# IDEA-Research/MP-Former

Measured on AMD Instinct MI355X. Metric: training images/sec COCO-instance R50 1024x1024, higher is better.
Workload: dtype bf16 (backbone, decoder) + f32 (pixel decoder, losses), as the reference's AMP; 1 GPU; COCO-instance R50, 100 queries, 80 classes, 1024x1024: full train step = R50 backbone + MSDeformAttn pixel decoder (6 layers) + MP masked decoder (9 layers, NUM_DN 1) + Hungarian matching + 60 losses + backward + grad all-reduce + clip + AdamW; head_only_workload=False, global_batch=2, per_gpu_batch=2, parallelism=dp1, msda_offsets=init, full=False, autograd_threads=backward on the launch thread, miopen_find_db=shipped

## Files before the change

include/mpformer_hip.h:

```cpp
#ifndef MPFORMER_HIP_H
#define MPFORMER_HIP_H

#include <stddef.h>
#include <stdint.h>

#ifdef __cplusplus
extern "C" {
#endif

enum { MPF_F32 = 0, MPF_F64 = 1, MPF_BF16 = 2, MPF_U8 = 3, MPF_BITS = 4  };

enum {
    MPF_OK = 0,
    MPF_E_DTYPE = -1,
    MPF_E_SHAPE = -2,
    MPF_E_NULL = -3,
    MPF_E_TOO_LARGE = -4
};

int mpf_abi_version(void);
const char* mpf_last_error(void);


int mpf_msda_forward(const void* value, const int64_t* spatial_shapes,
// ... 174 lines not shown
                       int pad, uint8_t* out, int32_t* flags, int N, int Q, int HW, void* stream);

typedef struct MpfLsaProblem {
    int64_t cost_off, n_rows, n_cols, row_stride;
    int64_t out_pos, col_base;
    int64_t a_base, a_stride, b_base, b_stride;
    int64_t scatter_base;
} MpfLsaProblem;

int mpf_lsa_assign(const float* cost, const MpfLsaProblem* problems, int n_problems, int max_dim, int64_t max_entries,
                   int32_t* row_out, int32_t* col_out, int64_t* aff_a, int64_t* aff_b, int64_t* scatter_dst,
                   const int64_t* scatter_src, void* stream);
int mpf_lsa_assign_status(const float* cost, const MpfLsaProblem* problems, int n_problems, int max_dim, int64_t max_entries,
                          int32_t* row_out, int32_t* col_out, int64_t* aff_a, int64_t* aff_b, int64_t* scatter_dst,
                          const int64_t* scatter_src, int32_t* status, void* stream);

typedef struct MpfDecoderLayer {
    const void *ca_wq, *ca_bq, *ca_wo, *ca_bo;
    const float *ca_gamma, *ca_beta;
    const void *sa_wq, *sa_bq, *sa_wk, *sa_bk, *sa_wv, *sa_bv, *sa_wo, *sa_bo;
    const float *sa_gamma, *sa_beta;
    const void *ff_w1, *ff_b1, *ff_w2, *ff_b2;
    const float *ff_gamma, *ff_beta;
    const float* x0;
    const void* xb0;
    const void *k_c, *v_c;
    const uint8_t *mask_c, *mask_s;
    void *q_c, *kT_c, *o_c;
    float* lse_c;
    float *s1, *mean1, *rstd1;
    void* xb1;
    void *q_s, *k_s, *v_s, *kT_s, *o_s;
    float* lse_s;
    float *s2, *mean2, *rstd2;
    void* xb2;
    void* h;
    float *s3, *mean3, *rstd3;
    float* x3;
    void* xb3;
    void *scratch, *attn_ws;
    uint64_t scratch_bytes, attn_ws_bytes;
    int32_t Qt, N, H, S, ffn_dim;
    float eps;
    int64_t kv_row_stride, kv_img_stride;
} MpfDecoderLayer;

typedef struct MpfDecoderLayerGrad {
    const float* g_x3;
    const void* g_xb3;
    float* d_x0;
    void* d_xb0;
    void *d_k_c, *d_v_c;
    void *d_ca_wq, *d_ca_bq, *d_ca_wo, *d_ca_bo;
    void *d_sa_wq, *d_sa_bq, *d_sa_wk, *d_sa_bk, *d_sa_wv, *d_sa_bv, *d_sa_wo, *d_sa_bo;
    void *d_ff_w1, *d_ff_b1, *d_ff_w2, *d_ff_b2;
    float* d_ln;
    int64_t dkv_row_stride, dkv_img_stride;
    const float* g_x3_plus;
} MpfDecoderLayerGrad;

int mpf_lin256_res_ln_forward(const void* a, const void* w, const void* bias, const float* x, const float* gamma, const float* beta,
                              float* s_out, float* y32, void* y16, float* mean, float* rstd, int rows, float eps, void* stream);
int mpf_ln256_mlp3_forward(const float* x, const float* gamma, const float* beta, const void* w0, const void* b0, const void* w1,
                           const void* b1, const void* w2, const void* b2, void* out, int rows, float eps, void* stream);
uint64_t mpf_decoder_layer_struct_bytes(int which);
uint64_t mpf_decoder_layer_scratch_bytes(int Qt, int N, int H, int S, int ffn_dim, int backward);
int mpf_decoder_layer_forward(const MpfDecoderLayer* layer, void* stream);
typedef struct MpfNextMask {
    const float* x;
    const float* ln_gamma;
    const float* ln_beta;
    const void* w0;
    const void* b0;
    const void* w1;
    const void* b1;
    const void* w2;
    const void* b2;
    const void* pooled;
    const uint8_t* mp_rows;
    uint8_t* out;
    int32_t* flags;
    void* scratch;
    size_t scratch_bytes;
    int N, Q, HW, pad;
    float eps;
} MpfNextMask;
size_t mpf_next_attn_mask_scratch_bytes(int N, int Q);
int mpf_next_attn_mask(const MpfNextMask* m, void* stream);
int mpf_decoder_layer_backward(const MpfDecoderLayer* layer, const MpfDecoderLayerGrad* grad, void* stream);

typedef struct MpfDecoderLayerPos {
    const float* qpos;
    void *xq0, *xq1;
    float* d_qpos;
} MpfDecoderLayerPos;
int mpf_qpos_operand_forward(const float* x, const float* qpos, void* out, int Q, int N, void* stream);
int mpf_qpos_backward(const void* dxq0, const void* dxq1, float* d_x0, float* d_qpos, int Q, int N, void* stream);
uint64_t mpf_decoder_layer_pos_struct_bytes(void);
uint64_t mpf_decoder_layer_pos_scratch_bytes(int Qt, int N, int H, int S, int ffn_dim, int backward);
int mpf_decoder_layer_pos_forward(const MpfDecoderLayer* layer, const MpfDecoderLayerPos* pos, void* stream);
int mpf_decoder_layer_pos_backward(const MpfDecoderLayer* layer, const MpfDecoderLayerPos* pos, const MpfDecoderLayerGrad* grad,
                                   void* stream);

typedef struct MpfScaleCastItem {
    const void* src;
    void* dst;
    const float* scale;
    int64_t numel, inner, first_block;
} MpfScaleCastItem;

int mpf_grouped_scale_cast(const MpfScaleCastItem* items_device, int n_items, int64_t total_blocks, int src_dtype, int dst_dtype,
                           void* stream);

#define MPF_AMAX_SLOT_FLOATS 512
typedef struct MpfAmaxItem {
    const float* src;
    float* out;
    int64_t numel, first_block;
} MpfAmaxItem;
typedef struct MpfSplitItemH2 {
    const float* src;
    void* dst;
    const float* amax;
    int64_t rows, cols, transpose, dst_ld, plane_stride, first_block;
} MpfSplitItemH2;
int mpf_amax_f32(const float* x, int64_t n, float* amax, void* stream);
int mpf_amax_f32_grouped(const MpfAmaxItem* items_device, int n_items, int64_t total_blocks, void* stream);
int mpf_h2_range_stats(const float* a, int rows, int cols, int64_t lda, const float* amax_slot, int log2_below,
                       unsigned long long* counters_device, void* stream);
int mpf_gemm3_split_grouped_h2(const MpfSplitItemH2* items_device, int n_items, int64_t total_blocks, void* stream);
typedef struct MpfNtItemH2 {
    const float* a;
    int64_t lda;
    const float* a_amax;
    const float* b;
    int64_t ldb;
    const float* b_amax;
    float* c_part;
    float* csum_a;
    int64_t Mdim, Ndim;
} MpfNtItemH2;
int mpf_gemm3_nt_h2(const float* a, int64_t lda, const float* a_amax, const float* b, int64_t ldb, const float* b_amax,
                    float* c_part, float* csum_a, float* csum_b, int R, int Mdim, int Ndim, int rows_per_split,
                    int transpose_out, void* stream);
int mpf_gemm3_nt_grouped_h2(const MpfNtItemH2* items, int n_items, int R, int rows_per_split, int64_t split_stride, void* stream);
int mpf_gemm3_conv3x3_h2(const float* x, const float* x_amax, const void* w_planes_h2, const float* w_amax, const float* bias,
                         float* y, float* out_amax, int n_img, int H, int W, int Cin, int Cout, int transposed, void* stream);
int mpf_gemm3_conv3x3_wgrad_h2(const float* dy, const float* dy_amax, const float* x, const float* x_amax, float* c_part,
                               float* csum_dy, int n_img, int H, int W, int Cin, int Cout, int rows_per_split, void* stream);
int mpf_gemm3_tn_h2(const float* a, int64_t lda, const float* a_amax, const void* b_planes_h2, const float* b_amax,
                    const float* bias, const float* c_in, int64_t ldcin, const float* c_in2, int64_t ldcin2,
                    const float* gate, int64_t ldgate, float* c, int64_t ldc, float* out_amax, int M, int N, int K,
                    int relu, void* stream);
int mpf_gemm3_tn_h2_bits(const float* a, int64_t lda, const float* a_amax, const void* b_planes_h2, const float* b_amax,
                         const float* bias, const float* c_in, int64_t ldcin, const float* c_in2, int64_t ldcin2,
                         const unsigned char* gate_bits, int64_t ldgbits, float* c, int64_t ldc, float* out_amax,
                         unsigned char* gate_bits_out, int64_t ldgbits_out, int M, int N, int K, int relu, void* stream);

typedef struct MpfNtItem {
    const float* a;
    int64_t lda;
    const float* b;
    int64_t ldb;
    float* c_part;
    float* csum_a;
    int64_t Mdim, Ndim;
} MpfNtItem;
int mpf_gemm3_nt_grouped(const MpfNtItem* items, int n_items, int R, int rows_per_split, int64_t split_stride, void* stream);

int mpf_gemm3_conv3x3(const float* x, const void* w_planes, const float* bias, float* y, int n_img, int H, int W, int Cin,
                      int Cout, int transposed, void* stream);
int mpf_gemm3_conv3x3_wgrad(const float* dy, const float* x, float* c_part, float* csum_dy, int n_img, int H, int W, int Cin, int Cout,
                            int rows_per_split, void* stream);

int mpf_gemm3_tn_ex(const void* a, int a_dtype, int64_t lda, const void* b_planes, const float* bias, const float* c_in, int64_t ldcin,
                    void* c, int c_dtype, int64_t ldc, int M, int N, int K, int relu, void* stream);
int mpf_gemm3_nt_ex(const void* a, int a_dtype, int64_t lda, const void* b, int b_dtype, int64_t ldb, float* c_part, float* csum_a,
                    int R, int Mdim, int Ndim, int rows_per_split, void* stream);

typedef struct MpfSplitItem {
    const float* src;
    void* dst;
    int64_t rows, cols, transpose, dst_ld, plane_stride, first_block;
} MpfSplitItem;

int mpf_gemm3_split_grouped(const MpfSplitItem* items_device, int n_items, int64_t total_blocks, void* stream);

typedef struct MpfOptItem {
    float* param;
    const float* grad;
    float* exp_avg;
    float* exp_avg_sq;
    int64_t numel, first_block;
    float lr, weight_decay, bc1, bc2_sqrt;
} MpfOptItem;

int mpf_clip_adamw_step(const MpfOptItem* items_device, int n_items, int64_t total_blocks, float max_norm, double beta1,
                        double beta2, double eps, float* partial, float* norm_clip, void* stream);

int mpf_transpose_f32(const float* in, int64_t in_batch_stride, float* out, int64_t out_batch_stride, int B, int R, int C,
                      void* stream);

int mpf_gemm3_nt_reduce(const float* c_part, int64_t c_numel, const float* s_part, int64_t s_numel, int nsplit,
                        float* c_out, float* s_out, void* stream);
int mpf_gemm3_nt_reduce_levels(const float* c_part, int64_t c_numel, const float* s_part, int64_t s_numel, int nsplit,
                               const int64_t* level_of_split, int n_levels, float* c_out, float* lvl_out, float* s_out, void* stream);

int mpf_tall_gemm_bf16(const void* a, int64_t lda, const void* b, int64_t ldb, const void* bias, void* c, int64_t ldc, int M, int N,
                       int K, void* stream);
size_t mpf_gemm_nt_bf16_workspace_bytes(int R, int Mdim, int Ndim, int rows_per_split);
int mpf_gemm_nt_bf16(const void* a, int64_t lda, const void* b, int64_t ldb, void* c_out, void* csum_out, int R, int Mdim,
                     int Ndim, int rows_per_split, void* workspace, size_t workspace_bytes, void* stream);

int mpf_small_gemm_bf16_blocked(const void* a, int64_t a_rs, int64_t a_ks, int a_blk, int64_t a_bs, const void* gate, const void* b,
                                int64_t b_rs, int64_t b_ks, const void* bias, const void* c_in, int64_t ldcin, void* c, int64_t ldc,
                                int c_blk, int64_t c_bs, void* rowsum_a, int I, int J, int Kc, int relu, void* stream);

int mpf_class_loss_forward(const void* logits, int dtype, int64_t sl, int64_t sn, int64_t sq, const int64_t* target,
                           int target_per_output, const float* weight, int L, int N, int Q, int C, float* lse, float* ce,
                           float* wsum, void* stream);
int mpf_class_loss_backward(const void* logits, int dtype, int64_t sl, int64_t sn, int64_t sq, const int64_t* target,
                            int target_per_output, const float* weight, int L, int N, int Q, int C, const float* lse,
                            const float* wsum, const float* grad_ce, void* dlogits, void* stream);
int mpf_mask_loss_finalize(const float* sums, const int64_t* runs, const float* norm, int n, int G, int points, float* out,
                           void* stream);
int mpf_mask_loss_finalize_backward(const float* sums, const int64_t* runs, const float* norm, int n, int G, int points,
                                    const float* grad_out, float* dsums, void* stream);

typedef struct {
    const void* a;
    const void* gate;
    const void* b;
    void* c;
    void* rowsum_a;
    int64_t a_rs, a_ks, a_bs, b_rs, b_ks, ldc;
    int a_blk, I, J, Kc;
} MpfSmallGemmItem;
int mpf_small_gemm_bf16_group(const MpfSmallGemmItem* items, int n_items, void* stream);
typedef struct MpfTransposeItem {
    const void* src;
    const void* gate;
    void* dst;
    int64_t ld;
    int R, C;
} MpfTransposeItem;
int mpf_transpose_group_bf16(const MpfTransposeItem* items, int n_items, int Rp, void* stream);

int mpf_bias_act(const void* x, const float* bias, const void* res, void* y, int64_t numel, int C, int dtype,
                 int relu, void* stream);
int mpf_relu_bwd_add(const void* ga, const void* gb, const void* y, void* out, int64_t numel, int dtype, void* stream);
int mpf_maxpool3x3s2_forward(const void* x, void* y, void* code, int N, int H, int W, int C, void* stream);
int mpf_maxpool3x3s2_backward(const void* gy, const void* code, void* gx, int N, int H, int W, int C, void* stream);

int mpf_upload_small(const void* host_src, void* device_dst, int64_t nbytes, void* stream);

int mpf_res_ln256_forward(const float* x, const void* t, int t_dtype, const float* gamma, const float* beta,
                          float* s_out, float* y32, void* y16, float* mean, float* rstd, int rows, float eps,
                          const float* padd, int padd_rows, float* y_plus, void* stream);
int mpf_res_ln256_forward_b(const float* x, const void* t, int t_dtype, const float* gamma, const float* beta, float* s_out, float* y32,
                            void* y16, float* mean, float* rstd, int rows, float eps, const float* padd, int padd_rows, float* y_plus,
                            float* y_bound, const float* padd_amax, float* yplus_bound, void* stream);
int mpf_res_ln256_backward(const float* s, const float* mean, const float* rstd, const float* gamma, const float* gy32,
                           const void* gy16, const float* gy_plus, float* ds32, void* ds16, float* dgamma, float* dbeta,
                           int rows, void* stream);
size_t mpf_res_ln256_backward_workspace_bytes(int rows);
int mpf_res_ln256_backward_ws(const float* s, const float* mean, const float* rstd, const float* gamma, const float* gy32,
                              const void* gy16, const float* gy_plus, float* ds32, void* ds16, float* dgamma, float* dbeta, int rows,
                              void* workspace, size_t workspace_bytes, void* stream);
int mpf_res_ln256_backward_ws_amax(const float* s, const float* mean, const float* rstd, const float* gamma, const float* gy32,
                                   const void* gy16, const float* gy_plus, float* ds32, void* ds16, float* dgamma, float* dbeta, int rows,
                                   void* workspace, size_t workspace_bytes, float* ds_amax, void* stream);
int mpf_res_ln256_backward_partial(const float* s, const float* mean, const float* rstd, const float* gamma, const float* gy32,
                                   const void* gy16, const float* gy_plus, float* ds32, void* ds16, int rows, void* partials,
                                   size_t partials_bytes, void* stream);
int mpf_res_ln256_backward_partial_amax(const float* s, const float* mean, const float* rstd, const float* gamma, const float* gy32,
                                        const void* gy16, const float* gy_plus, float* ds32, void* ds16, int rows, void* partials,
                                        size_t partials_bytes, float* ds_amax, void* stream);
int mpf_ln_partial_reduce(const void* partials, size_t stride_bytes, int rows, int n_ln, float* out, void* stream);
size_t mpf_res_ln256_backward_det_workspace_bytes(int rows);
int mpf_res_ln256_backward_det(const float* s, const float* mean, const float* rstd, const float* gamma, const float* gy32,
                               const void* gy16, const float* gy_plus, float* ds32, void* ds16, float* dgamma_dbeta, int rows,
                               void* workspace, size_t workspace_bytes, void* stream);
size_t mpf_res_ln256_backward_workspace_bytes(int rows);
int mpf_res_ln256_backward_ws(const float* s, const float* mean, const float* rstd, const float* gamma, const float* gy32,
                              const void* gy16, const float* gy_plus, float* ds32, void* ds16, float* dgamma, float* dbeta, int rows,
                              void* workspace, size_t workspace_bytes, void* stream);

int mpf_mask_loss_backward_dense(const void* pred, int pred_dtype, int h, int w, const int64_t* pred_rows,
                                 const void* gt, int gt_dtype, int H, int W, const int32_t* gt_rows, const float* coords,
                                 const float* grad_sums, void* grad, int grad_dtype, const int64_t* grad_offs,
                                 int n, int P, void* stream);

size_t mpf_group_stats_workspace_bytes(int rows, int64_t row_len);
int mpf_group_stats(const float* x, int rows, int64_t row_len, float eps, float* mean, float* rstd,
                    void* workspace, size_t workspace_bytes, void* stream);

int mpf_gn_cl_supported(int HW, int C, int G);
size_t mpf_gn_cl_workspace_bytes(int N, int HW, int C, int G);
int mpf_gn_cl_forward(const float* x, int64_t x_bs, const float* gamma, const float* beta, int N, int HW, int C, int G,
                      float eps, int relu, const float* top, int64_t top_bs, int W, float* y, int64_t y_bs, float* mean,
                      float* rstd, void* workspace, size_t workspace_bytes, void* stream);
int mpf_gn_cl_backward(const float* gy, int64_t gy_bs, const float* x, int64_t x_bs, const float* gamma, const float* beta,
                       const float* mean, const float* rstd, int N, int HW, int C, int G, int relu, float* dx,
                       int64_t dx_bs, float* dgamma, float* dbeta, void* workspace, size_t workspace_bytes, void* stream);
int mpf_upsample2x_cl_backward(const float* gy, int64_t gy_bs, int N, int Ht, int Wt, int C, float* dtop, int64_t dtop_bs,
                               void* stream);

size_t mpf_match_cost_fused_workspace_bytes(int G, int Q, int Tmax, int P, int tsamp_rows);
int mpf_match_cost_fused(const void* embed, const int64_t* embed_first, int64_t embed_row_stride, const void* features,
                         int64_t feat_img_stride, const int32_t* group_image, int h, int w, int channels, const float* coords,
                         const float* tsamp, int tsamp_rows, const int32_t* t_first, const int32_t* t_count, float* cost, int G,
                         int Q, int Tmax, int P, float w_mask, float w_dice, void* workspace, size_t workspace_bytes, void* stream);
size_t mpf_match_cost_fused_clip_workspace_bytes(int G, int Q, int Tmax, int P, int F, int tsamp_rows);
int mpf_match_cost_fused_clip(const void* embed, const int64_t* embed_first, int64_t embed_row_stride, const void* features,
                              int64_t feat_clip_stride, int64_t feat_frame_stride, const int32_t* group_clip, int h, int w,
                              int channels, const float* coords, const float* tsamp, int tsamp_rows, const int32_t* t_first,
                              const int32_t* t_count, float* cost, int G, int Q, int Tmax, int P, int F, float w_mask, float w_dice,
                              void* workspace, size_t workspace_bytes, void* stream);
int mpf_pair_planes_forward(const void* embed, const int64_t* row_off, const int32_t* pair_of_slot, const int32_t* slot_first,
                            const int32_t* slot_count, const void* features, int64_t feat_img_stride, void* out, int N, int HW,
                            int channels, void* stream);
size_t mpf_pair_planes_backward_workspace_bytes(int N, int HW, int total_slots, int max_count);
int mpf_pair_planes_backward(const void* grad_planes, const void* embed, const int64_t* row_off, const int32_t* pair_of_slot,
                             const int32_t* slot_first, const int32_t* slot_count, const void* features, int64_t feat_img_stride,
                             void* d_features, int64_t dfeat_img_stride, void* d_embed, int d_embed_dtype, int N, int HW, int channels,
                             int total_slots, int max_count, void* workspace, size_t workspace_bytes, void* stream);

int mpf_profile_enable(int on);
int mpf_profile_get(const char* name_substr, int* count, double* total_ms, double* total_bytes);
int mpf_profile_get_flops(const char* name_substr, double* total_flops);

enum {
    MPF_ENC_PV, MPF_ENC_PV_AM, MPF_ENC_PO, MPF_ENC_PO_AM, MPF_ENC_P1, MPF_ENC_P1_AM, MPF_ENC_P2, MPF_ENC_P2_AM, MPF_ENC_P288, MPF_ENC_P288_AM,
    MPF_ENC_BV, MPF_ENC_BO, MPF_ENC_BB1, MPF_ENC_BB2, MPF_ENC_B288, MPF_ENC_G1, MPF_ENC_B1, MPF_ENC_G2, MPF_ENC_B2,
    MPF_ENC_VALUE, MPF_ENC_RAW, MPF_ENC_LOC, MPF_ENC_ATTN, MPF_ENC_AO, MPF_ENC_S1, MPF_ENC_MEAN1, MPF_ENC_RSTD1, MPF_ENC_X1, MPF_ENC_H,
    MPF_ENC_HBITS, MPF_ENC_S2, MPF_ENC_MEAN2, MPF_ENC_RSTD2, MPF_ENC_X2, MPF_ENC_QN,
    MPF_ENC_AO_AM, MPF_ENC_X1_AM, MPF_ENC_H_AM, MPF_ENC_XN_AM, MPF_ENC_QN_AM,
    MPF_ENC_FIELDS
};
typedef struct MpfEncoderCall {
    int32_t N, S, M, L, P, nl, F, reserved;
    float eps, pad_;
    const int64_t* host_shapes;
    const void* shapes_dev;
    const void* lsi_dev;
    const float* ref;
    const float* pos_full;
    const float* pos_am;
    const float* x0;
    const float* x0_am;
    const float* q0;
    const float* q0_am;
    const uint64_t* layers;
} MpfEncoderCall;
int mpf_encoder_fields(void);
int mpf_encoder_forward(const MpfEncoderCall* call, void* stream);

enum {
    MPF_ENCB_X, MPF_ENCB_Q, MPF_ENCB_VALUE, MPF_ENCB_LOC, MPF_ENCB_ATTN, MPF_ENCB_AO, MPF_ENCB_S1, MPF_ENCB_MEAN1, MPF_ENCB_RSTD1, MPF_ENCB_X1,
    MPF_ENCB_H, MPF_ENCB_HBITS, MPF_ENCB_S2, MPF_ENCB_MEAN2, MPF_ENCB_RSTD2,
    MPF_ENCB_X_AM, MPF_ENCB_Q_AM, MPF_ENCB_AO_AM, MPF_ENCB_X1_AM, MPF_ENCB_H_AM,
    MPF_ENCB_G1, MPF_ENCB_G2,
    MPF_ENCB_TV, MPF_ENCB_TV_AM, MPF_ENCB_TO, MPF_ENCB_TO_AM, MPF_ENCB_T1, MPF_ENCB_T1_AM, MPF_ENCB_T2, MPF_ENCB_T2_AM, MPF_ENCB_T288, MPF_ENCB_T288_AM,
    MPF_ENCB_DS2_AM, MPF_ENCB_DH_AM, MPF_ENCB_DS1_AM, MPF_ENCB_DRAW_AM, MPF_ENCB_GV_AM,
    MPF_ENCB_WGRAD, MPF_ENCB_DW288, MPF_ENCB_LVL, MPF_ENCB_DB288,
    MPF_ENCB_FIELDS
};
typedef struct MpfEncoderBwdCall {
    int32_t N, S, M, L, P, nl, F, rps288, rps_group, reserved;
    int64_t group_stride;
    const int64_t* host_shapes;
    const float* gout;
    const int64_t* split_level;
    float *ds2, *dh, *dx1, *ds1, *dao, *gv, *draw;
    float* dq[2];
    float* g[2];
    float *cpart288, *cs288, *part_group;
    void* ln_parts;
    uint64_t ln_stride;
    void* msda_ws;
    uint64_t msda_ws_bytes;
    float* dgb_out;
    const uint64_t* layers;
} MpfEncoderBwdCall;
int mpf_encoder_bwd_fields(void);
int mpf_encoder_backward(const MpfEncoderBwdCall* call, void* stream);

int mpf_seg_softmax(const float* cls, int Q, int K1, float object_mask_threshold, float* probs, float* max_score, int* max_label,
                    int* kept, float* kept_score, void* stream);
int mpf_seg_semantic(const void* masks, int64_t stride_q, int dtype, int Q, int h, int w, int Hp, int Wp, int hi, int wi, int H, int W,
                     const float* probs, int K, float* out, void* stream);
size_t mpf_seg_instance_workspace_bytes(int T, int H, int W);
int mpf_seg_instance_scores(const void* masks, int64_t stride_q, int dtype, int Q, int h, int w, int Hp, int Wp, int hi, int wi, int H,
                            int W, const int64_t* sel_q, const float* cls_score, int T, float* scores, void* workspace,
                            size_t workspace_bytes, void* stream);
int mpf_seg_instance_masks(const void* masks, int64_t stride_q, int dtype, int Q, int h, int w, int Hp, int Wp, int hi, int wi, int H,
                           int W, const int64_t* sel_q, int T, float* masks_out, void* stream);
int mpf_seg_panoptic_areas(const void* masks, int64_t stride_q, int dtype, int Q, int h, int w, int Hp, int Wp, int hi, int wi, int H,
                           int W, const int* kept, const float* kept_score, int* code, int* areas, void* stream);
int mpf_seg_panoptic_paint(const int* code, int H, int W, const int* lut, int* out, void* stream);
int mpf_seg_semantic_labels(const void* masks, int64_t stride_q, int dtype, int Q, int h, int w, int Hp, int Wp, int hi, int wi, int H,
                            int W, const float* probs, int K, int* labels, void* stream);
int mpf_seg_labels_resize(const float* scores, int K, int hi, int wi, int H, int W, int* labels, void* stream);
int mpf_seg_confusion_add(const int* pred, const int* gt, int64_t n, int K, int ignore_label, int64_t* conf, void* stream);
size_t mpf_seg_instance_rle_workspace_bytes(int T, int H, int W);
int mpf_seg_instance_rle_count(const void* masks, int64_t stride_q, int dtype, int Q, int h, int w, int Hp, int Wp, int hi, int wi, int H,
                               int W, const int64_t* sel_q, int T, int64_t* offsets, void* workspace, size_t workspace_bytes,
                               void* stream);
int mpf_seg_instance_rle_write(const void* workspace, size_t workspace_bytes, int T, int H, int W, const int64_t* offsets, int64_t total,
                               uint32_t* pos, uint32_t* counts, void* stream);

int mpf_seg_tta_accumulate(const void* masks, int64_t stride_q, int dtype, int Q, int h, int w, int Hp, int Wp, int hi, int wi, int H,
                           int W, const float* probs, int K, int mode, float* acc, void* stream);
int mpf_seg_tta_resize_add(const float* scores, int K, int hi, int wi, int H, int W, int mode, float* acc, void* stream);
int mpf_seg_tta_finish(float* acc, int K, int H, int W, int count, int* labels , void* stream);

size_t mpf_seg_pq_workspace_bytes(int G, int S);
int mpf_seg_pq_pairs(const int* pred, const void* gt, int gt_format, int64_t n, const int* gt_ids, int G, int gt_base,
                     const int* pred_ids, int S, int pred_base, int void_id, int* table, size_t table_bytes, void* stream);
int mpf_seg_pq_match(int* table, size_t table_bytes, int G, int S, int K, const int* gt_cat, const int* gt_flags, const int* pred_cat,
                     int implicit, int64_t* tp, int64_t* fp, int64_t* fn, double* iou, int64_t* err, void* stream);

int mpf_seg_instance_bits(const void* masks, int64_t stride_q, int dtype, int Q, int h, int w, int Hp, int Wp, int hi, int wi, int H,
                          int W, const int64_t* sel_q, int T, uint64_t* bits, void* stream);
int mpf_seg_pack_masks(const void* masks, int dtype, int M, int H, int W, uint64_t* bits, void* stream);
int mpf_seg_mask_pairs(const uint64_t* a_bits, int T, const uint64_t* b_bits, int G, int64_t nwords, int* inter, int* area_a,
                       int* area_b, void* stream);
size_t mpf_seg_ap_workspace_bytes(int G, int A, int Tn);
int mpf_seg_ap_match(const int* inter, const int* area_d, const int* area_g, int D, int G, const float* dt_score, const int* dt_cat,
                     const int* gt_cat, const int* gt_crowd, const double* gt_area, const double* iou_thrs, int Tn,
                     const double* area_rngs, int A, int K, int max_det, int crowd_rule, int image, int64_t* records, int64_t* npig,
                     void* workspace, size_t workspace_bytes, void* stream);

int mpf_seg_mask_boundary(const uint64_t* bits, int M, int H, int W, int d, uint64_t* out, void* stream);
int mpf_seg_ap_match_boundary(const int* inter, const int* area_d, const int* area_g, const int* inter_b, const int* area_db,
                              const int* area_gb, int D, int G, const float* dt_score, const int* dt_cat, const int* gt_cat,
                              const int* gt_crowd, const double* gt_area, const double* iou_thrs, int Tn, const double* area_rngs, int A,
                              int K, int max_det, int crowd_rule, int image, int64_t* records, int64_t* npig, void* workspace,
                              size_t workspace_bytes, void* stream);

int mpf_seg_bits_boxes(const uint64_t* bits, int M, int H, int W, int* boxes , void* stream);
int mpf_seg_ap_match_box(const double* dt_box , const double* gt_box , int D, int G,
                         const float* dt_score, const int* dt_cat, const int* gt_cat, const int* gt_crowd, const double* gt_area,
                         const double* iou_thrs, int Tn, const double* area_rngs, int A, int K, int max_det, int crowd_rule, int image,
                         int64_t* records, int64_t* npig, void* workspace, size_t workspace_bytes, void* stream);

int mpf_seg_video_bits(const void* masks, int64_t stride_q, int64_t stride_f, int dtype, int Q, int F, int h, int w, int Hp, int Wp,
                       int hi, int wi, int H, int W, const int64_t* sel_q, int T, uint64_t* bits, int* frame_area,
                       uint8_t* dense , void* stream);
int mpf_seg_tube_areas(const int* frame_area, int M, int F, double* avg_area, void* stream);
int mpf_seg_ap_match_tube(const int* inter, const int* area_d, const int* area_g, int D, int G, const float* dt_score, const int* dt_cat,
                          const int* gt_cat, const int* gt_crowd, const double* gt_area, const double* dt_area, const double* iou_thrs,
                          int Tn, const double* area_rngs, int A, int K, int max_det, int crowd_rule, int image, int64_t* records,
                          int64_t* npig, void* workspace, size_t workspace_bytes, void* stream);
size_t mpf_seg_bits_rle_workspace_bytes(int M, int H, int W);
int mpf_seg_bits_rle_count(const uint64_t* bits, int M, int H, int W, int64_t* offsets, void* workspace, size_t workspace_bytes,
                           void* stream);
int mpf_seg_bits_rle_write(const uint64_t* bits, const void* workspace, size_t workspace_bytes, int M, int H, int W,
                           const int64_t* offsets, int64_t total, uint32_t* pos, uint32_t* counts, void* stream);

int mpf_seg_poly_stage_edges(void);
int mpf_seg_poly_toggles(const double* xy, const int64_t* ring_off, int R, int H, int W, uint64_t* planes, void* stream);
int mpf_seg_rle_toggles(const uint32_t* counts, const int64_t* off, int M, int H, int W, uint64_t* planes, void* stream);
int mpf_seg_toggles_fill(const uint64_t* planes, const int* plane_obj, int R, int M, int H, int W, uint64_t* bits, void* stream);
int mpf_seg_unpack_masks(const uint64_t* bits, int M, int H, int W, uint8_t* masks, void* stream);

size_t mpf_win_attn_workspace_bytes(int B, int Hp, int Wp, int heads, int ws);
int mpf_win_attn_forward(const void* qkv, const float* table, void* out, int B, int Hp, int Wp, int heads, int head_dim, int ws,
                         int shift, float scale, void* stream);
int mpf_win_attn_backward(const void* qkv, const float* table, const void* out, const void* dout, void* dqkv, float* dtable, int B,
                          int Hp, int Wp, int heads, int head_dim, int ws, int shift, float scale, void* workspace,
                          size_t workspace_bytes, void* stream);

#ifdef __cplusplus
}
#endif
#endif
```

mp_former_amd/_lib.py:

```python
import ctypes

import torch
import os

_HERE = os.path.dirname(os.path.abspath(__file__))
LIB_PATH = os.path.join(_HERE, "libmpformer_hip.so")
LIB_PATH = os.environ.get("MPF_LIB_PATH", LIB_PATH)
ABI_VERSION = 1

MPF_F32, MPF_F64, MPF_BF16, MPF_U8, MPF_BITS = 0, 1, 2, 3, 4
DTYPE = {torch.float32: MPF_F32, torch.float64: MPF_F64, torch.bfloat16: MPF_BF16, torch.uint8: MPF_U8, torch.bool: MPF_U8}

_lib = None
_status_fns = {}

_c_int = ctypes.c_int
_c_vp = ctypes.c_void_p

SIGNATURES = {
    "mpf_abi_version": (_c_int, []),
    "mpf_last_error": (ctypes.c_char_p, []),
    "mpf_last_kernel": (ctypes.c_char_p, []),
    "mpf_set_option": (_c_int, [ctypes.c_char_p, _c_int]),
    "mpf_match_cost_fused_workspace_bytes": (ctypes.c_size_t, [_c_int] * 5),
    "mpf_match_cost_fused": (_c_int, [_c_vp, _c_vp, ctypes.c_int64, _c_vp, ctypes.c_int64, _c_vp, _c_int, _c_int, _c_int, _c_vp, _c_vp, _c_int,
                                      _c_vp, _c_vp, _c_vp, _c_int, _c_int, _c_int, _c_int, ctypes.c_float, ctypes.c_float, _c_vp,
                                      ctypes.c_size_t, _c_vp]),
    "mpf_match_cost_fused_clip_workspace_bytes": (ctypes.c_size_t, [_c_int] * 6),
    "mpf_match_cost_fused_clip": (_c_int, [_c_vp, _c_vp, ctypes.c_int64, _c_vp, ctypes.c_int64, ctypes.c_int64, _c_vp, _c_int, _c_int, _c_int,
                                           _c_vp, _c_vp, _c_int, _c_vp, _c_vp, _c_vp, _c_int, _c_int, _c_int, _c_int, _c_int, ctypes.c_float,
                                           ctypes.c_float, _c_vp, ctypes.c_size_t, _c_vp]),
    "mpf_pair_planes_forward": (_c_int, [_c_vp] * 6 + [ctypes.c_int64, _c_vp, _c_int, _c_int, _c_int, _c_vp]),
    "mpf_pair_planes_backward_workspace_bytes": (ctypes.c_size_t, [_c_int] * 4),
    "mpf_pair_planes_backward": (_c_int, [_c_vp] * 7 + [ctypes.c_int64, _c_vp, ctypes.c_int64, _c_vp, _c_int, _c_int, _c_int, _c_int, _c_int,
                                          _c_int, _c_vp, ctypes.c_size_t, _c_vp]),
    "mpf_msda_dev_workspace_bytes": (ctypes.c_size_t, [_c_int] * 7),
    "mpf_msda_forward_dev": (_c_int, [_c_vp] * 6 + [_c_int] * 8 + [_c_vp, ctypes.c_size_t, _c_vp]),
    "mpf_msda_backward_dev": (_c_int, [_c_vp] * 9 + [_c_int] * 8 + [_c_vp, ctypes.c_size_t, _c_vp]),
    "mpf_msda_dev_geometry": (_c_int, [_c_vp, ctypes.POINTER(_c_int), _c_int]),
    "mpf_msda_stats": (_c_int, [ctypes.POINTER(ctypes.c_ulonglong), _c_int, _c_int]),
    "mpf_profile_enable": (_c_int, [_c_int]),
    "mpf_profile_get_flops": (_c_int, [ctypes.c_char_p, ctypes.POINTER(ctypes.c_double)]),
    "mpf_profile_get": (_c_int, [ctypes.c_char_p, ctypes.POINTER(_c_int), ctypes.POINTER(ctypes.c_double),
                                 ctypes.POINTER(ctypes.c_double)]),
    "mpf_point_sample": (_c_int, [_c_vp, _c_int, _c_int, _c_int, _c_vp, _c_vp, _c_vp, _c_vp, _c_int, _c_int, _c_vp]),
    "mpf_mask_loss_forward": (_c_int, [_c_vp, _c_int, _c_int, _c_int, _c_vp, _c_vp, _c_int, _c_int, _c_int, _c_vp, _c_vp,
                                       _c_vp, _c_int, _c_int, _c_int, _c_vp]),
    "mpf_pack_mask_bits": (_c_int, [_c_vp, _c_vp, ctypes.c_int64, _c_vp]),
    "mpf_mask_loss_backward": (_c_int, [_c_vp, _c_int, _c_int, _c_int, _c_vp, _c_vp, _c_int, _c_int, _c_vp, _c_vp,
                                        _c_vp, _c_vp, _c_vp, _c_int, _c_int, _c_vp]),
    "mpf_select_uncertain": (_c_int, [_c_vp, _c_vp, _c_vp, _c_int, _c_int, _c_int, _c_int, _c_vp]),
    "mpf_sample_select_uncertain": (_c_int, [_c_vp, _c_int, _c_int, _c_int, _c_vp, _c_vp, _c_vp, _c_int, _c_int, _c_int, _c_int, _c_vp]),
    "mpf_match_cost": (_c_int, [_c_vp, _c_int, _c_int, _c_int, _c_vp, _c_vp, _c_vp, _c_vp, _c_vp, _c_vp, _c_vp,
                                _c_int, _c_int, _c_int, ctypes.c_float, ctypes.c_float, _c_int, _c_vp]),
    "mpf_match_cost_clip_workspace_bytes": (ctypes.c_size_t, [_c_int] * 3),
    "mpf_match_cost_clip": (_c_int, [_c_vp, _c_int, _c_int, _c_int, _c_vp, _c_int, ctypes.c_int64, _c_vp, _c_vp, _c_vp, _c_vp, _c_vp, _c_vp,
                                     _c_int, _c_int, _c_int, ctypes.c_float, ctypes.c_float, _c_int, _c_vp, ctypes.c_size_t, _c_vp]),
    "mpf_attn_mask": (_c_int, [_c_vp, _c_int, ctypes.c_int64, ctypes.c_int64, _c_int, _c_int, _c_vp, _c_int, _c_vp,
                               _c_int, _c_int, _c_int, _c_int, _c_vp]),
    "mpf_attn_workspace_bytes": (ctypes.c_size_t, [_c_int] * 4),
    "mpf_attn_forward": (_c_int, [_c_vp, _c_vp, _c_vp, _c_vp, _c_int, _c_vp, _c_vp, _c_int, _c_int, _c_int, _c_int, _c_int,
                                  ctypes.c_float, _c_vp, ctypes.c_size_t, _c_vp]),
    "mpf_attn_backward": (_c_int, [_c_vp] * 8 + [_c_int] + [_c_vp] * 5 + [_c_int] * 6 + [ctypes.c_float, _c_vp, ctypes.c_size_t, _c_vp]),
    "mpf_attn_transpose2": (_c_int, [_c_vp] * 4 + [_c_int] * 4 + [_c_vp]),
    "mpf_attn_transpose2_strided": (_c_int, [_c_vp] * 2 + [ctypes.c_int64] * 2 + [_c_vp] * 2 + [_c_int] * 4 + [_c_vp]),
    "mpf_attn_forward_kv": (_c_int, [_c_vp, _c_vp, ctypes.c_int64, ctypes.c_int64, _c_vp, _c_vp, _c_int, _c_vp, _c_vp, _c_int, _c_int,
                                     _c_int, _c_int, _c_int, ctypes.c_float, _c_vp, ctypes.c_size_t, _c_vp]),
    "mpf_attn_backward_kv": (_c_int, [_c_vp] * 3 + [ctypes.c_int64] * 2 + [_c_vp] * 5 + [_c_int] + [_c_vp] * 5 + [ctypes.c_int64] * 2
                             + [_c_int] * 6 + [ctypes.c_float, _c_vp, ctypes.c_size_t, _c_vp]),
    "mpf_attn_backward_kv_aux": (_c_int, [_c_vp] * 3 + [ctypes.c_int64] * 2 + [_c_vp] * 5 + [_c_int] + [_c_vp] * 5 + [ctypes.c_int64] * 2
                                 + [_c_int] * 6 + [ctypes.c_float, _c_vp, ctypes.c_size_t, _c_vp, _c_vp]),
    "mpf_attn_bwd_aux_bytes": (ctypes.c_size_t, [_c_int] * 5),
    "mpf_attn_bwd_prep_aux": (_c_int, [_c_vp] * 5 + [_c_int] * 2 + [_c_vp] * 4 + [ctypes.c_size_t] + [_c_int] * 4 + [_c_vp]),
    "mpf_attn_delta": (_c_int, [_c_vp] * 3 + [_c_int] * 3 + [_c_vp]),
    "mpf_attn_bwd_prep": (_c_int, [_c_vp] * 6 + [_c_int] * 4 + [_c_vp]),
    "mpf_win_attn_workspace_bytes": (ctypes.c_size_t, [_c_int] * 5),
    "mpf_win_attn_forward": (_c_int, [_c_vp] * 3 + [_c_int] * 7 + [ctypes.c_float, _c_vp]),
    "mpf_win_attn_backward": (_c_int, [_c_vp] * 6 + [_c_int] * 7 + [ctypes.c_float, _c_vp, ctypes.c_size_t, _c_vp]),
    "mpf_gemm3_split": (_c_int, [_c_vp, _c_int, _c_int, _c_int, _c_vp, _c_vp]),
    "mpf_gemm3_tn": (_c_int, [_c_vp, ctypes.c_int64, _c_vp, _c_int, _c_vp, _c_vp, _c_vp, ctypes.c_int64, _c_vp, ctypes.c_int64,
                           _c_vp, ctypes.c_int64, _c_vp, ctypes.c_int64, _c_int, _c_int, _c_int, _c_int, _c_vp]),
    "mpf_gemm3_nt": (_c_int, [_c_vp, ctypes.c_int64, _c_vp, ctypes.c_int64, _c_vp, ctypes.c_int64, _c_int, _c_vp, _c_vp, _c_vp,
                           _c_int, _c_int, _c_int, _c_int, _c_int, _c_vp]),
    "mpf_amax_f32": (_c_int, [_c_vp, ctypes.c_int64, _c_vp, _c_vp]),
    "mpf_amax_f32_grouped": (_c_int, [_c_vp, _c_int, ctypes.c_int64, _c_vp]),
    "mpf_h2_range_stats": (_c_int, [_c_vp, _c_int, _c_int, ctypes.c_int64, _c_vp, _c_int, _c_vp, _c_vp]),
    "mpf_gemm3_split_grouped_h2": (_c_int, [_c_vp, _c_int, ctypes.c_int64, _c_vp]),
    "mpf_gemm3_tn_h2": (_c_int, [_c_vp, ctypes.c_int64, _c_vp, _c_vp, _c_vp, _c_vp, _c_vp, ctypes.c_int64, _c_vp, ctypes.c_int64,
                              _c_vp, ctypes.c_int64, _c_vp, ctypes.c_int64, _c_vp, _c_int, _c_int, _c_int, _c_int, _c_vp]),
    "mpf_gemm3_tn_h2_bits": (_c_int, [_c_vp, ctypes.c_int64, _c_vp, _c_vp, _c_vp, _c_vp, _c_vp, ctypes.c_int64, _c_vp, ctypes.c_int64,
                                   _c_vp, ctypes.c_int64, _c_vp, ctypes.c_int64, _c_vp, _c_vp, ctypes.c_int64,
                                   _c_int, _c_int, _c_int, _c_int, _c_vp]),
    "mpf_gemm3_nt_h2": (_c_int, [_c_vp, ctypes.c_int64, _c_vp, _c_vp, ctypes.c_int64, _c_vp, _c_vp, _c_vp, _c_vp,
                              _c_int, _c_int, _c_int, _c_int, _c_int, _c_vp]),
    "mpf_gemm3_nt_grouped_h2": (_c_int, [_c_vp, _c_int, _c_int, _c_int, ctypes.c_int64, _c_vp]),
    "mpf_gemm3_conv3x3_h2": (_c_int, [_c_vp] * 7 + [_c_int] * 6 + [_c_vp]),
    "mpf_gemm3_conv3x3_wgrad_h2": (_c_int, [_c_vp, _c_vp, _c_vp, _c_vp, _c_vp, _c_vp, _c_int, _c_int, _c_int, _c_int, _c_int, _c_int, _c_vp]),
    "mpf_gemm3_nt_grouped": (_c_int, [_c_vp, _c_int, _c_int, _c_int, ctypes.c_int64, _c_vp]),
    "mpf_small_gemm_bf16": (_c_int, [_c_vp, ctypes.c_int64, ctypes.c_int64, _c_vp, _c_vp, ctypes.c_int64, ctypes.c_int64, _c_vp, _c_vp,
                                     ctypes.c_int64, _c_vp, ctypes.c_int64, _c_vp, _c_int, _c_int, _c_int, _c_int, _c_vp]),
    "mpf_encoder_fields": (_c_int, []),
    "mpf_encoder_forward": (_c_int, [_c_vp, _c_vp]),
    "mpf_encoder_bwd_fields": (_c_int, []),
    "mpf_encoder_backward": (_c_int, [_c_vp, _c_vp]),
    "mpf_decoder_layer_struct_bytes": (ctypes.c_uint64, [_c_int]),
    "mpf_decoder_layer_scratch_bytes": (ctypes.c_uint64, [_c_int] * 6),
    "mpf_decoder_layer_forward": (_c_int, [_c_vp, _c_vp]),
    "mpf_next_attn_mask_scratch_bytes": (ctypes.c_size_t, [_c_int, _c_int]),
    "mpf_next_attn_mask": (_c_int, [_c_vp, _c_vp]),
    "mpf_lin256_res_ln_forward": (_c_int, [_c_vp] * 11 + [_c_int, ctypes.c_float, _c_vp]),
    "mpf_ln256_mlp3_forward": (_c_int, [_c_vp] * 10 + [_c_int, ctypes.c_float, _c_vp]),
    "mpf_decoder_layer_backward": (_c_int, [_c_vp, _c_vp, _c_vp]),
    "mpf_qpos_operand_forward": (_c_int, [_c_vp, _c_vp, _c_vp, _c_int, _c_int, _c_vp]),
    "mpf_qpos_backward": (_c_int, [_c_vp, _c_vp, _c_vp, _c_vp, _c_int, _c_int, _c_vp]),
    "mpf_decoder_layer_pos_struct_bytes": (ctypes.c_uint64, []),
    "mpf_decoder_layer_pos_scratch_bytes": (ctypes.c_uint64, [_c_int] * 6),
    "mpf_decoder_layer_pos_forward": (_c_int, [_c_vp, _c_vp, _c_vp]),
    "mpf_decoder_layer_pos_backward": (_c_int, [_c_vp, _c_vp, _c_vp, _c_vp]),
    "mpf_pool_features": (_c_int, [_c_vp, _c_int, _c_vp] + [_c_int] * 6 + [_c_vp]),
    "mpf_pool_features_cl": (_c_int, [_c_vp, ctypes.c_int64, _c_int, _c_vp, _c_int, _c_int, _c_int, _c_int, _c_int, _c_int, _c_vp]),
    "mpf_mask_head_bits": (_c_int, [_c_vp, ctypes.c_int64, ctypes.c_int64, _c_vp, _c_vp, _c_int, _c_vp, _c_vp] + [_c_int] * 3 + [_c_vp]),
    "mpf_lsa_assign": (_c_int, [_c_vp, _c_vp, _c_int, _c_int, ctypes.c_int64] + [_c_vp] * 7),
    "mpf_lsa_assign_status": (_c_int, [_c_vp, _c_vp, _c_int, _c_int, ctypes.c_int64] + [_c_vp] * 8),
    "mpf_mask_block_empty": (_c_int, [_c_vp, _c_vp] + [_c_int] * 5 + [_c_vp]),
    "mpf_mp_open_counts": (_c_int, [_c_vp, _c_int, _c_int, _c_vp, _c_vp]),
    "mpf_mp_noise_rows": (_c_int, [_c_vp] * 3 + [_c_int] * 4 + [ctypes.c_double, ctypes.c_uint64, ctypes.c_uint64, _c_vp, _c_vp]),
    "mpf_gemm_nt_bf16_workspace_bytes": (ctypes.c_size_t, [_c_int] * 4),
    "mpf_gemm_nt_bf16": (_c_int, [_c_vp, ctypes.c_int64, _c_vp, ctypes.c_int64, _c_vp, _c_vp, _c_int, _c_int, _c_int, _c_int, _c_vp,
                                  ctypes.c_size_t, _c_vp]),
    "mpf_gemm3_nt_reduce": (_c_int, [_c_vp, ctypes.c_int64, _c_vp, ctypes.c_int64, _c_int, _c_vp, _c_vp, _c_vp]),
    "mpf_grouped_scale_cast": (_c_int, [_c_vp, _c_int, ctypes.c_int64, _c_int, _c_int, _c_vp]),
    "mpf_gemm3_split_grouped": (_c_int, [_c_vp, _c_int, ctypes.c_int64, _c_vp]),
    "mpf_decoder_inputs_forward": (_c_int, [_c_vp, ctypes.c_int64, ctypes.c_int64, _c_vp, _c_vp, _c_vp, _c_vp, _c_int, _c_int, _c_int, _c_int,
                                            _c_vp]),
    "mpf_decoder_inputs_backward": (_c_int, [_c_vp, _c_vp, _c_int, _c_vp, ctypes.c_int64, ctypes.c_int64, _c_int, _c_int, _c_int, _c_vp]),
    "mpf_clip_inputs_forward": (_c_int, [_c_vp, ctypes.c_int64, ctypes.c_int64, _c_vp, _c_vp, _c_vp, _c_vp, _c_vp, _c_int, _c_int, _c_int, _c_int,
                                         _c_int, _c_vp]),
    "mpf_clip_inputs_backward": (_c_int, [_c_vp, _c_vp, _c_int, _c_vp, ctypes.c_int64, ctypes.c_int64, _c_int, _c_int, _c_int, _c_int, _c_vp]),
    "mpf_clip_adamw_step": (_c_int, [_c_vp, _c_int, ctypes.c_int64, ctypes.c_float, ctypes.c_double, ctypes.c_double, ctypes.c_double,
                                     _c_vp, _c_vp, _c_vp]),
    "mpf_transpose_f32": (_c_int, [_c_vp, ctypes.c_int64, _c_vp, ctypes.c_int64, _c_int, _c_int, _c_int, _c_vp]),
    "mpf_small_gemm_bf16_blocked": (_c_int, [_c_vp, ctypes.c_int64, ctypes.c_int64, _c_int, ctypes.c_int64, _c_vp, _c_vp, ctypes.c_int64,
                                             ctypes.c_int64, _c_vp, _c_vp, ctypes.c_int64, _c_vp, ctypes.c_int64, _c_int, ctypes.c_int64,
                                             _c_vp, _c_int, _c_int, _c_int, _c_int, _c_vp]),
    "mpf_small_gemm_bf16_group": (_c_int, [_c_vp, _c_int, _c_vp]),
    "mpf_transpose_group_bf16": (_c_int, [_c_vp, _c_int, _c_int, _c_vp]),
    "mpf_class_loss_forward": (_c_int, [_c_vp, _c_int, ctypes.c_int64, ctypes.c_int64, ctypes.c_int64, _c_vp, _c_int, _c_vp, _c_int, _c_int,
                                        _c_int, _c_int, _c_vp, _c_vp, _c_vp, _c_vp]),
    "mpf_class_loss_backward": (_c_int, [_c_vp, _c_int, ctypes.c_int64, ctypes.c_int64, ctypes.c_int64, _c_vp, _c_int, _c_vp, _c_int, _c_int,
                                         _c_int, _c_int, _c_vp, _c_vp, _c_vp, _c_vp, _c_vp]),
    "mpf_mask_loss_finalize": (_c_int, [_c_vp, _c_vp, _c_vp, _c_int, _c_int, _c_int, _c_vp, _c_vp]),
    "mpf_mask_loss_finalize_backward": (_c_int, [_c_vp, _c_vp, _c_vp, _c_int, _c_int, _c_int, _c_vp, _c_vp, _c_vp]),
    "mpf_bias_act": (_c_int, [_c_vp, _c_vp, _c_vp, _c_vp, ctypes.c_int64, _c_int, _c_int, _c_int, _c_vp]),
    "mpf_relu_bwd_add": (_c_int, [_c_vp, _c_vp, _c_vp, _c_vp, ctypes.c_int64, _c_int, _c_vp]),
    "mpf_maxpool3x3s2_forward": (_c_int, [_c_vp] * 3 + [_c_int] * 4 + [_c_vp]),
    "mpf_maxpool3x3s2_backward": (_c_int, [_c_vp] * 3 + [_c_int] * 4 + [_c_vp]),
    "mpf_upload_small": (_c_int, [_c_vp, _c_vp, ctypes.c_int64, _c_vp]),
    "mpf_tall_gemm_bf16": (_c_int, [_c_vp, ctypes.c_int64, _c_vp, ctypes.c_int64, _c_vp, _c_vp, ctypes.c_int64, _c_int, _c_int, _c_int, _c_vp]),
    "mpf_res_ln256_forward": (_c_int, [_c_vp, _c_vp, _c_int, _c_vp, _c_vp, _c_vp, _c_vp, _c_vp, _c_vp, _c_vp, _c_int, ctypes.c_float,
                                       _c_vp, _c_int, _c_vp, _c_vp]),
    "mpf_res_ln256_forward_b": (_c_int, [_c_vp, _c_vp, _c_int, _c_vp, _c_vp, _c_vp, _c_vp, _c_vp, _c_vp, _c_vp, _c_int, ctypes.c_float,
                                         _c_vp, _c_int, _c_vp, _c_vp, _c_vp, _c_vp, _c_vp]),
    "mpf_res_ln256_backward_ws_amax": (_c_int, [_c_vp] * 11 + [_c_int, _c_vp, ctypes.c_size_t, _c_vp, _c_vp]),
    "mpf_res_ln256_backward": (_c_int, [_c_vp] * 11 + [_c_int, _c_vp]),
    "mpf_mask_loss_backward_dense": (_c_int, [_c_vp, _c_int, _c_int, _c_int, _c_vp, _c_vp, _c_int, _c_int, _c_int, _c_vp, _c_vp, _c_vp,
                                              _c_vp, _c_int, _c_vp, _c_int, _c_int, _c_vp]),
    "mpf_gn_cl_supported": (_c_int, [_c_int, _c_int, _c_int]),
    "mpf_gn_cl_workspace_bytes": (ctypes.c_size_t, [_c_int, _c_int, _c_int, _c_int]),
    "mpf_gn_cl_forward": (_c_int, [_c_vp, ctypes.c_int64, _c_vp, _c_vp, _c_int, _c_int, _c_int, _c_int, ctypes.c_float, _c_int,
                                   _c_vp, ctypes.c_int64, _c_int, _c_vp, ctypes.c_int64, _c_vp, _c_vp, _c_vp, ctypes.c_size_t, _c_vp]),
    "mpf_gn_cl_backward": (_c_int, [_c_vp, ctypes.c_int64, _c_vp, ctypes.c_int64, _c_vp, _c_vp, _c_vp, _c_vp, _c_int, _c_int, _c_int,
                                    _c_int, _c_int, _c_vp, ctypes.c_int64, _c_vp, _c_vp, _c_vp, ctypes.c_size_t, _c_vp]),
    "mpf_upsample2x_cl_backward": (_c_int, [_c_vp, ctypes.c_int64, _c_int, _c_int, _c_int, _c_int, _c_vp, ctypes.c_int64, _c_vp]),
    "mpf_gemm3_conv3x3": (_c_int, [_c_vp, _c_vp, _c_vp, _c_vp, _c_int, _c_int, _c_int, _c_int, _c_int, _c_int, _c_vp]),
    "mpf_gemm3_conv3x3_wgrad": (_c_int, [_c_vp, _c_vp, _c_vp, _c_vp, _c_int, _c_int, _c_int, _c_int, _c_int, _c_int, _c_vp]),
    "mpf_gemm3_nt_reduce_levels": (_c_int, [_c_vp, ctypes.c_int64, _c_vp, ctypes.c_int64, _c_int, _c_vp, _c_int, _c_vp, _c_vp, _c_vp, _c_vp]),
    "mpf_gemm3_tn_ex": (_c_int, [_c_vp, _c_int, ctypes.c_int64, _c_vp, _c_vp, _c_vp, ctypes.c_int64, _c_vp, _c_int, ctypes.c_int64,
                                 _c_int, _c_int, _c_int, _c_int, _c_vp]),
    "mpf_gemm3_nt_ex": (_c_int, [_c_vp, _c_int, ctypes.c_int64, _c_vp, _c_int, ctypes.c_int64, _c_vp, _c_vp, _c_int, _c_int, _c_int, _c_int, _c_vp]),
    "mpf_res_ln256_backward_workspace_bytes": (ctypes.c_size_t, [_c_int]),
    "mpf_res_ln256_backward_partial": (_c_int, [_c_vp] * 9 + [_c_int, _c_vp, ctypes.c_size_t, _c_vp]),
    "mpf_res_ln256_backward_partial_amax": (_c_int, [_c_vp] * 9 + [_c_int, _c_vp, ctypes.c_size_t, _c_vp, _c_vp]),
    "mpf_ln_partial_reduce": (_c_int, [_c_vp, ctypes.c_size_t, _c_int, _c_int, _c_vp, _c_vp]),
    "mpf_res_ln256_backward_det_workspace_bytes": (ctypes.c_size_t, [_c_int]),
    "mpf_res_ln256_backward_det": (_c_int, [_c_vp] * 10 + [_c_int, _c_vp, ctypes.c_size_t, _c_vp]),
    "mpf_res_ln256_backward_ws": (_c_int, [_c_vp] * 11 + [_c_int, _c_vp, ctypes.c_size_t, _c_vp]),
    "mpf_group_stats_workspace_bytes": (ctypes.c_size_t, [_c_int, ctypes.c_int64]),
    "mpf_group_stats": (_c_int, [_c_vp, _c_int, ctypes.c_int64, ctypes.c_float, _c_vp, _c_vp, _c_vp, ctypes.c_size_t, _c_vp]),
    "mpf_msda_forward": (_c_int, [_c_vp] * 6 + [_c_int] * 8 + [_c_vp]),
    "mpf_msda_backward": (_c_int, [_c_vp] * 9 + [_c_int] * 8 + [_c_vp]),
    "mpf_msda_forward_hs": (_c_int, [_c_vp] * 7 + [_c_int] * 8 + [_c_vp]),
    "mpf_msda_forward_raw_hs": (_c_int, [_c_vp] * 9 + [_c_int] * 8 + [_c_vp]),
    "mpf_msda_forward_raw": (_c_int, [_c_vp] * 8 + [_c_int] * 8 + [_c_vp]),
    "mpf_msda_backward_ws_raw": (_c_int, [_c_vp] * 7 + [_c_int] * 8 + [_c_vp, ctypes.c_size_t, _c_vp]),
    "mpf_msda_backward_ws_raw_o": (_c_int, [_c_vp] * 8 + [_c_int] * 8 + [_c_vp, ctypes.c_size_t, _c_vp, _c_vp, _c_vp]),
    "mpf_msda_backward_workspace_bytes": (ctypes.c_size_t, [_c_int] * 5 + [_c_vp]),
    "mpf_msda_backward_ws": (_c_int, [_c_vp] * 8 + [_c_int] * 8 + [_c_vp, ctypes.c_size_t, _c_vp]),
    "mpf_seg_softmax": (_c_int, [_c_vp, _c_int, _c_int, ctypes.c_float] + [_c_vp] * 6),
    "mpf_seg_semantic": (_c_int, [_c_vp, ctypes.c_int64] + [_c_int] * 10 + [_c_vp, _c_int, _c_vp, _c_vp]),
    "mpf_seg_instance_workspace_bytes": (ctypes.c_size_t, [_c_int] * 3),
    "mpf_seg_instance_scores": (_c_int, [_c_vp, ctypes.c_int64] + [_c_int] * 10 + [_c_vp, _c_vp, _c_int, _c_vp, _c_vp, ctypes.c_size_t,
                                                                                   _c_vp]),
    "mpf_seg_instance_masks": (_c_int, [_c_vp, ctypes.c_int64] + [_c_int] * 10 + [_c_vp, _c_int, _c_vp, _c_vp]),
    "mpf_seg_panoptic_areas": (_c_int, [_c_vp, ctypes.c_int64] + [_c_int] * 10 + [_c_vp] * 5),
    "mpf_seg_panoptic_paint": (_c_int, [_c_vp, _c_int, _c_int, _c_vp, _c_vp, _c_vp]),
    "mpf_seg_semantic_labels": (_c_int, [_c_vp, ctypes.c_int64] + [_c_int] * 10 + [_c_vp, _c_int, _c_vp, _c_vp]),
    "mpf_seg_labels_resize": (_c_int, [_c_vp] + [_c_int] * 5 + [_c_vp, _c_vp]),
    "mpf_seg_confusion_add": (_c_int, [_c_vp, _c_vp, ctypes.c_int64, _c_int, _c_int, _c_vp, _c_vp]),
    "mpf_seg_instance_rle_workspace_bytes": (ctypes.c_size_t, [_c_int] * 3),
    "mpf_seg_instance_rle_count": (_c_int, [_c_vp, ctypes.c_int64] + [_c_int] * 10 + [_c_vp, _c_int, _c_vp, _c_vp, ctypes.c_size_t, _c_vp]),
    "mpf_seg_instance_rle_write": (_c_int, [_c_vp, ctypes.c_size_t, _c_int, _c_int, _c_int, _c_vp, ctypes.c_int64, _c_vp, _c_vp, _c_vp]),
    "mpf_seg_tta_accumulate": (_c_int, [_c_vp, ctypes.c_int64] + [_c_int] * 10 + [_c_vp, _c_int, _c_int, _c_vp, _c_vp]),
    "mpf_seg_tta_resize_add": (_c_int, [_c_vp] + [_c_int] * 6 + [_c_vp, _c_vp]),
    "mpf_seg_tta_finish": (_c_int, [_c_vp] + [_c_int] * 4 + [_c_vp, _c_vp]),
    "mpf_seg_pq_workspace_bytes": (ctypes.c_size_t, [_c_int] * 2),
    "mpf_seg_pq_pairs": (_c_int, [_c_vp, _c_vp, _c_int, ctypes.c_int64, _c_vp, _c_int, _c_int, _c_vp, _c_int, _c_int, _c_int, _c_vp,
                                  ctypes.c_size_t, _c_vp]),
    "mpf_seg_pq_match": (_c_int, [_c_vp, ctypes.c_size_t, _c_int, _c_int, _c_int, _c_vp, _c_vp, _c_vp, _c_int] + [_c_vp] * 6),
    "mpf_seg_instance_bits": (_c_int, [_c_vp, ctypes.c_int64] + [_c_int] * 10 + [_c_vp, _c_int, _c_vp, _c_vp]),
    "mpf_seg_pack_masks": (_c_int, [_c_vp, _c_int, _c_int, _c_int, _c_int, _c_vp, _c_vp]),
    "mpf_seg_mask_pairs": (_c_int, [_c_vp, _c_int, _c_vp, _c_int, ctypes.c_int64, _c_vp, _c_vp, _c_vp, _c_vp]),
    "mpf_seg_ap_workspace_bytes": (ctypes.c_size_t, [_c_int] * 3),
    "mpf_seg_ap_match": (_c_int, [_c_vp, _c_vp, _c_vp, _c_int, _c_int] + [_c_vp] * 6 + [_c_int, _c_vp] + [_c_int] * 5
                         + [_c_vp, _c_vp, _c_vp, ctypes.c_size_t, _c_vp]),
    "mpf_seg_mask_boundary": (_c_int, [_c_vp, _c_int, _c_int, _c_int, _c_int, _c_vp, _c_vp]),
    "mpf_seg_ap_match_boundary": (_c_int, [_c_vp] * 6 + [_c_int, _c_int] + [_c_vp] * 6 + [_c_int, _c_vp] + [_c_int] * 5
                                  + [_c_vp, _c_vp, _c_vp, ctypes.c_size_t, _c_vp]),
    "mpf_seg_bits_boxes": (_c_int, [_c_vp, _c_int, _c_int, _c_int, _c_vp, _c_vp]),
    "mpf_seg_ap_match_box": (_c_int, [_c_vp, _c_vp, _c_int, _c_int] + [_c_vp] * 6 + [_c_int, _c_vp] + [_c_int] * 5
                             + [_c_vp, _c_vp, _c_vp, ctypes.c_size_t, _c_vp]),
    "mpf_seg_video_bits": (_c_int, [_c_vp, ctypes.c_int64, ctypes.c_int64] + [_c_int] * 11 + [_c_vp, _c_int, _c_vp, _c_vp, _c_vp, _c_vp]),
    "mpf_seg_tube_areas": (_c_int, [_c_vp, _c_int, _c_int, _c_vp, _c_vp]),
    "mpf_seg_ap_match_tube": (_c_int, [_c_vp, _c_vp, _c_vp, _c_int, _c_int] + [_c_vp] * 7 + [_c_int, _c_vp] + [_c_int] * 5
                              + [_c_vp, _c_vp, _c_vp, ctypes.c_size_t, _c_vp]),
    "mpf_seg_bits_rle_workspace_bytes": (ctypes.c_size_t, [_c_int] * 3),
    "mpf_seg_bits_rle_count": (_c_int, [_c_vp, _c_int, _c_int, _c_int, _c_vp, _c_vp, ctypes.c_size_t, _c_vp]),
    "mpf_seg_bits_rle_write": (_c_int, [_c_vp, _c_vp, ctypes.c_size_t, _c_int, _c_int, _c_int, _c_vp, ctypes.c_int64, _c_vp, _c_vp, _c_vp]),
    "mpf_seg_poly_stage_edges": (_c_int, []),
    "mpf_seg_poly_toggles": (_c_int, [_c_vp, _c_vp, _c_int, _c_int, _c_int, _c_vp, _c_vp]),
    "mpf_seg_rle_toggles": (_c_int, [_c_vp, _c_vp, _c_int, _c_int, _c_int, _c_vp, _c_vp]),
    "mpf_seg_toggles_fill": (_c_int, [_c_vp, _c_vp, _c_int, _c_int, _c_int, _c_int, _c_vp, _c_vp]),
    "mpf_seg_unpack_masks": (_c_int, [_c_vp, _c_int, _c_int, _c_int, _c_vp, _c_vp]),
}


class NativeLibraryError(RuntimeError):
    pass


def lib():
    global _lib
    if _lib is None:
        if not os.path.exists(LIB_PATH):
            raise NativeLibraryError(
                f"{LIB_PATH} not found: build it with `python -c 'import __graft_entry__ as g; g.build()'` "
                "or `make -C mp_former_amd/csrc`.  mp_former_amd has no CPU / eager fallback.")
# ... 125 lines not shown
```

mp_former_amd/csrc/common.hip:

```cpp
#include "mpf_common.h"

#include <stdio.h>

#include <atomic>
#include <mutex>
#include <string>
#include <vector>

namespace {
thread_local char t_err[256] = "";
std::atomic<const char*> g_kernel{""};
}

namespace mpf {
int fail(int code, const char* msg)
{
    snprintf(t_err, sizeof(t_err), "%s", msg);
    return code;
}

int failf(int code, const char* who, const char* what)
{
    snprintf(t_err, sizeof(t_err), "%s: %s", who, what);
    return code;
}

int check(hipError_t err, const char* where)
{
    if (err == hipSuccess) return 0;
    snprintf(t_err, sizeof(t_err), "%s: %s (%d)", where, hipGetErrorString(err), (int)err);
    return (int)err;
}

void set_kernel(const char* name) { g_kernel.store(name, std::memory_order_relaxed); }

namespace {
struct ProfRec { const char* name; hipEvent_t e0, e1; double bytes, flops; };
std::mutex g_prof_mu;
std::vector<ProfRec> g_prof;
std::atomic<int> g_prof_on{0};
thread_local hipEvent_t t_e0 = nullptr;
}

bool prof_enabled() { return g_prof_on.load(std::memory_order_relaxed) != 0; }

void prof_begin(hipStream_t st)
{
    if (!prof_enabled()) return;
    hipEvent_t e;
    if (hipEventCreate(&e) != hipSuccess) { t_e0 = nullptr; return; }
    (void)hipEventRecord(e, st);
    t_e0 = e;
}

void prof_end(const char* name, hipStream_t st, double algorithmic_bytes, double flops)
{
    if (!prof_enabled() || !t_e0) return;
    hipEvent_t e;
    if (hipEventCreate(&e) != hipSuccess) return;
    (void)hipEventRecord(e, st);
    std::lock_guard<std::mutex> lk(g_prof_mu);
    g_prof.push_back({name, t_e0, e, algorithmic_bytes, flops});
    t_e0 = nullptr;
}
}

extern "C" int mpf_profile_enable(int on)
{
    std::lock_guard<std::mutex> lk(mpf::g_prof_mu);
    for (auto& r : mpf::g_prof) { (void)hipEventDestroy(r.e0); (void)hipEventDestroy(r.e1); }
    mpf::g_prof.clear();
    mpf::g_prof_on.store(on ? 1 : 0);
    return 0;
}

extern "C" int mpf_profile_get(const char* name_substr, int* count, double* total_ms, double* total_bytes)
{
    if (!name_substr || !count || !total_ms || !total_bytes) return MPF_E_NULL;
    std::lock_guard<std::mutex> lk(mpf::g_prof_mu);
    int n = 0; double ms = 0, by = 0;
    for (auto& r : mpf::g_prof) {
        if (!strstr(r.name, name_substr)) continue;
        if (hipEventSynchronize(r.e1) != hipSuccess) continue;
        float t = 0.f;
        if (hipEventElapsedTime(&t, r.e0, r.e1) != hipSuccess) continue;
        ms += t; by += r.bytes; ++n;
    }
    *count = n; *total_ms = ms; *total_bytes = by;
    return 0;
}

extern "C" int mpf_profile_get_flops(const char* name_substr, double* total_flops)
{
    if (!name_substr || !total_flops) return MPF_E_NULL;
    std::lock_guard<std::mutex> lk(mpf::g_prof_mu);
    double fl = 0;
    for (auto& r : mpf::g_prof)
        if (strstr(r.name, name_substr)) fl += r.flops;
    *total_flops = fl;
    return 0;
}

namespace {
constexpr int kUpPayload = 3968;
struct UpPayload { uint32_t w[kUpPayload / 4]; };
__global__ __launch_bounds__(256) void upload_small_kernel(UpPayload p, uint32_t* __restrict__ dst, int nwords)
{
    for (int i = threadIdx.x; i < nwords; i += 256) dst[i] = p.w[i];
}
}

extern "C" int mpf_upload_small(const void* host_src, void* device_dst, int64_t nbytes, void* stream)
{
    if (nbytes == 0) return 0;
    if (!host_src || !device_dst) return mpf::fail(MPF_E_NULL, "upload_small: NULL buffer");
    if (nbytes < 0 || (nbytes & 3) || ((uintptr_t)device_dst & 3)) return mpf::fail(MPF_E_SHAPE, "upload_small: size / destination must be multiples of 4 bytes");
    const unsigned char* src = static_cast<const unsigned char*>(host_src);
    unsigned char* dst = static_cast<unsigned char*>(device_dst);
    for (int64_t off = 0; off < nbytes; off += kUpPayload) {
        const int n = (int)((nbytes - off) < kUpPayload ? (nbytes - off) : kUpPayload);
        UpPayload p;
        memcpy(p.w, src + off, (size_t)n);
        hipLaunchKernelGGL(upload_small_kernel, dim3(1), dim3(256), 0, (hipStream_t)stream, p, reinterpret_cast<uint32_t*>(dst + off), n / 4);
    }
    return mpf::check(hipGetLastError(), "mpf_upload_small");
}

extern "C" int mpf_abi_version(void) { return 1; }
extern "C" const char* mpf_last_error(void) { return t_err; }
extern "C" const char* mpf_last_kernel(void) { return g_kernel.load(std::memory_order_relaxed); }

extern "C" int mpf_set_option(const char* key, int value)
{
    if (!key) return MPF_E_NULL;
    int r = mpf::set_msda_option(key, value);
    if (r <= 0) return r;
    r = mpf::set_binned_option(key, value);
    if (r <= 0) return r;
    r = mpf::set_gemm3_option(key, value);
    if (r <= 0) return r;
    r = mpf::set_decoder_option(key, value);
    if (r <= 0) return r;
    r = mpf::set_block_option(key, value);
    if (r <= 0) return r;
    r = mpf::set_attn_option(key, value);
    if (r <= 0) return r;
    r = mpf::set_small_gemm_option(key, value);
    if (r <= 0) return r;
    return mpf::fail(MPF_E_SHAPE, "mpf_set_option: unknown key");
}
```

mp_former_amd/csrc/encoder_layer.hip:

```cpp
#include <hip/hip_runtime.h>
#include <stdint.h>

#include "mpf_common.h"

#define MPF_TRY(expr)                \
    do {                             \
        const int rc_ = (expr);      \
        if (rc_ != 0) return rc_;    \
    } while (0)

extern "C" int mpf_encoder_fields(void) { return MPF_ENC_FIELDS; }
extern "C" int mpf_encoder_bwd_fields(void) { return MPF_ENCB_FIELDS; }

extern "C" int mpf_encoder_forward(const MpfEncoderCall* E, void* st)
{
    if (!E || !E->layers || !E->host_shapes || !E->shapes_dev || !E->lsi_dev || !E->ref || !E->x0 || !E->q0 || !E->x0_am || !E->q0_am)
        return mpf::fail(MPF_E_NULL, "encoder_forward: NULL buffer");
    if (E->N <= 0 || E->S <= 0 || E->M != 8 || E->L <= 0 || E->P <= 0 || E->nl <= 0 || E->F <= 0 || E->F % 128 != 0)
        return mpf::fail(MPF_E_SHAPE, "encoder_forward: needs 8 heads (256 channels), ffn width a multiple of 128, positive sizes");
    if (E->nl > 1 && (!E->pos_full || !E->pos_am)) return mpf::fail(MPF_E_NULL, "encoder_forward: NULL positional term");
    constexpr int C = 256;
    const int R = E->N * E->S, F = E->F, NO = E->M * E->L * E->P * 3;
    const float* x = E->x0;
    const float* x_am = E->x0_am;
    const float* q = E->q0;
    const float* q_am = E->q0_am;
    for (int i = 0; i < E->nl; ++i) {
        const uint64_t* f = E->layers + (size_t)i * MPF_ENC_FIELDS;
        auto P = [&](int k) { return reinterpret_cast<void*>(f[k]); };
        auto PF = [&](int k) { return reinterpret_cast<float*>(f[k]); };
        for (int k = 0; k < MPF_ENC_FIELDS; ++k)
            if (!f[k] && k != MPF_ENC_QN && k != MPF_ENC_QN_AM) return mpf::fail(MPF_E_NULL, "encoder_forward: NULL field in a layer table");
        const bool last = i + 1 == E->nl;
        if (!last && (!f[MPF_ENC_QN] || !f[MPF_ENC_QN_AM])) return mpf::fail(MPF_E_NULL, "encoder_forward: NULL q of the next layer");
        MPF_TRY(mpf_gemm3_tn_h2(x, C, x_am, P(MPF_ENC_PV), PF(MPF_ENC_PV_AM), PF(MPF_ENC_BV), nullptr, 0, nullptr, 0, nullptr, 0,
                                PF(MPF_ENC_VALUE), C, PF(MPF_ENC_AO_AM), R, C, C, 0, st));
        MPF_TRY(mpf_gemm3_tn_h2(q, C, q_am, P(MPF_ENC_P288), PF(MPF_ENC_P288_AM), PF(MPF_ENC_B288), nullptr, 0, nullptr, 0, nullptr, 0,
                                PF(MPF_ENC_RAW), NO, nullptr, R, NO, C, 0, st));
        MPF_TRY(mpf_msda_forward_raw_hs(P(MPF_ENC_VALUE), (const int64_t*)E->shapes_dev, (const int64_t*)E->lsi_dev, E->host_shapes,
                                        P(MPF_ENC_RAW), E->ref, P(MPF_ENC_LOC), P(MPF_ENC_ATTN), P(MPF_ENC_AO), E->N, E->S, E->M, 32,
                                        E->L, E->S, E->P, MPF_F32, st));
        MPF_TRY(mpf_gemm3_tn_h2(PF(MPF_ENC_AO), C, PF(MPF_ENC_AO_AM), P(MPF_ENC_PO), PF(MPF_ENC_PO_AM), PF(MPF_ENC_BO), x, C, nullptr, 0,
                                nullptr, 0, PF(MPF_ENC_S1), C, nullptr, R, C, C, 0, st));
        MPF_TRY(mpf_res_ln256_forward_b(PF(MPF_ENC_S1), nullptr, 0, PF(MPF_ENC_G1), PF(MPF_ENC_B1), nullptr, PF(MPF_ENC_X1), nullptr,
                                        PF(MPF_ENC_MEAN1), PF(MPF_ENC_RSTD1), R, E->eps, nullptr, 0, nullptr, PF(MPF_ENC_X1_AM), nullptr,
                                        nullptr, st));
        MPF_TRY(mpf_gemm3_tn_h2_bits(PF(MPF_ENC_X1), C, PF(MPF_ENC_X1_AM), P(MPF_ENC_P1), PF(MPF_ENC_P1_AM), PF(MPF_ENC_BB1), nullptr, 0,
                                     nullptr, 0, nullptr, 0, PF(MPF_ENC_H), F, PF(MPF_ENC_H_AM), (unsigned char*)P(MPF_ENC_HBITS), F / 8,
                                     R, F, C, 1, st));
        MPF_TRY(mpf_gemm3_tn_h2(PF(MPF_ENC_H), F, PF(MPF_ENC_H_AM), P(MPF_ENC_P2), PF(MPF_ENC_P2_AM), PF(MPF_ENC_BB2), PF(MPF_ENC_X1), C,
                                nullptr, 0, nullptr, 0, PF(MPF_ENC_S2), C, nullptr, R, C, F, 0, st));
        MPF_TRY(mpf_res_ln256_forward_b(PF(MPF_ENC_S2), nullptr, 0, PF(MPF_ENC_G2), PF(MPF_ENC_B2), nullptr, PF(MPF_ENC_X2), nullptr,
                                        PF(MPF_ENC_MEAN2), PF(MPF_ENC_RSTD2), R, E->eps, last ? nullptr : E->pos_full, last ? 0 : E->S,
                                        last ? nullptr : PF(MPF_ENC_QN), PF(MPF_ENC_XN_AM), last ? nullptr : E->pos_am,
                                        last ? nullptr : PF(MPF_ENC_QN_AM), st));
        x = PF(MPF_ENC_X2); x_am = PF(MPF_ENC_XN_AM);
        q = PF(MPF_ENC_QN); q_am = PF(MPF_ENC_QN_AM);
    }
    return 0;
}

extern "C" int mpf_encoder_backward(const MpfEncoderBwdCall* E, void* st)
{
    if (!E || !E->layers || !E->host_shapes || !E->gout || !E->split_level || !E->ds2 || !E->dh || !E->dx1 || !E->ds1 || !E->dao || !E->gv ||
        !E->draw || !E->dq[0] || !E->dq[1] || !E->g[0] || !E->g[1] || !E->cpart288 || !E->cs288 || !E->part_group || !E->ln_parts ||
        !E->msda_ws || !E->dgb_out)
        return mpf::fail(MPF_E_NULL, "encoder_backward: NULL buffer");
    if (E->N <= 0 || E->S <= 0 || E->M != 8 || E->L <= 0 || E->L > 4 || E->P <= 0 || E->nl <= 0 || E->F <= 0 || E->F % 128 != 0 || E->rps288 <= 0 ||
        E->rps_group <= 0 || E->group_stride <= 0)
        return mpf::fail(MPF_E_SHAPE, "encoder_backward: bad sizes");
    constexpr int C = 256;
    const int R = E->N * E->S, F = E->F, NO = E->M * E->L * E->P * 3;
    const int ns288 = (R + E->rps288 - 1) / E->rps288, nsg = (R + E->rps_group - 1) / E->rps_group;
    const float* g_in = E->gout;
    const float* gq_in = nullptr;
    int kln = 0;
    char* parts = static_cast<char*>(E->ln_parts);
    for (int i = E->nl - 1; i >= 0; --i) {
        const uint64_t* f = E->layers + (size_t)i * MPF_ENCB_FIELDS;
        for (int k = 0; k < MPF_ENCB_FIELDS; ++k)
            if (!f[k]) return mpf::fail(MPF_E_NULL, "encoder_backward: NULL field in a layer table");
        auto P = [&](int k) { return reinterpret_cast<void*>(f[k]); };
        auto PF = [&](int k) { return reinterpret_cast<float*>(f[k]); };
        float* g_out = E->g[i & 1];
        float* dq = E->dq[i & 1];
        MPF_TRY(mpf_res_ln256_backward_partial_amax(PF(MPF_ENCB_S2), PF(MPF_ENCB_MEAN2), PF(MPF_ENCB_RSTD2), PF(MPF_ENCB_G2), g_in, nullptr,
                                                    gq_in, E->ds2, nullptr, R, parts + (size_t)kln * E->ln_stride, E->ln_stride,
                                                    PF(MPF_ENCB_DS2_AM), st));
        ++kln;
        MPF_TRY(mpf_gemm3_tn_h2_bits(E->ds2, C, PF(MPF_ENCB_DS2_AM), P(MPF_ENCB_T2), PF(MPF_ENCB_T2_AM), nullptr, nullptr, 0, nullptr, 0,
                                     (const unsigned char*)P(MPF_ENCB_HBITS), F / 8, E->dh, F, PF(MPF_ENCB_DH_AM), nullptr, 0, R, F, C, 0, st));
        MPF_TRY(mpf_gemm3_tn_h2(E->dh, F, PF(MPF_ENCB_DH_AM), P(MPF_ENCB_T1), PF(MPF_ENCB_T1_AM), nullptr, E->ds2, C, nullptr, 0, nullptr, 0,
                                E->dx1, C, nullptr, R, C, F, 0, st));
        MPF_TRY(mpf_res_ln256_backward_partial_amax(PF(MPF_ENCB_S1), PF(MPF_ENCB_MEAN1), PF(MPF_ENCB_RSTD1), PF(MPF_ENCB_G1), E->dx1, nullptr,
                                                    nullptr, E->ds1, nullptr, R, parts + (size_t)kln * E->ln_stride, E->ln_stride,
                                                    PF(MPF_ENCB_DS1_AM), st));
        ++kln;
        MPF_TRY(mpf_gemm3_tn_h2(E->ds1, C, PF(MPF_ENCB_DS1_AM), P(MPF_ENCB_TO), PF(MPF_ENCB_TO_AM), nullptr, nullptr, 0, nullptr, 0, nullptr, 0,
                                E->dao, C, nullptr, R, C, C, 0, st));
        MPF_TRY(mpf_msda_backward_ws_raw_o(P(MPF_ENCB_VALUE), E->host_shapes, P(MPF_ENCB_LOC), P(MPF_ENCB_ATTN), E->dao, P(MPF_ENCB_AO), E->gv,
                                           E->draw, E->N, E->S, E->M, 32, E->L, E->S, E->P, MPF_F32, E->msda_ws, E->msda_ws_bytes,
                                           PF(MPF_ENCB_DRAW_AM), PF(MPF_ENCB_GV_AM), st));
        MPF_TRY(mpf_gemm3_tn_h2(E->draw, NO, PF(MPF_ENCB_DRAW_AM), P(MPF_ENCB_T288), PF(MPF_ENCB_T288_AM), nullptr, nullptr, 0, nullptr, 0,
                                nullptr, 0, dq, C, nullptr, R, C, NO, 0, st));
        MPF_TRY(mpf_gemm3_nt_h2(PF(MPF_ENCB_Q), C, PF(MPF_ENCB_Q_AM), E->draw, NO, PF(MPF_ENCB_DRAW_AM), E->cpart288, nullptr, E->cs288, R, C, NO,
                                E->rps288, 1, st));
        MPF_TRY(mpf_gemm3_nt_reduce_levels(E->cpart288, (int64_t)C * NO, E->cs288, NO, ns288, E->split_level, E->L, PF(MPF_ENCB_DW288),
                                           PF(MPF_ENCB_LVL), PF(MPF_ENCB_DB288), st));
        MPF_TRY(mpf_gemm3_tn_h2(E->gv, C, PF(MPF_ENCB_GV_AM), P(MPF_ENCB_TV), PF(MPF_ENCB_TV_AM), nullptr, E->ds1, C, i == 0 ? dq : nullptr,
                                i == 0 ? C : 0, nullptr, 0, g_out, C, nullptr, R, C, C, 0, st));
        {
            float* part = E->part_group;
            const int64_t o2 = 0, o1 = o2 + (int64_t)C * F + C, oo = o1 + (int64_t)F * C + F, ov = oo + (int64_t)C * C + C;
            MpfNtItemH2 it[4] = {
                {E->ds2, C, PF(MPF_ENCB_DS2_AM), PF(MPF_ENCB_H), F, PF(MPF_ENCB_H_AM), part + o2, part + o2 + (int64_t)C * F, C, F},
                {E->dh, F, PF(MPF_ENCB_DH_AM), PF(MPF_ENCB_X1), C, PF(MPF_ENCB_X1_AM), part + o1, part + o1 + (int64_t)F * C, F, C},
                {E->ds1, C, PF(MPF_ENCB_DS1_AM), PF(MPF_ENCB_AO), C, PF(MPF_ENCB_AO_AM), part + oo, part + oo + (int64_t)C * C, C, C},
                {E->gv, C, PF(MPF_ENCB_GV_AM), PF(MPF_ENCB_X), C, PF(MPF_ENCB_X_AM), part + ov, part + ov + (int64_t)C * C, C, C}};
            if (ov + (int64_t)C * C + C != E->group_stride) return mpf::fail(MPF_E_SHAPE, "encoder_backward: group_stride does not match the four gradients");
            MPF_TRY(mpf_gemm3_nt_grouped_h2(it, 4, R, E->rps_group, E->group_stride, st));
            MPF_TRY(mpf_gemm3_nt_reduce(part, E->group_stride, nullptr, 0, nsg, PF(MPF_ENCB_WGRAD), nullptr, st));
        }
        g_in = g_out;
        gq_in = dq;
    }
    return mpf_ln_partial_reduce(E->ln_parts, E->ln_stride, R, kln, E->dgb_out, st);
}
```

mp_former_amd/csrc/gemm3.hip:

```cpp
#include <hip/hip_runtime.h>

#include <algorithm>
#include <atomic>
#include <stdint.h>
#include <stdio.h>

#include "mpf_common.h"
#include "amax.h"
#ifndef G3_PRIO
#define G3_PRIO 1
#endif

namespace {

typedef __attribute__((ext_vector_type(8))) __bf16 bf16x8;
typedef __attribute__((ext_vector_type(4))) float f32x4;

constexpr int kBM = 128;
constexpr int kBK = 32;
constexpr int kThreads = 256;
constexpr int kAKc = kBM * 16;

struct G3 {
    const float* a;
    const float* a2;
    const unsigned short* bp;
    const float* bias;
    const float* cin;
    const float* cin2;
    const float* gate;
    float* c;
    int64_t lda, ldc, ldcin, ldcin2, ldgate, plane;
    int M, N, K, a2_rows, relu, tiles_n, ntiles;
    int bias_cm, cin_cm, cin2_cm, gate_cm;
    unsigned short* c16;
    int cv_H, cv_W, cv_cin, cv_sign;
    int tm0, ntiles2, tiles_n2;
    const float* a_amax;
    const float* b_amax;
    float* out_amax;
    const unsigned char* gbits;
    unsigned char* gbits_out;
    int64_t ldgbits, ldgbits_out;
    int gbits_cm;
    int t3_bm;
};

int g_ablate = 0;
int g_mixed = 1;
int g_two_pass = 256;
int g_two_pass_rows = 0;
int g_nt2 = 1;
int g_tn3 = 1;
int g_tn3_176 = 1;
int g_ws = 512;


__device__ __forceinline__ unsigned pack_hi16(unsigned a, unsigned b)
{
    return __builtin_amdgcn_perm(b, a, 0x07060302u);
}

__device__ __forceinline__ void split8(const float4 u, const float4 v, uint4* h, uint4* m, uint4* l)
{
    const float x[8] = {u.x, u.y, u.z, u.w, v.x, v.y, v.z, v.w};
    unsigned hb[8], mb[8], lb[8];
#pragma unroll
    for (int i = 0; i < 8; ++i) {
        const unsigned xb = __float_as_uint(x[i]);
        hb[i] = xb;
        const float r1 = x[i] - __uint_as_float(xb & 0xFFFF0000u);
        const unsigned rb = __float_as_uint(r1);
        mb[i] = rb;
        const float r2 = r1 - __uint_as_float(rb & 0xFFFF0000u);
        lb[i] = __float_as_uint(r2) + 0x8000u;
    }
    *h = make_uint4(pack_hi16(hb[0], hb[1]), pack_hi16(hb[2], hb[3]), pack_hi16(hb[4], hb[5]), pack_hi16(hb[6], hb[7]));
    *m = make_uint4(pack_hi16(mb[0], mb[1]), pack_hi16(mb[2], mb[3]), pack_hi16(mb[4], mb[5]), pack_hi16(mb[6], mb[7]));
    *l = make_uint4(pack_hi16(lb[0], lb[1]), pack_hi16(lb[2], lb[3]), pack_hi16(lb[4], lb[5]), pack_hi16(lb[6], lb[7]));
}

typedef __attribute__((ext_vector_type(8))) _Float16 f16x8;
typedef __attribute__((ext_vector_type(2))) _Float16 f16x2;
typedef __attribute__((ext_vector_type(2))) float f32x2;

__device__ __forceinline__ void split8h(const float4 u, const float4 v, const float scale, uint4* h, uint4* l)
{
    const float x[8] = {u.x, u.y, u.z, u.w, v.x, v.y, v.z, v.w};
    unsigned hb[4], lb[4];
#pragma unroll
    for (int i = 0; i < 4; ++i) {
        const f32x2 s = {x[2 * i] * scale, x[2 * i + 1] * scale};
        const f16x2 hh = __builtin_convertvector(s, f16x2);
        const f32x2 back = __builtin_convertvector(hh, f32x2);
        const f32x2 r = {s[0] - back[0], s[1] - back[1]};
        const f16x2 ll = __builtin_convertvector(r, f16x2);
        union { f16x2 f; unsigned u; } ch, cl;
        ch.f = hh; cl.f = ll;
        hb[i] = ch.u; lb[i] = cl.u;
    }
    *h = make_uint4(hb[0], hb[1], hb[2], hb[3]);
    *l = make_uint4(lb[0], lb[1], lb[2], lb[3]);
}

__device__ __forceinline__ void h2_scale(const unsigned amax_bits, float* scale, float* inv)
{
    int e = (int)((amax_bits >> 23) & 0xffu);
    e = max(e, 30);
    *scale = __uint_as_float((unsigned)(268 - e) << 23);
    *inv = __uint_as_float((unsigned)(e - 14) << 23);
}

__device__ __forceinline__ f16x8 as_fragh(const uint4 v)
{
    union { uint4 u; f16x8 f; } c;
    c.u = v;
    return c.f;
}

__device__ __forceinline__ float4 add4(float4 x, float4 y) { return make_float4(x.x + y.x, x.y + y.y, x.z + y.z, x.w + y.w); }

__device__ __forceinline__ bf16x8 as_frag(const uint4 v)
{
    union { uint4 u; bf16x8 f; } c;
    c.u = v;
    return c.f;
}

typedef __attribute__((ext_vector_type(16))) float f32x16;

template <int NJ, bool W32 = false>
struct Acc {
    f32x4 v[4][NJ];

    __device__ __forceinline__ void zero()
    {
#pragma unroll
        for (int i = 0; i < 4; ++i)
#pragma unroll
            for (int j = 0; j < NJ; ++j) v[i][j] = f32x4{0.f, 0.f, 0.f, 0.f};
    }

    struct NoHook { __device__ __forceinline__ void operator()(int) const {} };

    template <int AKC, int BKC, bool ONE = false, bool A1 = false, bool BROW = false, typename Hook = NoHook>
    __device__ __forceinline__ void step(const unsigned char* lds, int a_base, int b_base, int lane, Hook hook = Hook())
    {
        const int r16 = lane & 15, g = lane >> 4;
        constexpr int BJ = BROW ? 1024 : 256;
        const int a_frag = a_base + g * AKC + (r16 ^ (2 * g)) * 16;
        const int b_frag = BROW ? b_base + (r16 * 4 + (g ^ ((0 - (r16 >> 2)) & 3))) * 16 : b_base + g * BKC + (r16 ^ (2 * g)) * 16;
        if (A1) {
            bf16x8 fa0[4];
#pragma unroll
            for (int i = 0; i < 4; ++i) fa0[i] = as_frag(*reinterpret_cast<const uint4*>(lds + a_frag + i * 256));
#pragma unroll
            for (int j = 0; j < NJ; ++j) {
                bf16x8 fb[3];
#pragma unroll
                for (int pl = 0; pl < 3; ++pl)
                    fb[pl] = as_frag(*reinterpret_cast<const uint4*>(lds + b_frag + pl * 4 * BKC + j * BJ));
#pragma unroll
                for (int i = 0; i < 4; ++i) v[i][j] = __builtin_amdgcn_mfma_f32_16x16x32_bf16(fb[2], fa0[i], v[i][j], 0, 0, 0);
#pragma unroll
                for (int i = 0; i < 4; ++i) v[i][j] = __builtin_amdgcn_mfma_f32_16x16x32_bf16(fb[1], fa0[i], v[i][j], 0, 0, 0);
#pragma unroll
                for (int i = 0; i < 4; ++i) v[i][j] = __builtin_amdgcn_mfma_f32_16x16x32_bf16(fb[0], fa0[i], v[i][j], 0, 0, 0);
            }
            return;
        }
        if (ONE) {
            bf16x8 fa0[4];
#pragma unroll
            for (int i = 0; i < 4; ++i) fa0[i] = as_frag(*reinterpret_cast<const uint4*>(lds + a_frag + i * 256));
#pragma unroll
            for (int j = 0; j < NJ; ++j) {
                const bf16x8 fb0 = as_frag(*reinterpret_cast<const uint4*>(lds + b_frag + j * BJ));
#pragma unroll
                for (int i = 0; i < 4; ++i) v[i][j] = __builtin_amdgcn_mfma_f32_16x16x32_bf16(fb0, fa0[i], v[i][j], 0, 0, 0);
            }
            return;
        }
        bf16x8 fa[3][4];
#pragma unroll
        for (int pl = 0; pl < 3; ++pl)
#pragma unroll
            for (int i = 0; i < 4; ++i)
                fa[pl][i] = as_frag(*reinterpret_cast<const uint4*>(lds + a_frag + pl * 4 * AKC + i * 256));
#pragma unroll
        for (int j = 0; j < NJ; ++j) {
            bf16x8 fb[3];
#pragma unroll
            for (int pl = 0; pl < 3; ++pl)
                fb[pl] = as_frag(*reinterpret_cast<const uint4*>(lds + b_frag + pl * 4 * BKC + j * BJ));
#pragma unroll
            for (int i = 0; i < 4; ++i) v[i][j] = __builtin_amdgcn_mfma_f32_16x16x32_bf16(fb[0], fa[2][i], v[i][j], 0, 0, 0);
#pragma unroll
            for (int i = 0; i < 4; ++i) v[i][j] = __builtin_amdgcn_mfma_f32_16x16x32_bf16(fb[2], fa[0][i], v[i][j], 0, 0, 0);
#pragma unroll
            for (int i = 0; i < 4; ++i) v[i][j] = __builtin_amdgcn_mfma_f32_16x16x32_bf16(fb[1], fa[1][i], v[i][j], 0, 0, 0);
#pragma unroll
            for (int i = 0; i < 4; ++i) v[i][j] = __builtin_amdgcn_mfma_f32_16x16x32_bf16(fb[0], fa[1][i], v[i][j], 0, 0, 0);
#pragma unroll
            for (int i = 0; i < 4; ++i) v[i][j] = __builtin_amdgcn_mfma_f32_16x16x32_bf16(fb[1], fa[0][i], v[i][j], 0, 0, 0);
#pragma unroll
            for (int i = 0; i < 4; ++i) v[i][j] = __builtin_amdgcn_mfma_f32_16x16x32_bf16(fb[0], fa[0][i], v[i][j], 0, 0, 0);
            hook(j);
        }
    }

    template <int AKC, int BKC, bool BROW = false>
    __device__ __forceinline__ void step_h2(const unsigned char* lds, int a_base, int b_base, int lane)
    {
        const int r16 = lane & 15, g = lane >> 4;
        constexpr int BJ = BROW ? 1024 : 256;
        const int a_frag = a_base + g * AKC + (r16 ^ (2 * g)) * 16;
        const int b_frag = BROW ? b_base + (r16 * 4 + (g ^ ((0 - (r16 >> 2)) & 3))) * 16 : b_base + g * BKC + (r16 ^ (2 * g)) * 16;
        f16x8 fa[2][4];
#pragma unroll
        for (int pl = 0; pl < 2; ++pl)
#pragma unroll
            for (int i = 0; i < 4; ++i) fa[pl][i] = as_fragh(*reinterpret_cast<const uint4*>(lds + a_frag + pl * 4 * AKC + i * 256));
#pragma unroll
        for (int j = 0; j < NJ; ++j) {
            f16x8 fb[2];
#pragma unroll
            for (int pl = 0; pl < 2; ++pl) fb[pl] = as_fragh(*reinterpret_cast<const uint4*>(lds + b_frag + pl * 4 * BKC + j * BJ));
#pragma unroll
            for (int i = 0; i < 4; ++i) v[i][j] = __builtin_amdgcn_mfma_f32_16x16x32_f16(fb[1], fa[0][i], v[i][j], 0, 0, 0);
#pragma unroll
            for (int i = 0; i < 4; ++i) v[i][j] = __builtin_amdgcn_mfma_f32_16x16x32_f16(fb[0], fa[1][i], v[i][j], 0, 0, 0);
#pragma unroll
            for (int i = 0; i < 4; ++i) v[i][j] = __builtin_amdgcn_mfma_f32_16x16x32_f16(fb[0], fa[0][i], v[i][j], 0, 0, 0);
        }
    }

    template <typename F>
    __device__ __forceinline__ void quads(int lane, F f) const
    {
        const int r16 = lane & 15, g = lane >> 4;
#pragma unroll
        for (int j = 0; j < NJ; ++j)
#pragma unroll
            for (int i = 0; i < 4; ++i) f(i * 16 + r16, j * 16 + g * 4, make_float4(v[i][j][0], v[i][j][1], v[i][j][2], v[i][j][3]));
    }
};

template <>
struct Acc<4, true> {
    f32x16 v[2][2];

    __device__ __forceinline__ void zero()
    {
#pragma unroll
        for (int i = 0; i < 2; ++i)
#pragma unroll
            for (int j = 0; j < 2; ++j)
#pragma unroll
                for (int e = 0; e < 16; ++e) v[i][j][e] = 0.f;
    }

    template <int AKC, int BKC, bool ONE = false, bool A1 = false, bool B1 = false>
    __device__ __forceinline__ void step(const unsigned char* lds, int a_base, int b_base, int lane)
    {
// ... 1142 lines not shown
        for (int c = lane; c < cols / 4; c += 64) {
            const float4 v = row[c];
            m = fmaxf(fmaxf(m, fmaxf(fabsf(v.x), fabsf(v.y))), fmaxf(fabsf(v.z), fabsf(v.w)));
        }
#pragma unroll
        for (int o = 32; o >= 1; o >>= 1) m = fmaxf(m, __shfl_xor(m, o));
        nz += m > 0.f;
        below += (m > 0.f && m < thr);
    }
    __shared__ unsigned red[8];
    if (lane == 0) { red[wave * 2] = nz; red[wave * 2 + 1] = below; }
    __syncthreads();
    if (threadIdx.x < 2) {
        const unsigned v = red[threadIdx.x] + red[2 + threadIdx.x] + red[4 + threadIdx.x] + red[6 + threadIdx.x];
        if (v) atomicAdd(counters + threadIdx.x, (unsigned long long)v);
    }
}

extern "C" int mpf_h2_range_stats(const float* a, int rows, int cols, int64_t lda, const float* amax_slot, int log2_below,
                                  unsigned long long* counters_device, void* stream)
{
    if (!a || !amax_slot || !counters_device) return mpf::fail(MPF_E_NULL, "h2_range_stats: NULL buffer");
    if (rows <= 0 || cols <= 0 || cols % 4 || lda < cols || lda % 4 || ((uintptr_t)a & 15) || log2_below < 0 || log2_below > 120)
        return mpf::fail(MPF_E_SHAPE, "h2_range_stats: cols and lda must be multiples of 4, a 16-byte aligned, 0 <= log2_below <= 120");
    const int blocks = std::min(2048, (rows + 3) / 4);
    mpf::set_kernel("h2_range_stats_kernel");
    hipLaunchKernelGGL(h2_range_stats_kernel, dim3(blocks), dim3(256), 0, (hipStream_t)stream, a, rows, cols, lda, amax_slot, log2_below,
                       counters_device);
    return mpf::check(hipGetLastError(), "mpf_h2_range_stats");
}

extern "C" int mpf_amax_f32_grouped(const MpfAmaxItem* items_device, int n_items, int64_t total_blocks, void* stream)
{
    if (n_items == 0 || total_blocks == 0) return 0;
    if (!items_device) return mpf::fail(MPF_E_NULL, "amax_f32_grouped: NULL table");
    if (n_items < 0 || total_blocks < 0 || total_blocks > 0x7fffffffLL) return mpf::fail(MPF_E_SHAPE, "amax_f32_grouped: bad sizes");
    mpf::set_kernel("amax_grouped_kernel");
    hipLaunchKernelGGL(amax_grouped_kernel, dim3((unsigned)total_blocks), dim3(256), 0, (hipStream_t)stream, items_device, n_items);
    return mpf::check(hipGetLastError(), "mpf_amax_f32_grouped");
}

extern "C" int mpf_gemm3_split_grouped_h2(const MpfSplitItemH2* items_device, int n_items, int64_t total_blocks, void* stream)
{
    if (n_items == 0 || total_blocks == 0) return 0;
    if (!items_device) return mpf::fail(MPF_E_NULL, "gemm3_split_grouped_h2: NULL table");
    if (n_items < 0 || total_blocks < 0 || total_blocks > 0x7fffffffLL) return mpf::fail(MPF_E_SHAPE, "gemm3_split_grouped_h2: bad sizes");
    mpf::set_kernel("gemm3_split_grouped_h2_kernel");
    hipLaunchKernelGGL(gemm3_split_grouped_h2_kernel, dim3((unsigned)total_blocks), dim3(256), 0, (hipStream_t)stream, items_device,
                       n_items);
    return mpf::check(hipGetLastError(), "mpf_gemm3_split_grouped_h2");
}

int mpf::set_gemm3_option(const char* key, int v)
{
    if (!strcmp(key, "gemm3_mixed_tiles")) { g_mixed = v; return 0; }
    if (!strcmp(key, "gemm3_two_pass")) { g_two_pass = v; return 0; }
    if (!strcmp(key, "gemm3_two_pass_rows")) { g_two_pass_rows = v; return 0; }
    if (!strcmp(key, "gemm3_ws")) { g_ws = v; return 0; }
    if (!strcmp(key, "gemm3_tn3")) { g_tn3 = v; return 0; }
    if (!strcmp(key, "gemm3_tn3_176")) { g_tn3_176 = v; return 0; }
    if (!strcmp(key, "gemm3_nt2")) { g_nt2 = v; return 0; }
    if (strcmp(key, "gemm3_ablate") != 0) return 1;
    g_ablate = v;
    return 0;
}

extern "C" int mpf_gemm3_split(const float* w, int rows, int cols, int transpose, void* planes, void* stream)
{
    hipStream_t st = (hipStream_t)stream;
    if (!w || !planes) return mpf::fail(MPF_E_NULL, "gemm3_split: NULL buffer");
    if (rows <= 0 || cols <= 0) return mpf::fail(MPF_E_SHAPE, "gemm3_split: bad sizes");
    const int64_t total = (int64_t)rows * cols;
    const int blocks = (int)((total + 255) / 256 < 2048 ? (total + 255) / 256 : 2048);
    mpf::set_kernel("gemm3_split_kernel");
    hipLaunchKernelGGL(gemm3_split_kernel, dim3(blocks), dim3(256), 0, st, w, (unsigned short*)planes, rows, cols, transpose);
    return mpf::check(hipGetLastError(), "mpf_gemm3_split");
}

extern "C" int mpf_gemm3_split_grouped(const MpfSplitItem* items_device, int n_items, int64_t total_blocks, void* stream)
{
    if (n_items == 0 || total_blocks == 0) return 0;
    if (!items_device) return mpf::fail(MPF_E_NULL, "gemm3_split_grouped: NULL table");
    if (n_items < 0 || total_blocks < 0 || total_blocks > 0x7fffffffLL) return mpf::fail(MPF_E_SHAPE, "gemm3_split_grouped: bad sizes");
    mpf::set_kernel("gemm3_split_grouped_kernel");
    hipLaunchKernelGGL(gemm3_split_grouped_kernel, dim3((unsigned)total_blocks), dim3(256), 0, (hipStream_t)stream, items_device,
                       n_items);
    return mpf::check(hipGetLastError(), "mpf_gemm3_split_grouped");
}

namespace {

struct Route {
    const void* fn = nullptr;
    const char* name = nullptr;
    const char* what = nullptr;
    int threads = kThreads;
    int blocks = 0;
    size_t lds = 0;
    mpf::LdsAttr* attr = nullptr;
    double w_el = 6.0;
    int arg[2] = {0, 0};
};

struct Work { double bytes, flops; };

template <typename P>
int g3_launch(const Route& r, const P& p, hipStream_t st, const Work w)
{
    if (r.lds)
        if (int e = mpf::ensure_dynamic_lds(r.fn, r.lds, *r.attr)) return e;
    mpf::prof_begin(st);
    mpf::set_kernel(r.name);
    void* args[] = {(void*)&p, (void*)&r.arg[0], (void*)&r.arg[1]};
    if (hipError_t e = hipLaunchKernel(r.fn, dim3(r.blocks), dim3(r.threads), args, r.lds, st); e != hipSuccess) return mpf::check(e, r.what);
    mpf::prof_end(r.name, st, w.bytes, w.flops);
    return mpf::check(hipGetLastError(), r.what);
}

constexpr int round8(int tiles) { return (tiles + 7) / 8 * 8; }
constexpr int cdiv(int a, int b) { return (a + b - 1) / b; }
inline int g3_slots() { return 2 * mpf::cu_count(); }

struct ColTile { int bn, tiles_n; };
inline ColTile g3_col_tile(int N)
{
    const int t128 = cdiv(N, 128), t96 = cdiv(N, 96);
    return t96 * 96 < t128 * 128 ? ColTile{96, t96} : ColTile{128, t128};
}


int g3_fill(G3& p, const char* who, const void* a, int64_t lda, const void* planes, const float* bias, int64_t ldc, int M, int N, int K)
{
    const float* consts = nullptr;
    if (int rc = g3_consts(&consts, who)) return rc;
    p = G3{};
    p.a = (const float*)a; p.lda = lda; p.bp = (const unsigned short*)planes; p.plane = (int64_t)N * K; p.ldc = ldc;
    p.M = M; p.N = N; p.K = K;
    p.bias = bias ? bias : consts; p.bias_cm = bias ? 1 : 0;
    p.cin = p.cin2 = consts; p.gate = consts + 4;
    p.gbits = reinterpret_cast<const unsigned char*>(consts + 8);
    p.cv_sign = 1;
    p.t3_bm = kT3BM;
    return 0;
}

inline void g3_operand(const float*& slot, int64_t& ld, int& cm, const float* v, int64_t ldv)
{
    if (v) { slot = v; ld = ldv; cm = 1; }
}

inline Work g3_tn_work(const G3& p, const Route& r, double a_el = 4.0)
{
    const double M = p.M, N = p.N, K = p.K;
    return {a_el * M * (p.cv_cin ? p.cv_cin : p.K) + (p.c16 ? 2.0 : 4.0) * M * N + r.w_el * N * K, 2.0 * M * N * K};
}

Route g3_ws_route(const G3& p)
{
    static const struct { int key; const void* fn; } kEpilogues[] = {
        {0, (const void*)gemm3_ws_kernel<0, false, false, false>},  {8, (const void*)gemm3_ws_kernel<1, false, false, false>},
        {2, (const void*)gemm3_ws_kernel<0, false, true, false>},   {10, (const void*)gemm3_ws_kernel<1, false, true, false>},
        {3, (const void*)gemm3_ws_kernel<0, false, true, true>},    {4, (const void*)gemm3_ws_kernel<0, true, false, false>},
        {12, (const void*)gemm3_ws_kernel<1, true, false, false>}};
    static mpf::LdsAttr attr[sizeof(kEpilogues) / sizeof(kEpilogues[0])];
    const int key = (p.cin_cm ? 8 : 0) | (p.gbits_cm ? 4 : 0) | (p.relu ? 2 : 0) | (p.gbits_out ? 1 : 0);
    Route r;
    for (size_t i = 0; i < sizeof(kEpilogues) / sizeof(kEpilogues[0]); ++i) {
        if (kEpilogues[i].key != key) continue;
        const int ncg = p.N / 256;
        int per_xcd = mpf::cu_count() / 8 / ncg * ncg;
        if (per_xcd < ncg) per_xcd = ncg;
        int workers = per_xcd / ncg * 8;
        const int tiles16 = cdiv(p.M, 16);
        if (workers > tiles16) workers = round8(tiles16);
        r.fn = kEpilogues[i].fn; r.name = "gemm3_tn_kernel<h2 ws>"; r.what = "mpf_gemm3_tn_h2(ws)";
        r.threads = kWsThreads; r.lds = kWsLds; r.attr = &attr[i]; r.w_el = 4.0;
        r.blocks = workers * ncg;
        r.arg[0] = cdiv(cdiv(p.M, workers), 16) * 16;
        r.arg[1] = ncg;
    }
    return r;
}

Route g3_tn_route(G3& p, bool a_bf16, const char* what)
{
    const bool h2 = p.a_amax != nullptr, a2 = p.a2 != nullptr, a_al16 = ((uintptr_t)p.a & 15) == 0;
    const int M = p.M, N = p.N;
    const ColTile ct = g3_col_tile(N);
    const int tiles_m = cdiv(M, kBM);
    p.tiles_n = ct.tiles_n;
    p.ntiles = tiles_m * ct.tiles_n;
    Route r;
    r.what = what;
    r.w_el = h2 ? 4.0 : 6.0;
    if (h2 && !a2 && !p.gate_cm && !p.cin2_cm && g_ws > 0 && N >= g_ws && p.K == kWsK && N % 256 == 0 && a_al16) {
        const Route ws = g3_ws_route(p);
        if (ws.fn) return ws;
    }
    if (h2 && !a2 && g_tn3 && N % 256 == 0 && M >= 2048 && a_al16 && p.lda % 4 == 0) {
        const int cus = mpf::cu_count(), nt3 = cdiv(M, kT3BM) * (N / 256), rem = nt3 % cus;
        if (g_tn3 == 2 || (nt3 >= cus * 3 / 4 && (rem == 0 || 4 * rem >= 3 * cus || nt3 >= 4 * cus))) {
            const int nt176 = cdiv(M, 176) * (N / 256);
            static mpf::LdsAttr attr;
            if (g_tn3_176 && cdiv(nt176, cus) <= cdiv(nt3, cus)) p.t3_bm = 176;
            p.tiles_n = N / 256;
            p.ntiles = cdiv(M, p.t3_bm) * p.tiles_n;
            r.fn = (const void*)gemm3_tn3_kernel;
            r.name = p.t3_bm == kT3BM ? "gemm3_tn_kernel<h2 192x256>" : "gemm3_tn_kernel<h2 192x256:176>";
            r.what = "mpf_gemm3_tn_h2(192x256)";
            r.threads = kT3T; r.lds = kT3Lds; r.attr = &attr;
            r.blocks = round8(p.ntiles);
            return r;
        }
    }
    if (!a2 && !a_bf16 && g_two_pass > 0 && N % 256 == 0 && N >= g_two_pass) {
        const int slots = g3_slots();
        p.tiles_n = N / 256;
        const int t128 = cdiv(M, 128) * p.tiles_n, t96 = cdiv(M, 96) * p.tiles_n;
        const bool rows96 = g_two_pass_rows == 96 || (g_two_pass_rows == 0 && cdiv(t96, slots) * 96 < cdiv(t128, slots) * 128);
        p.ntiles = rows96 ? t96 : t128;
        if (h2) {
            r.fn = rows96 ? (const void*)gemm3_tn2_kernel<96, false, true> : (const void*)gemm3_tn2_kernel<128, false, true>;
            r.name = rows96 ? "gemm3_tn_kernel<h2 96x256>" : "gemm3_tn_kernel<h2 128x256>";
        } else {
            r.fn = rows96 ? (const void*)gemm3_tn2_kernel<96> : (const void*)gemm3_tn2_kernel<128>;
            r.name = rows96 ? "gemm3_tn_kernel<96x256>" : "gemm3_tn_kernel<128x256>";
        }
        r.blocks = round8(p.ntiles);
        return r;
    }
    const bool w96 = ct.bn == 96;
    r.blocks = round8(p.ntiles);
    if (h2) {
        r.fn = w96 ? (const void*)gemm3_tn_kernel<96, false, true> : (const void*)gemm3_tn_kernel<128, false, true>;
        r.name = w96 ? "gemm3_tn_kernel<h2 96>" : "gemm3_tn_kernel<h2 128>";
        r.what = "mpf_gemm3_tn_h2";
        return r;
    }
    if (!w96 && N % 64 == 0 && g_mixed && !a_bf16 && !p.c16) {
        const int slots = g3_slots(), rounds = p.ntiles / slots, rem = p.ntiles - rounds * slots;
        if (rounds >= 1 && rem > 0 && 2 * rem <= slots && slots % p.tiles_n == 0) {
            p.tm0 = rounds * (slots / p.tiles_n);
            p.tiles_n2 = N / 64;
            p.ntiles2 = (tiles_m - p.tm0) * p.tiles_n2;
            p.ntiles = p.tm0 * p.tiles_n;
            r.fn = a2 ? (const void*)gemm3_tn_mixed_kernel<true> : (const void*)gemm3_tn_mixed_kernel<false>;
            r.name = "gemm3_tn_kernel<128+64>";
            r.blocks = round8(p.ntiles) + round8(p.ntiles2);
            return r;
        }
    }
    if (a_bf16) {
        r.fn = w96 ? (const void*)gemm3_tn_abf_kernel<96> : (const void*)gemm3_tn_abf_kernel<128>;
        r.name = "gemm3_tn_kernel<a16>";
    } else if (a2) {
        r.fn = w96 ? (const void*)gemm3_tn_kernel<96, true> : (const void*)gemm3_tn_kernel<128, true>;
        r.name = w96 ? "gemm3_tn_kernel<96>" : "gemm3_tn_kernel<128>";
    } else {
        r.fn = w96 ? (const void*)gemm3_tn_kernel<96, false> : (const void*)gemm3_tn_kernel<128, false>;
        r.name = p.c16 ? "gemm3_tn_kernel<c16>" : w96 ? "gemm3_tn_kernel<96>" : "gemm3_tn_kernel<128>";
    }
    return r;
}

Route g3_conv_route(G3& p)
{
    const bool h2 = p.a_amax != nullptr, two_pass = h2 || (g_two_pass > 0 && p.N % 256 == 0);
    Route r;
    r.what = "mpf_gemm3_conv3x3";
    r.w_el = h2 ? 4.0 : 6.0;
    r.name = h2 ? "gemm3_conv_kernel<h2>" : "gemm3_conv_kernel";
    r.fn = h2 ? (const void*)gemm3_tn2_kernel<128, true, true> : two_pass ? (const void*)gemm3_tn2_kernel<128, true> : (const void*)gemm3_conv_kernel;
    p.tiles_n = two_pass ? p.N / 256 : cdiv(p.N, 128);
    p.ntiles = cdiv(p.M, kBM) * p.tiles_n;
    r.blocks = round8(p.ntiles);
    return r;
}

int g3_tn_impl(const float* a, int64_t lda, const float* a2, int a2_rows, const void* b_planes,
               const float* bias, const float* c_in, int64_t ldcin, const float* c_in2, int64_t ldcin2,
               const float* gate, int64_t ldgate, float* c, int64_t ldc, int M, int N, int K,
               int relu, void* stream, const float* a_amax, const float* b_amax, float* out_amax,
               const unsigned char* gbits = nullptr, int64_t ldgbits = 0, unsigned char* gbits_out = nullptr,
               int64_t ldgbits_out = 0)
{
    if (!a || !b_planes || !c) return mpf::fail(MPF_E_NULL, "gemm3_tn: NULL buffer");
    if (M <= 0 || N <= 0 || K <= 0) return mpf::fail(MPF_E_SHAPE, "gemm3_tn: bad sizes");
    if (K % kBK != 0 || N % 4 != 0 || lda % 4 != 0 || ldc % 4 != 0 || (c_in && ldcin % 4 != 0) || (c_in2 && ldcin2 % 4 != 0) ||
        (gate && ldgate % 4 != 0))
        return mpf::fail(MPF_E_SHAPE, "gemm3_tn: K must be a multiple of 32; N, lda, ldc multiples of 4");
    if (a2 && a2_rows <= 0) return mpf::fail(MPF_E_SHAPE, "gemm3_tn: a2_rows must be positive");
    G3 p;
    if (int rc = g3_fill(p, "gemm3_tn: constants", a, lda, b_planes, bias, ldc, M, N, K)) return rc;
    p.c = c; p.a2 = a2; p.a2_rows = a2_rows; p.relu = relu;
    g3_operand(p.cin, p.ldcin, p.cin_cm, c_in, ldcin);
    g3_operand(p.cin2, p.ldcin2, p.cin2_cm, c_in2, ldcin2);
    g3_operand(p.gate, p.ldgate, p.gate_cm, gate, ldgate);
    if (gbits) { p.gbits = gbits; p.ldgbits = ldgbits; p.gbits_cm = 1; }
    p.gbits_out = gbits_out; p.ldgbits_out = ldgbits_out;
    p.a_amax = a_amax; p.b_amax = b_amax; p.out_amax = out_amax;
    const Route r = g3_tn_route(p, false, "mpf_gemm3_tn");
    return g3_launch(r, p, (hipStream_t)stream, g3_tn_work(p, r));
}

int g3_conv_impl(const float* x, const void* w_planes, const float* bias, float* y, int n_img, int H, int W, int Cin,
                 int Cout, int transposed, void* stream, const float* x_amax, const float* w_amax, float* out_amax)
{
    if (!x || !w_planes || !y) return mpf::fail(MPF_E_NULL, "gemm3_conv3x3: NULL buffer");
    if (n_img <= 0 || H <= 0 || W <= 0 || Cin <= 0 || Cout <= 0 || Cin % 32 != 0 || Cout % 4 != 0)
        return mpf::fail(MPF_E_SHAPE, "gemm3_conv3x3: Cin must be a multiple of 32, Cout of 4");
    const int64_t M64 = (int64_t)n_img * H * W;
    if (M64 >= (1ll << 31) / 4 || M64 * Cin >= (1ll << 40)) return mpf::fail(MPF_E_TOO_LARGE, "gemm3_conv3x3: image too large");
    G3 p;
    if (int rc = g3_fill(p, "gemm3_conv3x3: constants", x, Cin, w_planes, bias, Cout, (int)M64, Cout, 9 * Cin)) return rc;
    p.c = y;
    p.cv_H = H; p.cv_W = W; p.cv_cin = Cin; p.cv_sign = transposed ? -1 : 1;
    p.a_amax = x_amax; p.b_amax = w_amax; p.out_amax = out_amax;
    const Route r = g3_conv_route(p);
    return g3_launch(r, p, (hipStream_t)stream, g3_tn_work(p, r));
}

}

extern "C" int mpf_gemm3_tn(const float* a, int64_t lda, const float* a2, int a2_rows, const void* b_planes,
                            const float* bias, const float* c_in, int64_t ldcin, const float* c_in2, int64_t ldcin2,
                            const float* gate, int64_t ldgate, float* c, int64_t ldc, int M, int N, int K,
                            int relu, void* stream)
{
    return g3_tn_impl(a, lda, a2, a2_rows, b_planes, bias, c_in, ldcin, c_in2, ldcin2, gate, ldgate, c, ldc, M, N, K, relu, stream,
                      nullptr, nullptr, nullptr);
}

extern "C" int mpf_gemm3_tn_h2(const float* a, int64_t lda, const float* a_amax, const void* b_planes_h2, const float* b_amax,
                               const float* bias, const float* c_in, int64_t ldcin, const float* c_in2, int64_t ldcin2,
                               const float* gate, int64_t ldgate, float* c, int64_t ldc, float* out_amax, int M, int N, int K,
                               int relu, void* stream)
{
    if (!a_amax || !b_amax) return mpf::fail(MPF_E_NULL, "gemm3_tn_h2: NULL amax");
    return g3_tn_impl(a, lda, nullptr, 0, b_planes_h2, bias, c_in, ldcin, c_in2, ldcin2, gate, ldgate, c, ldc, M, N, K, relu, stream,
                      a_amax, b_amax, out_amax);
}

extern "C" int mpf_gemm3_tn_h2_bits(const float* a, int64_t lda, const float* a_amax, const void* b_planes_h2, const float* b_amax,
                                    const float* bias, const float* c_in, int64_t ldcin, const float* c_in2, int64_t ldcin2,
                                    const unsigned char* gate_bits, int64_t ldgbits, float* c, int64_t ldc, float* out_amax,
                                    unsigned char* gate_bits_out, int64_t ldgbits_out, int M, int N, int K, int relu, void* stream)
{
    if (!a_amax || !b_amax) return mpf::fail(MPF_E_NULL, "gemm3_tn_h2_bits: NULL amax");
    if (N % 128 != 0 || (gate_bits && (ldgbits < N / 8 || ldgbits % 8 != 0 || ((uintptr_t)gate_bits & 7))) ||
        (gate_bits_out && (ldgbits_out < N / 8 || ldgbits_out % 8 != 0 || ((uintptr_t)gate_bits_out & 7))))
        return mpf::fail(MPF_E_SHAPE, "gemm3_tn_h2_bits: N must be a multiple of 128; mask rows of >= N / 8 bytes, 8-byte aligned");
    return g3_tn_impl(a, lda, nullptr, 0, b_planes_h2, bias, c_in, ldcin, c_in2, ldcin2, nullptr, 0, c, ldc, M, N, K, relu, stream,
                      a_amax, b_amax, out_amax, gate_bits, ldgbits, gate_bits_out, ldgbits_out);
}

extern "C" int mpf_gemm3_tn_ex(const void* a, int a_dtype, int64_t lda, const void* b_planes, const float* bias, const float* c_in,
                               int64_t ldcin, void* c, int c_dtype, int64_t ldc, int M, int N, int K, int relu, void* stream)
{
    if (!a || !b_planes || !c) return mpf::fail(MPF_E_NULL, "gemm3_tn_ex: NULL buffer");
    if ((a_dtype != MPF_F32 && a_dtype != MPF_BF16) || (c_dtype != MPF_F32 && c_dtype != MPF_BF16))
        return mpf::fail(MPF_E_DTYPE, "gemm3_tn_ex: a / c must be MPF_F32 or MPF_BF16");
    const bool a16 = a_dtype == MPF_BF16;
    if (M <= 0 || N <= 0 || K <= 0 || K % kBK != 0 || N % 4 != 0 || lda % (a16 ? 8 : 4) != 0 || ldc % 4 != 0 || (c_in && ldcin % 4 != 0) ||
        ((uintptr_t)a & 15))
        return mpf::fail(MPF_E_SHAPE, "gemm3_tn_ex: K must be a multiple of 32, N / ldc of 4, 16-byte aligned A rows");
    if (!a16 && c_dtype == MPF_F32)
        return mpf_gemm3_tn((const float*)a, lda, nullptr, 0, b_planes, bias, c_in, ldcin, nullptr, 0, nullptr, 0, (float*)c, ldc, M, N, K, relu, stream);
    G3 p;
    if (int rc = g3_fill(p, "gemm3_tn_ex: constants", a, lda, b_planes, bias, ldc, M, N, K)) return rc;
    if (c_dtype == MPF_BF16) p.c16 = (unsigned short*)c;
    else p.c = (float*)c;
    p.relu = relu;
    g3_operand(p.cin, p.ldcin, p.cin_cm, c_in, ldcin);
    const Route r = g3_tn_route(p, a16, "mpf_gemm3_tn_ex");
    return g3_launch(r, p, (hipStream_t)stream, g3_tn_work(p, r, a16 ? 2.0 : 4.0));
}

extern "C" int mpf_gemm3_conv3x3(const float* x, const void* w_planes, const float* bias, float* y, int n_img, int H, int W, int Cin,
                                 int Cout, int transposed, void* stream)
{
    return g3_conv_impl(x, w_planes, bias, y, n_img, H, W, Cin, Cout, transposed, stream, nullptr, nullptr, nullptr);
}

extern "C" int mpf_gemm3_conv3x3_h2(const float* x, const float* x_amax, const void* w_planes_h2, const float* w_amax, const float* bias,
                                    float* y, float* out_amax, int n_img, int H, int W, int Cin, int Cout, int transposed, void* stream)
{
    if (!x_amax || !w_amax) return mpf::fail(MPF_E_NULL, "gemm3_conv3x3_h2: NULL amax");
    if (Cout % 256 != 0) return mpf::fail(MPF_E_SHAPE, "gemm3_conv3x3_h2: Cout must be a multiple of 256");
    return g3_conv_impl(x, w_planes_h2, bias, y, n_img, H, W, Cin, Cout, transposed, stream, x_amax, w_amax, out_amax);
}

namespace {

int g3n_fill(G3N& p, const char* who, const void* a, int64_t lda, int el_a, const void* b, int64_t ldb, int el_b, float* c_part,
             float* csum_a, int R, int Mdim, int Ndim, int rows_per_split)
{
    const uint64_t ab = ((uint64_t)(R - 1) * lda + Mdim) * el_a, bb = ((uint64_t)(R - 1) * ldb + Ndim) * el_b;
    if (ab >= (1ull << 32) || bb >= (1ull << 32) || lda * el_a >= (1ll << 31) || ldb * el_b >= (1ll << 31)) {
        char msg[96];
        snprintf(msg, sizeof(msg), "%s: an operand spans 4 GiB or more", who);
        return mpf::fail(MPF_E_TOO_LARGE, msg);
    }
    p = G3N{};
    p.a = (const float*)a; p.b = (const float*)b; p.c = c_part; p.csum_a = csum_a;
    p.lda = lda; p.ldb = ldb;
    p.R = R; p.Mdim = Mdim; p.Ndim = Ndim; p.rows_per_split = rows_per_split;
    p.nsplit = cdiv(R, rows_per_split);
    p.a_bytes = (unsigned)ab; p.b_bytes = (unsigned)bb;
    p.c_ss = (int64_t)Mdim * Ndim; p.csa_ss = Mdim; p.csb_ss = Ndim;
    return 0;
}

inline void g3n_tiles(G3N& p, int bm, int bn)
{
    p.tiles_m = cdiv(p.Mdim, bm);
    p.tiles_n = cdiv(p.Ndim, bn);
    p.ntiles = p.tiles_m * p.tiles_n * p.nsplit;
}

inline Route g3n_route(const void* fn, const char* name, const char* what, int tiles)
{
    Route r;
    r.fn = fn; r.name = name; r.what = what; r.blocks = round8(tiles);
    return r;
}

inline Route g3n_route_256(const void* fn, mpf::LdsAttr& attr, const char* name, const char* what, int tiles)
{
    Route r = g3n_route(fn, name, what, tiles);
    r.threads = kN2T; r.lds = kN2Lds; r.attr = &attr;
    return r;
}

inline Work g3n_work(const G3N& p, double a_el = 4.0, double b_el = 4.0)
{
    const double R = p.R, M = p.Mdim, N = p.Ndim;
    return {a_el * R * M + b_el * R * (p.cv_cin ? p.cv_cin : p.Ndim) + 4.0 * p.nsplit * M * N, 2.0 * R * M * N};
}

int g3_nt_impl(const float* a, int64_t lda, const float* b, int64_t ldb, const float* b2, int64_t ldb2, int b2_rows,
               float* c_part, float* csum_a, float* csum_b, int R, int Mdim, int Ndim, int rows_per_split,
               int transpose_out, void* stream, const float* a_amax, const float* b_amax)
{
    if (!a || !b || !c_part) return mpf::fail(MPF_E_NULL, "gemm3_nt: NULL buffer");
    if (R <= 0 || Mdim <= 0 || Ndim <= 0 || rows_per_split <= 0 || rows_per_split % kBK != 0)
        return mpf::fail(MPF_E_SHAPE, "gemm3_nt: bad sizes (rows_per_split must be a positive multiple of 32)");
    if (b2 && b2_rows <= 0) return mpf::fail(MPF_E_SHAPE, "gemm3_nt: b2_rows must be positive");
    if (!transpose_out && Ndim % 4 != 0) return mpf::fail(MPF_E_SHAPE, "gemm3_nt: Ndim must be a multiple of 4 unless transpose_out");
    G3N p;
    if (int rc = g3n_fill(p, "gemm3_nt", a, lda, 4, b, ldb, 4, c_part, csum_a, R, Mdim, Ndim, rows_per_split)) return rc;
    p.b2 = b2; p.ldb2 = ldb2; p.b2_rows = b2_rows; p.csum_b = csum_b; p.transpose_out = transpose_out;
    p.a_amax = a_amax; p.b_amax = b_amax;
    const bool w96 = g3_col_tile(Ndim).bn == 96;
    g3n_tiles(p, kBM, w96 ? 96 : 128);
    const void* fn = a_amax ? (w96 ? (const void*)gemm3_nt_kernel<96, false, false, false, false, true>
                                   : (const void*)gemm3_nt_kernel<128, false, false, false, false, true>)
                            : (w96 ? (const void*)gemm3_nt_kernel<96> : (const void*)gemm3_nt_kernel<128>);
    const char* name = a_amax ? (w96 ? "gemm3_nt_kernel<96>h2" : "gemm3_nt_kernel<128>h2") : (w96 ? "gemm3_nt_kernel<96>" : "gemm3_nt_kernel<128>");
    return g3_launch(g3n_route(fn, name, "mpf_gemm3_nt", p.ntiles), p, (hipStream_t)stream, g3n_work(p));
}

template <typename Item, bool H2>
int g3_nt_grouped_impl(const Item* items, int n_items, int R, int rows_per_split, int64_t split_stride, void* stream)
{
    if (!items) return mpf::fail(MPF_E_NULL, "gemm3_nt_grouped: NULL items");
    if (n_items <= 0 || n_items > kNtGroupMax) return mpf::fail(MPF_E_SHAPE, "gemm3_nt_grouped: 1..8 items");
    if (R <= 0 || rows_per_split <= 0 || rows_per_split % kBK != 0 || split_stride <= 0)
        return mpf::fail(MPF_E_SHAPE, "gemm3_nt_grouped: bad sizes (rows_per_split must be a positive multiple of 32)");
    G3NG g{};
    Work w{0.0, 0.0};
    bool big = H2 && g_nt2;
    for (int i = 0; i < n_items && big; ++i) big = items[i].Mdim % 256 == 0 && items[i].Ndim % 256 == 0 && items[i].Mdim > 0 && items[i].Ndim > 0;
    for (int i = 0; i < n_items; ++i) {
        const Item& it = items[i];
        if (!it.a || !it.b || !it.c_part) return mpf::fail(MPF_E_NULL, "gemm3_nt_grouped: NULL buffer");
        if (it.Mdim <= 0 || it.Ndim <= 0 || it.Ndim % 4 != 0 || it.Mdim > (1 << 20) || it.Ndim > (1 << 20))
            return mpf::fail(MPF_E_SHAPE, "gemm3_nt_grouped: Ndim must be a positive multiple of 4");
        G3N& p = g.it[i];
        if (int rc = g3n_fill(p, "gemm3_nt_grouped", it.a, it.lda, 4, it.b, it.ldb, 4, it.c_part, it.csum_a, R, (int)it.Mdim, (int)it.Ndim,
                              rows_per_split))
            return rc;
        p.c_ss = p.csa_ss = split_stride; p.csb_ss = 0;
        g3n_tiles(p, big ? 256 : kBM, big ? 256 : 128);
        if constexpr (H2) {
            if (!it.a_amax || !it.b_amax) return mpf::fail(MPF_E_NULL, "gemm3_nt_grouped_h2: NULL amax");
            p.a_amax = it.a_amax; p.b_amax = it.b_amax;
        }
        g.ntiles += p.ntiles;
        g.tile_end[i] = g.ntiles;
        const Work wi = g3n_work(p);
        w.bytes += wi.bytes; w.flops += wi.flops;
    }
    g.n_items = n_items;
// ... 263 lines not shown
```

mp_former_amd/csrc/gemm3_tn3.h:

```cpp
constexpr int kT3BM = 192;
constexpr int kT3T = 512;
constexpr int kT3AKc = kT3BM * 16;
constexpr int kT3A = 2 * 4 * kT3AKc;
constexpr int kT3B = 2 * 256 * 64;
constexpr int kT3Stage = kT3A + kT3B;
constexpr int kT3Lds = 2 * kT3Stage;

__device__ __forceinline__ void split4h(const float4 u, const float scale, uint2* h, uint2* l)
{
    const float x[4] = {u.x, u.y, u.z, u.w};
    unsigned hb[2], lb[2];
#pragma unroll
    for (int i = 0; i < 2; ++i) {
        const f32x2 s = {x[2 * i] * scale, x[2 * i + 1] * scale};
        const f16x2 hh = __builtin_convertvector(s, f16x2);
        const f32x2 back = __builtin_convertvector(hh, f32x2);
        const f32x2 r = {s[0] - back[0], s[1] - back[1]};
        const f16x2 ll = __builtin_convertvector(r, f16x2);
        union { f16x2 f; unsigned u; } ch, cl;
        ch.f = hh; cl.f = ll;
        hb[i] = ch.u; lb[i] = cl.u;
    }
    *h = make_uint2(hb[0], hb[1]);
    *l = make_uint2(lb[0], lb[1]);
}

__global__ __launch_bounds__(kT3T, 2) void gemm3_tn3_kernel(G3 p)
{
    extern __shared__ __attribute__((aligned(16))) unsigned char t3_lds[];
    const int per_xcd = (p.ntiles + 7) >> 3;
    const int tile = ((int)blockIdx.x & 7) * per_xcd + ((int)blockIdx.x >> 3);
    if (tile >= p.ntiles) return;
    const int tm = tile / p.tiles_n, tn = tile - tm * p.tiles_n;
    const int bm = p.t3_bm;
    const int m0 = tm * bm, n0 = tn * 256, m_end = min(m0 + bm, p.M);
    const int tid = threadIdx.x, lane = tid & 63;
    const int wave = __builtin_amdgcn_readfirstlane(tid >> 6);
    const int wr = wave >> 2, wc = wave & 3;
    const int r16 = lane & 15, g = lane >> 4;

    float sc_a, inv_a, sc_b, inv_b;
    h2_scale(amax_read(p.a_amax), &sc_a, &inv_a);
    h2_scale(amax_read(p.b_amax), &sc_b, &inv_b);
    (void)sc_b;

    const int srow = tid >> 3, shc = tid & 7;
    const float* ap[3];
    int aoff[3];
#pragma unroll
    for (int u = 0; u < 3; ++u) {
        const int row = srow + 64 * u;
        ap[u] = p.a + (int64_t)min(m0 + row, m_end - 1) * p.lda + shc * 4;
        const int kc = shc >> 1;
        aoff[u] = kc * kT3AKc + (row ^ (2 * kc)) * 16 + (shc & 1) * 8;
    }
    unsigned boff[4];
    int bdst[4];
    {
        const int nl = lane >> 2, kc = (lane & 3) ^ ((0 - (nl >> 2)) & 3);
#pragma unroll
        for (int i = 0; i < 4; ++i) {
            const int q = wave + 8 * i;
            const int pl = q >> 4, nb = (q & 15) * 16;
            boff[i] = (unsigned)(((int64_t)pl * p.plane + (int64_t)(n0 + nb + nl) * p.K + kc * 8) * 2);
            bdst[i] = __builtin_amdgcn_readfirstlane(kT3A + pl * (256 * 64) + nb * 64);
        }
    }
    const unsigned lds0 = (unsigned)(uintptr_t)t3_lds;

    float4 ra[2][3];
#define T3_LOAD_A(set, k0)                                                            \
    {                                                                                 \
        _Pragma("unroll") for (int u = 0; u < 3; ++u) ra[set][u] = *reinterpret_cast<const float4*>(ap[u] + (k0)); \
    }
    f32x4 acc[6][4];
#pragma unroll
    for (int i = 0; i < 6; ++i)
#pragma unroll
        for (int j = 0; j < 4; ++j) acc[i][j] = f32x4{0.f, 0.f, 0.f, 0.f};

    const int nk = p.K / kBK;
    const int klast = (nk - 1) * kBK;
    const int nrt = wr ? (bm - 96) >> 4 : 6;
    const int a_frag = g * kT3AKc + ((wr * 96 + r16) ^ (2 * g)) * 16;
    const int b_frag = kT3A + (wc * 64 + r16) * 64 + ((g ^ ((0 - (r16 >> 2)) & 3)) * 16);

    T3_LOAD_A(0, 0);
    __builtin_amdgcn_sched_barrier(0);
#pragma unroll
    for (int i = 0; i < 4; ++i) glds16(p.bp, boff[i], lds0 + (unsigned)bdst[i]);
    __builtin_amdgcn_sched_barrier(0);
    T3_LOAD_A(1, min(kBK, klast));
    __builtin_amdgcn_sched_barrier(0);

#define T3_STEP(set, kt)                                                                                                        \
    {                                                                                                                           \
        unsigned char* st = t3_lds + ((kt) & 1) * kT3Stage;                                                                     \
        _Pragma("unroll") for (int u = 0; u < 3; ++u) {                                                                         \
            uint2 h, l;                                                                                                         \
            split4h(ra[set][u], sc_a, &h, &l);                                                                                  \
            *reinterpret_cast<uint2*>(st + aoff[u]) = h;                                                                        \
            *reinterpret_cast<uint2*>(st + 4 * kT3AKc + aoff[u]) = l;                                                           \
        }                                                                                                                       \
        __builtin_amdgcn_sched_barrier(0);                                                                                      \
        T3_LOAD_A(set, min(((kt) + 2) * kBK, klast));                                                                           \
        __builtin_amdgcn_sched_barrier(0);                                                                                      \
         \
        asm volatile("s_waitcnt vmcnt(3)" ::: "memory");                                                                        \
        ws_barrier();                                                                                                           \
                      \
        const int kn = min(((kt) + 1) * kBK, klast);                                                                            \
        const unsigned nst = lds0 + (unsigned)((((kt) + 1) & 1) * kT3Stage);                                                    \
        f16x8 fb[2][4];                                                                                                         \
        _Pragma("unroll") for (int pl = 0; pl < 2; ++pl) _Pragma("unroll") for (int j = 0; j < 4; ++j)                          \
            fb[pl][j] = as_fragh(*reinterpret_cast<const uint4*>(st + b_frag + pl * (256 * 64) + j * 1024));                    \
        _Pragma("unroll") for (int i = 0; i < 6; ++i) {                                                                         \
            if (i == 5 && nrt < 6) break;                                                                                       \
            const f16x8 fh0 = as_fragh(*reinterpret_cast<const uint4*>(st + a_frag + i * 256));                                 \
            const f16x8 fh1 = as_fragh(*reinterpret_cast<const uint4*>(st + a_frag + 4 * kT3AKc + i * 256));                    \
            _Pragma("unroll") for (int j = 0; j < 4; ++j) acc[i][j] = __builtin_amdgcn_mfma_f32_16x16x32_f16(fb[1][j], fh0, acc[i][j], 0, 0, 0); \
            _Pragma("unroll") for (int j = 0; j < 4; ++j) acc[i][j] = __builtin_amdgcn_mfma_f32_16x16x32_f16(fb[0][j], fh1, acc[i][j], 0, 0, 0); \
            _Pragma("unroll") for (int j = 0; j < 4; ++j) acc[i][j] = __builtin_amdgcn_mfma_f32_16x16x32_f16(fb[0][j], fh0, acc[i][j], 0, 0, 0); \
            if (i < 4) glds16(p.bp + kn, boff[i], nst + (unsigned)bdst[i]);                                                     \
        }                                                                                                                       \
    }
    int kt = 0;
    for (; kt + 1 < nk; kt += 2) {
        T3_STEP(0, kt)
        T3_STEP(1, kt + 1)
    }
    if (kt < nk) T3_STEP(0, kt)
#undef T3_STEP
#undef T3_LOAD_A
    asm volatile("s_waitcnt vmcnt(0)" ::: "memory");
    float omax = 0.f;
#pragma unroll
    for (int hf = 0; hf < 2; ++hf) {
        struct { f32x4 v[3][4]; } out;
#pragma unroll
        for (int i = 0; i < 3; ++i)
#pragma unroll
            for (int j = 0; j < 4; ++j) out.v[i][j] = acc[hf * 3 + i][j];
        omax = fmaxf(omax, g3_epilogue<4, 3, decltype(out), true, true>(p, out, lane, m0 + wr * 96 + hf * 48, n0 + wc * 64, inv_a, inv_b, m_end));
    }
    if (p.out_amax) {
        float m = omax;
#pragma unroll
        for (int o = 32; o >= 1; o >>= 1) m = fmaxf(m, __shfl_xor(m, o));
        float* red = reinterpret_cast<float*>(t3_lds);
        __syncthreads();
        if (lane == 0) red[wave] = m;
        __syncthreads();
        if (tid == 0) {
            m = red[0];
#pragma unroll
            for (int w = 1; w < 8; ++w) m = fmaxf(m, red[w]);
            atomicMax(reinterpret_cast<unsigned*>(p.out_amax) + (blockIdx.x % kAmaxSub) * kAmaxStride, __float_as_uint(m));
        }
    }
}
```

mp_former_amd/csrc/mpf_common.h:

```cpp
#pragma once
#include <hip/hip_runtime.h>
#include <string.h>

#include <atomic>
#include <initializer_list>
#include <type_traits>

#include "../../include/mpformer_hip.h"

namespace mpf {
inline size_t align256(size_t x) { return (x + 255) & ~(size_t)255; }

template <int... Vs, class F>
void with_int_of(int v, F&& f) { (void)((v == Vs && (f(std::integral_constant<int, Vs>{}), true)) || ...); }
template <class F>
void with_bool(bool b, F&& f) { b ? f(std::true_type{}) : f(std::false_type{}); }

int fail(int code, const char* msg);
int failf(int code, const char* who, const char* what);
inline bool any_null(std::initializer_list<const void*> ps) { bool null = false; for (const void* p : ps) null |= !p; return null; }
int check(hipError_t err, const char* where);
void set_kernel(const char* name);
void prof_begin(hipStream_t st);
void prof_end(const char* name, hipStream_t st, double algorithmic_bytes, double flops = 0.0);
constexpr int kMaxDevices = 32;
struct LdsAttr { std::atomic<int> bytes[kMaxDevices] = {}; };
inline int ensure_dynamic_lds(const void* fn, size_t bytes, LdsAttr& slots)
{
    int dev = 0;
    if (hipGetDevice(&dev) != hipSuccess || dev < 0 || dev >= kMaxDevices) dev = -1;
    if (dev >= 0 && slots.bytes[dev].load(std::memory_order_relaxed) >= (int)bytes) return 0;
    if (int e = check(hipFuncSetAttribute(fn, hipFuncAttributeMaxDynamicSharedMemorySize, (int)bytes), "hipFuncSetAttribute")) return e;
    if (dev >= 0) slots.bytes[dev].store((int)bytes, std::memory_order_relaxed);
    return 0;
}
inline int cu_count()
{
    static std::atomic<int> cache[kMaxDevices];
    int dev = 0, cus = 0;
    if (hipGetDevice(&dev) != hipSuccess || dev < 0 || dev >= kMaxDevices) return 256;
    cus = cache[dev].load(std::memory_order_relaxed);
    if (cus > 0) return cus;
    if (hipDeviceGetAttribute(&cus, hipDeviceAttributeMultiprocessorCount, dev) != hipSuccess || cus <= 0) cus = 256;
    cache[dev].store(cus, std::memory_order_relaxed);
    return cus;
}
int bf16_rows_add256(const void* g, float* acc, int64_t rows, void* stream);
int set_msda_option(const char* key, int v);
int set_binned_option(const char* key, int v);
int set_gemm3_option(const char* key, int v);
int set_block_option(const char* key, int v);
int set_decoder_option(const char* key, int v);
int set_attn_option(const char* key, int v);
int set_small_gemm_option(const char* key, int v);
}
```

mp_former_amd/encoder_fused.py:

```python
import ctypes
import math
import os
from collections import namedtuple
from itertools import accumulate, chain, islice

import numpy as np
import torch
from torch.autograd import Function

from . import _lib
from .gemm3 import (amax, amax_slots, gemm3_h2, gemm3_h2_bits, gemm3_nt, gemm3_nt_grouped, nt_reduce_levels, split_weights_grouped_h2,
                    workgroup_slots)
from .msda import host_workspace, ms_deform_attn_backward_raw, ms_deform_attn_forward_raw
from .resln import LnGradGroup, ln256_forward, ln_partial_stride

_EPS = 1e-5

RANGE_AUDIT = None

RANGE_GUARD_EVERY = int(os.environ.get("MPF_H2_RANGE_GUARD_EVERY", "64"))
RANGE_GUARD_LOG2 = 18
RANGE_GUARD_SHARE = 1e-3
_GUARD_SLOTS = 64
_guard = {"calls": 0, "active": False, "names": {}, "counters": None, "pending": None, "host": None, "warned": False}


def _guard_begin():
    n = _guard["calls"]
    _guard["calls"] = n + 1
    if RANGE_GUARD_EVERY <= 0 or RANGE_AUDIT is not None:
        return False
    if not (n == 2 or (n > 2 and (n - 2) % RANGE_GUARD_EVERY == 0) or RANGE_GUARD_EVERY == 1):
        return False
    if _guard["pending"] is not None and _guard["pending"][1].query():
        _guard["host"] = _guard["pending"][0].clone()
        _guard["pending"] = None
        _guard_check(_guard["host"])
    if _guard["counters"] is not None and _guard["pending"] is None:
        pinned = torch.empty((_GUARD_SLOTS, 2), dtype=torch.int64).pin_memory()
        pinned.copy_(_guard["counters"], non_blocking=True)
        ev = torch.cuda.Event()
        ev.record()
        _guard["pending"] = (pinned, ev)
    return True


def _guard_shares(host):
    out = {}
    for name, i in _guard["names"].items():
        nz, below = int(host[i, 0]), int(host[i, 1])
        out[name] = {"rows": nz, "below": below, "share": below / nz if nz else 0.0}
    return out


def _guard_check(host):
    bad = {k: v for k, v in _guard_shares(host).items() if v["share"] > RANGE_GUARD_SHARE}
    if bad and not _guard["warned"]:
        import warnings
        _guard["warned"] = True
        worst = max(bad.items(), key=lambda kv: kv[1]["share"])
        warnings.warn("mp_former_amd: fp16 x 2 GEMM operand '%s' has %.3f %% of its non-zero rows below 2^-%d of the operand's largest "
                      "magnitude (%d of %d): those rows keep fewer than 22 bits in the pixel decoder's fp32 GEMMs (DESIGN.md section 2); "
                      "%d operand(s) over the %.1f %% bar" % (worst[0], 100 * worst[1]["share"], RANGE_GUARD_LOG2, worst[1]["below"],
                                                               worst[1]["rows"], len(bad), 100 * RANGE_GUARD_SHARE))


def range_guard_report(sync=False, reset=False):
    if _guard["counters"] is None:
        return {}
    if sync:
        host = _guard["counters"].cpu()
        _guard_check(host)
    else:
        host = _guard["host"]
        if host is None:
            return {}
    rep = _guard_shares(host)
    if reset:
        _guard["counters"].zero_()
        _guard["host"] = _guard["pending"] = None
        _guard["warned"] = False
    return rep


def _audit(name, t, slot):
    if _guard["active"]:
        if _guard["counters"] is None or _guard["counters"].device != t.device:
            _guard["counters"] = torch.zeros((_GUARD_SLOTS, 2), dtype=torch.int64, device=t.device)
        i = _guard["names"].setdefault(name, len(_guard["names"]))
        if i < _GUARD_SLOTS and t.dim() == 2 and t.stride(1) == 1 and t.shape[1] % 4 == 0 and t.stride(0) % 4 == 0:
            _lib.call("mpf_h2_range_stats", t.device, t.data_ptr(), t.shape[0], t.shape[1], t.stride(0), slot.data_ptr(), RANGE_GUARD_LOG2,
                      _guard["counters"][i].data_ptr(), _lib.stream_ptr(t.device))
    if RANGE_AUDIT is None:
        return
    from .gemm3 import amax_value
    ref = amax_value(slot).clamp_min(1e-38)
    r = (t.detach().abs().amax(1) / ref).clamp(2.0 ** -41, 1.0)
    b = torch.floor(-torch.log2(r)).clamp(0, 40).long()
    h = torch.bincount(b, minlength=41)
    RANGE_AUDIT[name] = h if name not in RANGE_AUDIT else RANGE_AUDIT[name] + h


_PARAM_SLOTS = ((("self_attn", "sampling_offsets"), "wso", "bso"), (("self_attn", "attention_weights"), "waw", "baw"),
                (("self_attn", "value_proj"), "wv", "bv"), (("self_attn", "output_proj"), "wo", "bo"), (("norm1",), "g1", "b1"),
                (("linear1",), "w1", "bb1"), (("linear2",), "w2", "bb2"), (("norm2",), "g2", "b2"))
LayerParams = namedtuple("LayerParams", [n for _, w, b in _PARAM_SLOTS for n in (w, b)], defaults=(None,) * (2 * len(_PARAM_SLOTS)))
PARAMS_PER_LAYER = len(LayerParams._fields)
Saved = namedtuple("Saved", "x q value loc attn ao s1 mean1 rstd1 x1 h s2 mean2 rstd2 x_am ao_am x1_am h_am q_am hbits")
_PLANE_SRCS = (("v", ("wv",)), ("o", ("wo",)), ("1", ("w1",)), ("2", ("w2",)), ("288", ("wso", "waw")))
FwdPlanes = namedtuple("FwdPlanes", [f"p{k}{am}" for k, _ in _PLANE_SRCS for am in ("", "_am")])
BwdPlanes = namedtuple("BwdPlanes", [f"t{k}{am}" for k, _ in _PLANE_SRCS for am in ("", "_am")])
FwdAmax = namedtuple("FwdAmax", "ao_am x1_am h_am xn_am qn_am")
BwdAmax = namedtuple("BwdAmax", "ds2_am dh_am ds1_am draw_am gv_am")


def _records(cls, items, n):
    it = iter(items)
    return [cls._make(islice(it, len(cls._fields))) for _ in range(n)], tuple(it)


def _put(row, at, rec):
    for k, t in zip(rec._fields, rec):
        if k in at:
            row[at[k]] = t.data_ptr()


def layer_params(layer):
    owners = layer.__dict__.get("_mpf_param_owners")
    if owners is not None:
        for path, m in owners:
            cur = layer
            for name in path:
                cur = cur._modules.get(name)
                if cur is None:
                    break
            if cur is not m:
                owners = None
                break
    if owners is None:
        owners = []
        for path, _, _ in _PARAM_SLOTS:
            m = layer
            for name in path:
                m = getattr(m, name)
            owners.append((path, m))
        layer.__dict__["_mpf_param_owners"] = owners
    return LayerParams._make(m._parameters[k] for _, m in owners for k in ("weight", "bias"))


def _weight_planes(prm):
    groups = []
    for p in prm:
        srcs = [[getattr(p, n) for n in names] for _, names in _PLANE_SRCS]
        groups += [(w, False) for w in srcs] + [(w, True) for w in srcs]
    it = chain.from_iterable(split_weights_grouped_h2(groups))
    return [(FwdPlanes._make(islice(it, len(FwdPlanes._fields))), BwdPlanes._make(islice(it, len(BwdPlanes._fields)))) for _ in prm]


def rows_per_split(sizes):
    g = 0
    for s_ in sizes:
        g = math.gcd(g, s_)
    for r in (512, 256, 128, 1024, 64, 32):
        if g % r == 0:
# ... 20 lines not shown


_ENC_FIELDS = ("pv", "pv_am", "po", "po_am", "p1", "p1_am", "p2", "p2_am", "p288", "p288_am", "bv", "bo", "bb1", "bb2", "b288", "g1", "b1",
               "g2", "b2", "value", "raw", "loc", "attn", "ao", "s1", "mean1", "rstd1", "x1", "h", "hbits", "s2", "mean2", "rstd2", "x2", "qn",
               "ao_am", "x1_am", "h_am", "xn_am", "qn_am")
_ENC_AT = {k: i for i, k in enumerate(_ENC_FIELDS)}
_NATIVE_FWD = os.environ.get("MPF_ENCODER_NATIVE", "1") != "0"
_NATIVE_BWD = _NATIVE_FWD
ROUTE_CALLS = {"native_fwd": 0, "python_fwd": 0, "native_bwd": 0, "python_bwd": 0}


class MpfEncoderCall(ctypes.Structure):
    _fields_ = [("N", ctypes.c_int32), ("S", ctypes.c_int32), ("M", ctypes.c_int32), ("L", ctypes.c_int32), ("P", ctypes.c_int32),
                ("nl", ctypes.c_int32), ("F", ctypes.c_int32), ("reserved", ctypes.c_int32), ("eps", ctypes.c_float), ("pad_", ctypes.c_float),
                ("host_shapes", ctypes.c_void_p), ("shapes_dev", ctypes.c_void_p), ("lsi_dev", ctypes.c_void_p), ("ref", ctypes.c_void_p),
                ("pos_full", ctypes.c_void_p), ("pos_am", ctypes.c_void_p), ("x0", ctypes.c_void_p), ("x0_am", ctypes.c_void_p),
                ("q0", ctypes.c_void_p), ("q0_am", ctypes.c_void_p), ("layers", ctypes.c_void_p)]


def _native_forward_applies(guarded, meta, C, prm):
    F = prm[0].w1.shape[0]
    return (_NATIVE_FWD and RANGE_AUDIT is None and not guarded and getattr(meta["shapes"], "_mpf_host", None) is not None and C == 256
            and meta["n_heads"] == 8 and F % 128 == 0 and all(p.w1.shape[0] == F for p in prm))


def _arena_members(rows, C, F, no, M, L, P):
    R, f32 = math.prod(rows), torch.float32
    return (("value", (R, C), f32), ("raw", (R, no), f32), ("loc", (*rows, M, L, P, 2), f32), ("attn", (*rows, M, L, P), f32), ("ao", (R, C), f32),
            ("s1", (R, C), f32), ("mean1", (R,), f32), ("rstd1", (R,), f32), ("x1", (R, C), f32), ("h", (R, F), f32),
            ("hbits", (R, F // 8), torch.uint8), ("s2", (R, C), f32), ("mean2", (R,), f32), ("rstd2", (R,), f32), ("x2", (R, C), f32),
            ("qn", (R, C), f32))


_arena_layouts = {}


def _arena_layout(R, C, F, no, M, L, P):
    key = (R, C, F, no, M, L, P)
    hit = _arena_layouts.get(key)
    if hit is None:
        offs, tot = {}, 0
        for name, shape, dt in _arena_members((R,), C, F, no, M, L, P):
            n = math.prod(shape) * dt.itemsize // 4
            offs[name] = (tot, n)
            tot += (n + 3) // 4 * 4
        hit = _arena_layouts[key] = (offs, tot)
    return hit


def _native_forward(x, x_am, q_am, pos_full, pos_am, prm, planes, b288_all, ams, meta, dims):
    N, S, C = dims
    R, nl, F = N * S, len(prm), prm[0].w1.shape[0]
    M, L, P = meta["n_heads"], meta["n_levels"], meta["n_points"]
    no3 = M * L * P * 3
    lib = _lib.lib()
    if lib.mpf_encoder_fields() != len(_ENC_FIELDS):
        raise RuntimeError("MpfEncoderCall field table differs between encoder_fused.py and libmpformer_hip.so")
    q = (x.view(N, S, C) + pos_full).view(R, C)
    amax(q, q_am)
    offs, per = _arena_layout(R, C, F, no3, M, L, P)
    arena = torch.empty((nl, per), dtype=torch.float32, device=x.device)
    tab = np.zeros((nl, len(_ENC_FIELDS)), dtype=np.uint64)
    for row, p, w, am, b288, a in zip(tab, prm, planes, ams, b288_all, arena):
        for rec in (p, w, am):
            _put(row, _ENC_AT, rec)
        row[_ENC_AT["b288"]] = b288.data_ptr()
        for k, (o, _) in offs.items():
            row[_ENC_AT[k]] = a.data_ptr() + 4 * o
    assert tab.all(), "a field of _ENC_FIELDS that no record fills"
    host_shapes = meta["shapes"]._mpf_host
    call = MpfEncoderCall(N, S, M, L, P, nl, F, 0, _EPS, 0.0, host_shapes.data_ptr(), meta["shapes"].data_ptr(), meta["lsi"].data_ptr(),
                          meta["ref"].data_ptr(), pos_full.data_ptr(), pos_am.data_ptr(), x.data_ptr(), x_am.data_ptr(), q.data_ptr(),
                          q_am.data_ptr(), tab.ctypes.data)
    _lib.call("mpf_encoder_forward", x.device, ctypes.byref(call), _lib.stream_ptr(x.device))
    saved, members = [], _arena_members((N, S), C, F, no3, M, L, P)
    for am, a in zip(ams, arena):
        t = {k: a[offs[k][0]:sum(offs[k])].view(dt).view(shape) for k, shape, dt in members}
        saved.append(Saved(x=x, q=q, x_am=x_am, q_am=q_am, ao_am=am.ao_am, x1_am=am.x1_am, h_am=am.h_am,
                           **{k: v for k, v in t.items() if k in Saved._fields}))
        x, q, x_am, q_am = t["x2"], t["qn"], am.xn_am, am.qn_am
    return saved, x


def _python_forward(x, x_am, q_am, pos_full, pos_am, prm, planes, b288_all, ams, meta, dims):
    N, S, C = dims
    R, M, shapes = N * S, meta["n_heads"], meta["shapes"]
    host_shapes = getattr(shapes, "_mpf_host", None)
    saved, q = [], None
    for i, (p, w, am, b288) in enumerate(zip(prm, planes, ams, b288_all)):
        _audit("fwd x (value_proj)", x, x_am)
        value = gemm3_h2(x, x_am, w.pv, w.pv_am, p.bv, out_amax=am.ao_am)
        if q is None:
            q = (x.view(N, S, C) + pos_full).view(R, C)
            amax(q, q_am)
        _audit("fwd q (offsets | weights)", q, q_am)
        raw = gemm3_h2(q, q_am, w.p288, w.p288_am, b288)
        ao, loc, attn = ms_deform_attn_forward_raw(value.view(N, S, M, C // M), shapes, meta["lsi"], raw, meta["ref"], host_shapes)
        ao = ao.view(R, C)
        _audit("fwd attention output (output_proj)", ao, am.ao_am)
        s1 = gemm3_h2(ao, am.ao_am, w.po, w.po_am, p.bo, cin=x)
        x1, mean1, rstd1, _ = ln256_forward(s1, p.g1, p.b1, _EPS, y_bound=am.x1_am)
        if w.p1.shape[1] % 128 == 0:
            h, hbits = gemm3_h2_bits(x1, am.x1_am, w.p1, w.p1_am, p.bb1, relu=True, out_amax=am.h_am, want_bits=True)
        else:
            h, hbits = gemm3_h2(x1, am.x1_am, w.p1, w.p1_am, p.bb1, relu=True, out_amax=am.h_am), None
        _audit("fwd x1 (linear1)", x1, am.x1_am)
        _audit("fwd hidden (linear2)", h, am.h_am)
        s2 = gemm3_h2(h, am.h_am, w.p2, w.p2_am, p.bb2, cin=x1)
        last = i + 1 == len(prm)
        x2, mean2, rstd2, qn = ln256_forward(s2, p.g2, p.b2, _EPS, padd=None if last else pos_full, y_bound=am.xn_am,
                                             padd_amax=None if last else pos_am, yplus_bound=None if last else am.qn_am)
        saved.append(Saved(x, q, value, loc, attn, ao, s1, mean1, rstd1, x1, h, s2, mean2, rstd2, x_am, am.ao_am, am.x1_am, am.h_am, q_am, hbits))
        x, q, x_am, q_am = x2, qn, am.xn_am, am.qn_am
    return saved, x


_ENCB_FIELDS = ("x", "q", "value", "loc", "attn", "ao", "s1", "mean1", "rstd1", "x1", "h", "hbits", "s2", "mean2", "rstd2",
                "x_am", "q_am", "ao_am", "x1_am", "h_am", "g1", "g2", "tv", "tv_am", "to", "to_am", "t1", "t1_am", "t2", "t2_am", "t288", "t288_am",
                "ds2_am", "dh_am", "ds1_am", "draw_am", "gv_am", "wgrad", "dw288", "lvl", "db288")
_ENCB_AT = {k: i for i, k in enumerate(_ENCB_FIELDS)}


class MpfEncoderBwdCall(ctypes.Structure):
    _fields_ = [("N", ctypes.c_int32), ("S", ctypes.c_int32), ("M", ctypes.c_int32), ("L", ctypes.c_int32), ("P", ctypes.c_int32),
                ("nl", ctypes.c_int32), ("F", ctypes.c_int32), ("rps288", ctypes.c_int32), ("rps_group", ctypes.c_int32),
                ("reserved", ctypes.c_int32), ("group_stride", ctypes.c_int64), ("host_shapes", ctypes.c_void_p), ("gout", ctypes.c_void_p),
                ("split_level", ctypes.c_void_p), ("ds2", ctypes.c_void_p), ("dh", ctypes.c_void_p), ("dx1", ctypes.c_void_p),
                ("ds1", ctypes.c_void_p), ("dao", ctypes.c_void_p), ("gv", ctypes.c_void_p), ("draw", ctypes.c_void_p),
                ("dq", ctypes.c_void_p * 2), ("g", ctypes.c_void_p * 2), ("cpart288", ctypes.c_void_p), ("cs288", ctypes.c_void_p),
                ("part_group", ctypes.c_void_p), ("ln_parts", ctypes.c_void_p), ("ln_stride", ctypes.c_uint64), ("msda_ws", ctypes.c_void_p),
                ("msda_ws_bytes", ctypes.c_uint64), ("dgb_out", ctypes.c_void_p), ("layers", ctypes.c_void_p)]


def _native_backward_applies(guarded, meta, aligned, C, prm, saved):
    F = prm[0].w1.shape[0]
    return (_NATIVE_BWD and RANGE_AUDIT is None and not guarded and getattr(meta["shapes"], "_mpf_host", None) is not None and aligned
            and meta["n_levels"] <= 4 and C == 256 and meta["n_heads"] == 8 and F % 256 == 0
            and all(s.hbits is not None and p.w1.shape[0] == F for s, p in zip(saved, prm)))


def _native_backward(gout, prm, saved, planes_t, meta, dims, rps, split_level):
    N, S, C = dims
    R, nl, F = N * S, len(prm), prm[0].w1.shape[0]
    M, L, P = meta["n_heads"], meta["n_levels"], meta["n_points"]
    no, no3 = M * L * P * 2, M * L * P * 3
    dev, lib = gout.device, _lib.lib()
    if lib.mpf_encoder_bwd_fields() != len(_ENCB_FIELDS):
        raise RuntimeError("MpfEncoderBwdCall field table differs between encoder_fused.py and libmpformer_hip.so")
    wgrads = (("w2", "bb2", C, F), ("w1", "bb1", F, C), ("wo", "bo", C, C), ("wv", "bv", C, C))
    rpg = _wgrad_rps(R, [(m_, n_) for _, _, m_, n_ in wgrads], dev)
    ns288, nsg = (R + rps - 1) // rps, (R + rpg - 1) // rpg
    gstride = sum(m_ * n_ + m_ for _, _, m_, n_ in wgrads)
    outs = (("wgrad", gstride), ("dw288", no3 * C), ("lvl", L * no3), ("db288", no3))
    tmps = (("ds2", R * C), ("dx1", R * C), ("ds1", R * C), ("dao", R * C), ("gv", R * C), ("dh", R * F), ("draw", R * no3), ("dq0", R * C),
            ("dq1", R * C), ("g0", R * C), ("g1", R * C), ("cpart", ns288 * no3 * C), ("cs", ns288 * no3), ("pgroup", nsg * gstride))
    oo = dict(zip((k for k, _ in outs), accumulate((n for _, n in outs), initial=0)))
    ot = dict(zip((k for k, _ in tmps), accumulate((n for _, n in tmps), initial=0)))
    out = torch.empty((nl, sum(n for _, n in outs)), dtype=torch.float32, device=dev)
    tmp = torch.empty(sum(n for _, n in tmps), dtype=torch.float32, device=dev)
    t = {k: tmp.data_ptr() + 4 * o for k, o in ot.items()}
    ln_stride = ln_partial_stride(R)
    ln_parts = torch.empty(2 * nl * ln_stride, dtype=torch.uint8, device=dev)
    host_shapes = meta["shapes"]._mpf_host
    stream = _lib.stream_ptr(dev)
    ws = host_workspace(dev, stream, N, M, L, S, P, host_shapes)
    dgb = torch.empty((2 * nl, 2, 256), dtype=torch.float32, device=dev)
    ams, _ = _records(BwdAmax, amax_slots(len(BwdAmax._fields) * nl, dev).unbind(0), nl)
    tab = np.zeros((nl, len(_ENCB_FIELDS)), dtype=np.uint64)
    for row, p, s, w, am, o_ in zip(tab, prm, saved, planes_t, ams, out):
        for rec in (s, p, w, am):
            _put(row, _ENCB_AT, rec)
        for k, o in oo.items():
            row[_ENCB_AT[k]] = o_.data_ptr() + 4 * o
    assert tab.all(), "a field of _ENCB_FIELDS that no record fills"
    call = MpfEncoderBwdCall(N, S, M, L, P, nl, F, rps, rpg, 0, gstride, host_shapes.data_ptr(), gout.data_ptr(), split_level.data_ptr(),
                             t["ds2"], t["dh"], t["dx1"], t["ds1"], t["dao"], t["gv"], t["draw"], (ctypes.c_void_p * 2)(t["dq0"], t["dq1"]),
                             (ctypes.c_void_p * 2)(t["g0"], t["g1"]), t["cpart"], t["cs"], t["pgroup"],
                             ln_parts.data_ptr(), ln_stride, ws.data_ptr(), ws.numel(), dgb.data_ptr(), tab.ctypes.data)
    _lib.call("mpf_encoder_backward", dev, ctypes.byref(call), stream)
    dprm = []
    for o_ in out:
        dw288, db288 = o_[oo["dw288"]:oo["lvl"]].view(no3, C), o_[oo["db288"]:]
        d, k = {}, 0
        for w, b, m_, n_ in wgrads:
            d[w], d[b] = o_[k:k + m_ * n_].view(m_, n_), o_[k + m_ * n_:k + m_ * n_ + m_]
            k += m_ * n_ + m_
        dprm.append(LayerParams(wso=dw288[:no], bso=db288[:no], waw=dw288[no:], baw=db288[no:], **d))
    g = tmp[ot["g0"]:ot["g0"] + R * C].view(R, C)
    return g, dprm, dgb, out[:, oo["lvl"]:oo["db288"]].view(nl, L, no3)


def _python_backward(g, prm, saved, planes_t, meta, dims, rps, aligned, split_level):
    N, S, C = dims
    R, nl = N * S, len(prm)
    M, L = meta["n_heads"], meta["n_levels"]
    sizes, host_shapes = meta["sizes"], getattr(meta["shapes"], "_mpf_host", None)
    no = M * L * meta["n_points"] * 2
    ams, _ = _records(BwdAmax, amax_slots(len(BwdAmax._fields) * nl, g.device).unbind(0), nl)
    dprm, lvls, gq = [None] * nl, [None] * nl, None
    lng = LnGradGroup(2 * nl, R, g.device)
    for i in reversed(range(nl)):
        p, s, t, am = prm[i], saved[i], planes_t[i], ams[i]
        ds2 = lng.backward(s.s2, s.mean2, s.rstd2, p.g2, g, gq, ds_amax=am.ds2_am)
        if s.hbits is not None:
            dh = gemm3_h2_bits(ds2, am.ds2_am, t.t2, t.t2_am, gate_bits=s.hbits, out_amax=am.dh_am)
        else:
            dh = gemm3_h2(ds2, am.ds2_am, t.t2, t.t2_am, gate=s.h, out_amax=am.dh_am)
        _audit("bwd ds2 (d linear2 output)", ds2, am.ds2_am)
        _audit("bwd dh (d hidden)", dh, am.dh_am)
        dx1 = gemm3_h2(dh, am.dh_am, t.t1, t.t1_am, cin=ds2)
        ds1 = lng.backward(s.s1, s.mean1, s.rstd1, p.g1, dx1, ds_amax=am.ds1_am)
        _audit("bwd ds1 (d output_proj output)", ds1, am.ds1_am)
        dao = gemm3_h2(ds1, am.ds1_am, t.to, t.to_am)
        gv, draw = ms_deform_attn_backward_raw(s.value.view(N, S, M, C // M), host_shapes, s.loc, s.attn, dao.view(N, S, C), s.ao.view(N, S, C),
                                               am.draw_am, am.gv_am)
        _audit("bwd draw (d offsets | weights)", draw, am.draw_am)
        _audit("bwd grad_value (d value_proj output)", gv.view(R, C), am.gv_am)
        dq = gemm3_h2(draw, am.draw_am, t.t288, t.t288_am)
        cpart, _, cs = gemm3_nt(s.q, draw, rps, want_csum_b=True, transpose_out=True, amax_ab=(s.q_am, am.draw_am))
        if aligned and L <= 4 and cpart[0].numel() % 4 == 0:
            dw288, lvl, db288 = nt_reduce_levels(cpart, cs, split_level, L)
        else:
            dw288 = cpart.sum(0)
            if aligned:
                lvl = torch.zeros((L, draw.shape[1]), dtype=torch.float32, device=g.device).index_add_(0, split_level, cs)
            else:
                lvl = torch.stack([sl.sum((0, 1)) for sl in draw.view(N, S, -1).split(sizes, 1)])
            db288 = lvl.sum(0)
        lvls[i] = lvl
        gv2 = gv.view(R, C)
        g = gemm3_h2(gv2, am.gv_am, t.tv, t.tv_am, cin=ds1, cin2=dq if i == 0 else None)
        gq = dq
        (w2, bb2), (w1, bb1), (wo, bo), (wv, bv) = _wgrad_group(
            [(ds2, s.h), (dh, s.x1), (ds1, s.ao), (gv2, s.x)], [(am.ds2_am, s.h_am), (am.dh_am, s.x1_am), (am.ds1_am, s.ao_am), (am.gv_am, s.x_am)])
        dprm[i] = LayerParams(wso=dw288[:no], bso=db288[:no], waw=dw288[no:], baw=db288[no:], wv=wv, bv=bv, wo=wo, bo=bo, w1=w1, bb1=bb1,
                              w2=w2, bb2=bb2)
    return g, dprm, lng.finish(), torch.stack(lvls)


class EncoderFn(Function):
    @staticmethod
    def forward(ctx, src, pos_const, level_embed, meta, *params):
        N, S, C = src.shape
        prm, _ = _records(LayerParams, params, len(params) // PARAMS_PER_LAYER)
        nl = len(prm)
        pos_full = pos_const + level_embed.index_select(0, meta["level_idx"])
        x = src.reshape(N * S, C)
        planes = _weight_planes(prm)
        b288_all = torch.cat([t for p in prm for t in (p.bso, p.baw)]).view(nl, -1)
        ams, (x_am, q_am, pos_am) = _records(FwdAmax, amax_slots(len(FwdAmax._fields) * nl + 3, src.device).unbind(0), nl)
        amax(x, x_am)
        amax(pos_full, pos_am)
        ctx.guarded = guarded = _guard_begin()
        native = _native_forward_applies(guarded, meta, C, prm)
        ROUTE_CALLS["native_fwd" if native else "python_fwd"] += 1
        _guard["active"] = guarded
        try:
            saved, x = (_native_forward if native else _python_forward)(x, x_am, q_am, pos_full, pos_am, prm, [f for f, _ in planes], b288_all,
                                                                        ams, meta, (N, S, C))
        finally:
            _guard["active"] = False
        ctx.save_for_backward(*params, *chain.from_iterable(saved))
        ctx.meta, ctx.nl, ctx.dims = meta, nl, (N, S, C)
        ctx.planes_t = [t for _, t in planes]
        return x.view(N, S, C).clone() if native and not any(ctx.needs_input_grad) else x.view(N, S, C)

    @staticmethod
    def backward(ctx, gout):
        N, S, C = ctx.dims
        meta, nl = ctx.meta, ctx.nl
        prm, rest = _records(LayerParams, ctx.saved_tensors, nl)
        saved, _ = _records(Saved, rest, nl)
        g = gout.reshape(N * S, C).contiguous()
        rps, aligned = rows_per_split(meta["sizes"])
        split_level = None
        if aligned:
            key = ("split_level", rps, N)
            split_level = meta.get(key)
            if split_level is None:
                split_level = meta["level_idx"][::rps].repeat(N)
                meta[key] = split_level
        guarded = bool(getattr(ctx, "guarded", False))
        native = _native_backward_applies(guarded, meta, aligned, C, prm, saved)
        ROUTE_CALLS["native_bwd" if native else "python_bwd"] += 1
        if native:
            g, dprm, dgb, lvls_all = _native_backward(g, prm, saved, ctx.planes_t, meta, (N, S, C), rps, split_level)
        else:
            _guard["active"] = guarded
            try:
                g, dprm, dgb, lvls_all = _python_backward(g, prm, saved, ctx.planes_t, meta, (N, S, C), rps, aligned, split_level)
            finally:
                _guard["active"] = False
        for z, i in enumerate(reversed(range(nl))):
            dprm[i] = dprm[i]._replace(g2=dgb[2 * z, 0], b2=dgb[2 * z, 1], g1=dgb[2 * z + 1, 0], b1=dgb[2 * z + 1, 1])
        w288_all = torch.cat([t for p in prm for t in (p.wso, p.waw)]).view(nl, -1, C)
        d_level = (lvls_all[:, :, :, None] * w288_all[:, None, :, :]).sum((0, 2))
        return (g.view(N, S, C), None, d_level, None, *chain.from_iterable(dprm))
```

mp_former_amd/gemm3.py:

```python
import functools

import torch

from . import _lib


def split_weight(w, transpose=False):
    assert w.is_cuda and w.dtype == torch.float32 and w.dim() == 2 and w.is_contiguous()
    r, c = w.shape
    out = torch.empty((3, c, r) if transpose else (3, r, c), dtype=torch.bfloat16, device=w.device)
    _lib.call("mpf_gemm3_split", w.device, w.data_ptr(), r, c, 1 if transpose else 0, out.data_ptr(), _lib.stream_ptr(w.device))
    return out


def split_weights_grouped(groups):
    import numpy as np
    from ._h2d import upload
    dev = groups[0][0][0].device
    sizes, tot = [], 0
    for srcs, _ in groups:
        n = sum(t.numel() for t in srcs)
        sizes.append((tot, n))
        tot += 3 * n
    buf = torch.empty(tot, dtype=torch.bfloat16, device=dev)
    base = buf.data_ptr()
    rows_tab, blk, outs = [], 0, []
    for (srcs, tr), (off, n) in zip(groups, sizes):
        K = srcs[0].shape[1]
        R = sum(t.shape[0] for t in srcs)
        r0 = 0
        for t in srcs:
            assert t.dtype == torch.float32 and t.is_contiguous() and t.shape[1] == K
            dst = base + 2 * (off + (r0 if tr else r0 * K))
            rows_tab.append((t.data_ptr(), dst, t.shape[0], K, 1 if tr else 0, R if tr else K, n, blk))
            blk += (t.numel() + 1023) // 1024
            r0 += t.shape[0]
        outs.append(buf[off:off + 3 * n].view((3, K, R) if tr else (3, R, K)))
    items = upload(np.asarray(rows_tab, dtype=np.int64).reshape(-1), dev)
    _lib.call("mpf_gemm3_split_grouped", dev, items.data_ptr(), len(rows_tab), blk, _lib.stream_ptr(dev))
    return outs


AMAX_SLOT = 512


def amax_slots(n, device):
    return torch.zeros((n, AMAX_SLOT), dtype=torch.float32, device=device)


def amax_value(slot):
    return slot.view(-1)[::32][:16].max()


def amax(t, out=None):
    assert t.is_cuda and t.dtype == torch.float32 and t.is_contiguous()
    if out is None:
        out = torch.zeros(AMAX_SLOT, dtype=torch.float32, device=t.device)
    _lib.call("mpf_amax_f32", t.device, t.data_ptr(), t.numel(), out.data_ptr(), _lib.stream_ptr(t.device))
    return out


def split_weights_grouped_h2(groups):
    import numpy as np
    from ._h2d import upload
    dev = groups[0][0][0].device
    sizes, tot = [], 0
    for srcs, _ in groups:
        n = sum(t.numel() for t in srcs)
        sizes.append((tot, n))
        tot += 2 * n
    buf = torch.empty(tot, dtype=torch.float16, device=dev)
    slots = amax_slots(len(groups), dev)
    base, sbase = buf.data_ptr(), slots.data_ptr()
    am_tab, sp_tab, ablk, sblk, outs = [], [], 0, 0, []
    seen = {}
    for gi, ((srcs, tr), (off, n)) in enumerate(zip(groups, sizes)):
        K = srcs[0].shape[1]
        R = sum(t.shape[0] for t in srcs)
        key = tuple(t.data_ptr() for t in srcs)
        slot = sbase + 4 * AMAX_SLOT * gi
        if key in seen:
            slot_src = seen[key]
        else:
            seen[key] = gi
            slot_src = gi
            for t in srcs:
                am_tab.append((t.data_ptr(), slot, t.numel(), ablk))
                ablk += (t.numel() + 4095) // 4096
        slot = sbase + 4 * AMAX_SLOT * slot_src
        r0 = 0
        for t in srcs:
            assert t.dtype == torch.float32 and t.is_contiguous() and t.shape[1] == K
            dst = base + 2 * (off + (r0 if tr else r0 * K))
            sp_tab.append((t.data_ptr(), dst, slot, t.shape[0], K, 1 if tr else 0, R if tr else K, n, sblk))
            sblk += (t.numel() + 1023) // 1024
            r0 += t.shape[0]
        outs.append((buf[off:off + 2 * n].view((2, K, R) if tr else (2, R, K)), slots[slot_src]))
    both = upload(np.asarray([x for row in am_tab for x in row] + [x for row in sp_tab for x in row], dtype=np.int64), dev)
    _lib.call("mpf_amax_f32_grouped", dev, both.data_ptr(), len(am_tab), ablk, _lib.stream_ptr(dev))
    _lib.call("mpf_gemm3_split_grouped_h2", dev, both.data_ptr() + 8 * 4 * len(am_tab), len(sp_tab), sblk, _lib.stream_ptr(dev))
    return outs


def gemm3_h2(a, a_amax, planes, w_amax, bias=None, cin=None, cin2=None, gate=None, relu=False, out_amax=None):
    assert a.is_cuda and a.dtype == torch.float32 and a.dim() == 2 and a.stride(1) == 1
    assert planes.dtype == torch.float16 and planes.is_contiguous() and planes.shape[0] == 2
    M, K = a.shape
    N = planes.shape[1]
    assert planes.shape[2] == K
    c = torch.empty((M, N), dtype=torch.float32, device=a.device)
    _lib.call("mpf_gemm3_tn_h2", a.device,
              a.data_ptr(), a.stride(0), a_amax.data_ptr(), planes.data_ptr(), w_amax.data_ptr(), _lib.ptr(bias),
              _lib.ptr(cin), _rows(cin, N) if cin is not None else 0, _lib.ptr(cin2), _rows(cin2, N) if cin2 is not None else 0,
              _lib.ptr(gate), _rows(gate, N) if gate is not None else 0, c.data_ptr(), c.stride(0), _lib.ptr(out_amax), M, N, K,
              1 if relu else 0, _lib.stream_ptr(a.device))
    return c


def gemm3_h2_bits(a, a_amax, planes, w_amax, bias=None, cin=None, cin2=None, gate_bits=None, relu=False, out_amax=None,
                  want_bits=False):
    assert a.is_cuda and a.dtype == torch.float32 and a.dim() == 2 and a.stride(1) == 1
    assert planes.dtype == torch.float16 and planes.is_contiguous() and planes.shape[0] == 2
    M, K = a.shape
    N = planes.shape[1]
    assert planes.shape[2] == K and N % 128 == 0
    if gate_bits is not None:
        assert gate_bits.dtype == torch.uint8 and gate_bits.shape == (M, N // 8) and gate_bits.is_contiguous()
    c = torch.empty((M, N), dtype=torch.float32, device=a.device)
    bits = torch.empty((M, N // 8), dtype=torch.uint8, device=a.device) if want_bits else None
    _lib.call("mpf_gemm3_tn_h2_bits", a.device,
              a.data_ptr(), a.stride(0), a_amax.data_ptr(), planes.data_ptr(), w_amax.data_ptr(), _lib.ptr(bias),
              _lib.ptr(cin), _rows(cin, N) if cin is not None else 0, _lib.ptr(cin2), _rows(cin2, N) if cin2 is not None else 0,
              _lib.ptr(gate_bits), N // 8, c.data_ptr(), c.stride(0), _lib.ptr(out_amax), _lib.ptr(bits), N // 8, M, N, K,
              1 if relu else 0, _lib.stream_ptr(a.device))
    return (c, bits) if want_bits else c


def _rows(t, n):
    assert t.dtype == torch.float32 and t.dim() == 2 and t.stride(1) == 1 and t.shape[1] == n
    return t.stride(0)


def gemm3(a, planes, bias=None, a2=None, cin=None, cin2=None, gate=None, relu=False, out=None):
    assert a.is_cuda and a.dtype == torch.float32 and a.dim() == 2 and a.stride(1) == 1
    M, K = a.shape
    N = planes.shape[1]
    assert planes.shape[2] == K and planes.dtype == torch.bfloat16 and planes.is_contiguous()
    c = out if out is not None else torch.empty((M, N), dtype=torch.float32, device=a.device)
    assert c.shape == (M, N) and c.stride(1) == 1
    if a2 is not None:
        assert a2.dtype == torch.float32 and a2.dim() == 2 and a2.is_contiguous() and a2.shape[1] == K
    if bias is not None:
        assert bias.dtype == torch.float32 and bias.is_contiguous() and bias.numel() == N
    _lib.call("mpf_gemm3_tn", a.device,
              a.data_ptr(), a.stride(0), _lib.ptr(a2), a2.shape[0] if a2 is not None else 0, planes.data_ptr(), _lib.ptr(bias),
              _lib.ptr(cin), _rows(cin, N) if cin is not None else 0, _lib.ptr(cin2), _rows(cin2, N) if cin2 is not None else 0,
              _lib.ptr(gate), _rows(gate, N) if gate is not None else 0, c.data_ptr(), c.stride(0), M, N, K,
              1 if relu else 0, _lib.stream_ptr(a.device))
    return c


def pick_rows_per_split(R, out_tiles, align=None):
    want = max(1, 400 // max(out_tiles, 1))
    rps = max(32, (R // want) // 32 * 32)
    if align:
        while rps > 32 and align % rps != 0:
            rps -= 32
        if align % rps != 0:
            return None
    return rps


@functools.lru_cache(None)
def workgroup_slots(device):
    return 2 * torch.cuda.get_device_properties(device).multi_processor_count


def balanced_rps(R, M, N, device, base=1 << 30):
    slots = workgroup_slots(device)
    tiles = ((M + 127) // 128) * ((N + 127) // 128)
    rounds = max(1, -(-tiles * max(1, R // base) // slots))
    ns = max(1, rounds * slots // tiles)
    return max(128, ((-(-R // ns)) + 31) // 32 * 32)


def gemm3_nt(a, b, rows_per_split, b2=None, want_csum_a=False, want_csum_b=False, transpose_out=False, amax_ab=None):
    assert a.is_cuda and a.dtype == torch.float32 and b.dtype == torch.float32
    assert a.dim() == 2 and b.dim() == 2 and a.stride(1) == 1 and b.stride(1) == 1 and a.shape[0] == b.shape[0]
    R, M = a.shape
    N = b.shape[1]
    ns = (R + rows_per_split - 1) // rows_per_split
    c = torch.empty((ns, N, M) if transpose_out else (ns, M, N), dtype=torch.float32, device=a.device)
    ca = torch.empty((ns, M), dtype=torch.float32, device=a.device) if want_csum_a else None
    cb = torch.empty((ns, N), dtype=torch.float32, device=a.device) if want_csum_b else None
    if b2 is not None:
        assert b2.dtype == torch.float32 and b2.dim() == 2 and b2.stride(1) == 1 and b2.shape[1] == N
    if amax_ab is not None:
        assert b2 is None
        _lib.call("mpf_gemm3_nt_h2", a.device,
                  a.data_ptr(), a.stride(0), amax_ab[0].data_ptr(), b.data_ptr(), b.stride(0), amax_ab[1].data_ptr(), c.data_ptr(),
                  _lib.ptr(ca), _lib.ptr(cb), R, M, N, rows_per_split, 1 if transpose_out else 0, _lib.stream_ptr(a.device))
    else:
        _lib.call("mpf_gemm3_nt", a.device,
                  a.data_ptr(), a.stride(0), b.data_ptr(), b.stride(0), _lib.ptr(b2), b2.stride(0) if b2 is not None else 0,
                  b2.shape[0] if b2 is not None else 0, c.data_ptr(), _lib.ptr(ca), _lib.ptr(cb), R, M, N, rows_per_split,
                  1 if transpose_out else 0, _lib.stream_ptr(a.device))
    return c, ca, cb


def gemm3_nt_grouped(pairs, rows_per_split, amax_pairs=None):
    import numpy as np
    R = pairs[0][0].shape[0]
    dev = pairs[0][0].device
    ns = (R + rows_per_split - 1) // rows_per_split
    offs, tot = [], 0
    for g, x in pairs:
        assert g.is_cuda and g.dtype == torch.float32 and x.dtype == torch.float32 and g.dim() == 2 and x.dim() == 2
        assert g.stride(1) == 1 and x.stride(1) == 1 and g.shape[0] == R and x.shape[0] == R and x.shape[1] % 4 == 0
        offs.append(tot)
        tot += (g.shape[1] * x.shape[1] + g.shape[1] + 3) // 4 * 4
    padded = any((g.shape[1] * x.shape[1] + g.shape[1]) % 4 for g, x in pairs)
    part = (torch.zeros if padded else torch.empty)((ns, tot), dtype=torch.float32, device=dev)
    base = part.data_ptr()
    items = np.empty((len(pairs), 8 if amax_pairs is None else 10), dtype=np.int64)
    for i, ((g, x), o) in enumerate(zip(pairs, offs)):
        M, N = g.shape[1], x.shape[1]
        if amax_pairs is None:
            items[i] = (g.data_ptr(), g.stride(0), x.data_ptr(), x.stride(0), base + 4 * o, base + 4 * (o + M * N), M, N)
        else:
            items[i] = (g.data_ptr(), g.stride(0), amax_pairs[i][0].data_ptr(), x.data_ptr(), x.stride(0), amax_pairs[i][1].data_ptr(),
                        base + 4 * o, base + 4 * (o + M * N), M, N)
    _lib.call("mpf_gemm3_nt_grouped" if amax_pairs is None else "mpf_gemm3_nt_grouped_h2", dev,
              items.ctypes.data, len(pairs), R, rows_per_split, tot, _lib.stream_ptr(dev))
    out, _ = nt_reduce(part)
    res = []
    for (g, x), o in zip(pairs, offs):
        M, N = g.shape[1], x.shape[1]
        res.append((out[o:o + M * N].view(M, N), out[o + M * N:o + M * N + M]))
    return res


def nt_reduce(c_part, s_part=None):
    ns = c_part.shape[0]
    c = torch.empty(c_part.shape[1:], dtype=torch.float32, device=c_part.device)
    s = torch.empty(s_part.shape[1:], dtype=torch.float32, device=c_part.device) if s_part is not None else None
    if c.numel() % 4 or (s is not None and s.numel() % 4):
        return c_part.sum(0), (s_part.sum(0) if s_part is not None else None)
    _lib.call("mpf_gemm3_nt_reduce", c_part.device, c_part.data_ptr(), c.numel(), _lib.ptr(s_part), s.numel() if s is not None else 0, ns,
              c.data_ptr(), _lib.ptr(s), _lib.stream_ptr(c_part.device))
    return c, s


def nt_reduce_levels(c_part, s_part, level_of_split, n_levels):
    ns = c_part.shape[0]
    c = torch.empty(c_part.shape[1:], dtype=torch.float32, device=c_part.device)
    n = s_part.shape[1]
    lvl = torch.empty((n_levels, n), dtype=torch.float32, device=c_part.device)
    s = torch.empty((n,), dtype=torch.float32, device=c_part.device)
    assert level_of_split.dtype == torch.int64 and level_of_split.numel() == ns and c.numel() % 4 == 0 and n % 4 == 0 and n_levels <= 4
    _lib.call("mpf_gemm3_nt_reduce_levels", c_part.device, c_part.data_ptr(), c.numel(), s_part.data_ptr(), n, ns,
              level_of_split.data_ptr(), n_levels, c.data_ptr(), lvl.data_ptr(), s.data_ptr(), _lib.stream_ptr(c_part.device))
    return c, lvl, s


def gemm3_ex(a, planes, bias=None, cin=None, relu=False, out_dtype=torch.float32):
    assert a.is_cuda and a.dim() == 2 and a.stride(1) == 1 and a.dtype in (torch.float32, torch.bfloat16)
    M, K = a.shape
    N = planes.shape[1]
    assert planes.shape[2] == K and planes.dtype == torch.bfloat16 and planes.is_contiguous()
    c = torch.empty((M, N), dtype=out_dtype, device=a.device)
    _lib.call("mpf_gemm3_tn_ex", a.device, a.data_ptr(), _lib.DTYPE[a.dtype], a.stride(0), planes.data_ptr(), _lib.ptr(bias), _lib.ptr(cin),
# ... 16 lines not shown
```

Before: 86.57 images/sec.

## Fuse encoder backward dq and value-grad GEMMs into one concatenated-K kernel

In the MSDeformAttn encoder backward, the two GEMMs that make the input gradient (draw x T288 and grad_value x TV) now run as one 192x256 tile kernel that walks both K segments in turn. The intermediate dq buffer and its separate write and read are gone, and dq now goes straight into g for every layer instead of through the next layer's LN backward. To handle the two fp16 split scalings, the accumulator is rescaled with ldexp at the segment boundary and again at the end. This saves one launch and one R x C round trip per layer, at the cost of more complex kernel addressing and some precision risk if the two segments' exponents differ widely.

```diff
diff --git a/include/mpformer_hip.h b/include/mpformer_hip.h
--- a/include/mpformer_hip.h
+++ b/include/mpformer_hip.h
@@ -350,6 +350,9 @@
                     const float* bias, const float* c_in, int64_t ldcin, const float* c_in2, int64_t ldcin2,
                     const float* gate, int64_t ldgate, float* c, int64_t ldc, float* out_amax, int M, int N, int K,
                     int relu, void* stream);
+int mpf_gemm3_tn_h2_cat2(const float* a1, int64_t lda1, const float* a1_amax, const void* w1_planes_h2, const float* w1_amax, int K1,
+                         const float* a2, int64_t lda2, const float* a2_amax, const void* w2_planes_h2, const float* w2_amax, int K2,
+                         const float* c_in, int64_t ldcin, float* c, int64_t ldc, int M, int N, void* stream);
 int mpf_gemm3_tn_h2_bits(const float* a, int64_t lda, const float* a_amax, const void* b_planes_h2, const float* b_amax,
                          const float* bias, const float* c_in, int64_t ldcin, const float* c_in2, int64_t ldcin2,
                          const unsigned char* gate_bits, int64_t ldgbits, float* c, int64_t ldc, float* out_amax,
@@ -582,6 +585,7 @@
     const uint64_t* layers;
 } MpfEncoderBwdCall;
 int mpf_encoder_bwd_fields(void);
+int mpf_encoder_dx_cat(void);
 int mpf_encoder_backward(const MpfEncoderBwdCall* call, void* stream);
 
 int mpf_seg_softmax(const float* cls, int Q, int K1, float object_mask_threshold, float* probs, float* max_score, int* max_label,
diff --git a/mp_former_amd/_lib.py b/mp_former_amd/_lib.py
--- a/mp_former_amd/_lib.py
+++ b/mp_former_amd/_lib.py
@@ -88,6 +88,8 @@
     "mpf_gemm3_split_grouped_h2": (_c_int, [_c_vp, _c_int, ctypes.c_int64, _c_vp]),
     "mpf_gemm3_tn_h2": (_c_int, [_c_vp, ctypes.c_int64, _c_vp, _c_vp, _c_vp, _c_vp, _c_vp, ctypes.c_int64, _c_vp, ctypes.c_int64,
                               _c_vp, ctypes.c_int64, _c_vp, ctypes.c_int64, _c_vp, _c_int, _c_int, _c_int, _c_int, _c_vp]),
+    "mpf_gemm3_tn_h2_cat2": (_c_int, [_c_vp, ctypes.c_int64, _c_vp, _c_vp, _c_vp, _c_int, _c_vp, ctypes.c_int64, _c_vp, _c_vp, _c_vp, _c_int,
+                                   _c_vp, ctypes.c_int64, _c_vp, ctypes.c_int64, _c_int, _c_int, _c_vp]),
     "mpf_gemm3_tn_h2_bits": (_c_int, [_c_vp, ctypes.c_int64, _c_vp, _c_vp, _c_vp, _c_vp, _c_vp, ctypes.c_int64, _c_vp, ctypes.c_int64,
                                    _c_vp, ctypes.c_int64, _c_vp, ctypes.c_int64, _c_vp, _c_vp, ctypes.c_int64,
                                    _c_int, _c_int, _c_int, _c_int, _c_vp]),
@@ -102,6 +104,7 @@
     "mpf_encoder_fields": (_c_int, []),
     "mpf_encoder_forward": (_c_int, [_c_vp, _c_vp]),
     "mpf_encoder_bwd_fields": (_c_int, []),
+    "mpf_encoder_dx_cat": (_c_int, []),
     "mpf_encoder_backward": (_c_int, [_c_vp, _c_vp]),
     "mpf_decoder_layer_struct_bytes": (ctypes.c_uint64, [_c_int]),
     "mpf_decoder_layer_scratch_bytes": (ctypes.c_uint64, [_c_int] * 6),
diff --git a/mp_former_amd/csrc/common.hip b/mp_former_amd/csrc/common.hip
--- a/mp_former_amd/csrc/common.hip
+++ b/mp_former_amd/csrc/common.hip
@@ -147,5 +147,7 @@
     if (r <= 0) return r;
     r = mpf::set_small_gemm_option(key, value);
     if (r <= 0) return r;
+    r = mpf::set_encoder_option(key, value);
+    if (r <= 0) return r;
     return mpf::fail(MPF_E_SHAPE, "mpf_set_option: unknown key");
 }
diff --git a/mp_former_amd/csrc/encoder_layer.hip b/mp_former_amd/csrc/encoder_layer.hip
--- a/mp_former_amd/csrc/encoder_layer.hip
+++ b/mp_former_amd/csrc/encoder_layer.hip
@@ -1,5 +1,6 @@
 #include <hip/hip_runtime.h>
 #include <stdint.h>
+#include <string.h>
 
 #include "mpf_common.h"
 
@@ -11,6 +12,17 @@
 
 extern "C" int mpf_encoder_fields(void) { return MPF_ENC_FIELDS; }
 extern "C" int mpf_encoder_bwd_fields(void) { return MPF_ENCB_FIELDS; }
+
+namespace {
+int g_dx_cat = 1;
+}
+int mpf::set_encoder_option(const char* key, int v)
+{
+    if (strcmp(key, "encoder_dx_cat") != 0) return 1;
+    g_dx_cat = v;
+    return 0;
+}
+extern "C" int mpf_encoder_dx_cat(void) { return g_dx_cat; }
 
 extern "C" int mpf_encoder_forward(const MpfEncoderCall* E, void* st)
 {
@@ -63,7 +75,7 @@
 extern "C" int mpf_encoder_backward(const MpfEncoderBwdCall* E, void* st)
 {
     if (!E || !E->layers || !E->host_shapes || !E->gout || !E->split_level || !E->ds2 || !E->dh || !E->dx1 || !E->ds1 || !E->dao || !E->gv ||
-        !E->draw || !E->dq[0] || !E->dq[1] || !E->g[0] || !E->g[1] || !E->cpart288 || !E->cs288 || !E->part_group || !E->ln_parts ||
+        !E->draw || (!g_dx_cat && (!E->dq[0] || !E->dq[1])) || !E->g[0] || !E->g[1] || !E->cpart288 || !E->cs288 || !E->part_group || !E->ln_parts ||
         !E->msda_ws || !E->dgb_out)
         return mpf::fail(MPF_E_NULL, "encoder_backward: NULL buffer");
     if (E->N <= 0 || E->S <= 0 || E->M != 8 || E->L <= 0 || E->L > 4 || E->P <= 0 || E->nl <= 0 || E->F <= 0 || E->F % 128 != 0 || E->rps288 <= 0 ||
@@ -83,7 +95,7 @@
         auto P = [&](int k) { return reinterpret_cast<void*>(f[k]); };
         auto PF = [&](int k) { return reinterpret_cast<float*>(f[k]); };
         float* g_out = E->g[i & 1];
-        float* dq = E->dq[i & 1];
+        float* dq = g_dx_cat ? nullptr : E->dq[i & 1];
         MPF_TRY(mpf_res_ln256_backward_partial_amax(PF(MPF_ENCB_S2), PF(MPF_ENCB_MEAN2), PF(MPF_ENCB_RSTD2), PF(MPF_ENCB_G2), g_in, nullptr,
                                                     gq_in, E->ds2, nullptr, R, parts + (size_t)kln * E->ln_stride, E->ln_stride,
                                                     PF(MPF_ENCB_DS2_AM), st));
@@ -101,14 +113,19 @@
         MPF_TRY(mpf_msda_backward_ws_raw_o(P(MPF_ENCB_VALUE), E->host_shapes, P(MPF_ENCB_LOC), P(MPF_ENCB_ATTN), E->dao, P(MPF_ENCB_AO), E->gv,
                                            E->draw, E->N, E->S, E->M, 32, E->L, E->S, E->P, MPF_F32, E->msda_ws, E->msda_ws_bytes,
                                            PF(MPF_ENCB_DRAW_AM), PF(MPF_ENCB_GV_AM), st));
-        MPF_TRY(mpf_gemm3_tn_h2(E->draw, NO, PF(MPF_ENCB_DRAW_AM), P(MPF_ENCB_T288), PF(MPF_ENCB_T288_AM), nullptr, nullptr, 0, nullptr, 0,
-                                nullptr, 0, dq, C, nullptr, R, C, NO, 0, st));
+        if (!g_dx_cat)
+            MPF_TRY(mpf_gemm3_tn_h2(E->draw, NO, PF(MPF_ENCB_DRAW_AM), P(MPF_ENCB_T288), PF(MPF_ENCB_T288_AM), nullptr, nullptr, 0, nullptr, 0,
+                                    nullptr, 0, dq, C, nullptr, R, C, NO, 0, st));
         MPF_TRY(mpf_gemm3_nt_h2(PF(MPF_ENCB_Q), C, PF(MPF_ENCB_Q_AM), E->draw, NO, PF(MPF_ENCB_DRAW_AM), E->cpart288, nullptr, E->cs288, R, C, NO,
                                 E->rps288, 1, st));
         MPF_TRY(mpf_gemm3_nt_reduce_levels(E->cpart288, (int64_t)C * NO, E->cs288, NO, ns288, E->split_level, E->L, PF(MPF_ENCB_DW288),
                                            PF(MPF_ENCB_LVL), PF(MPF_ENCB_DB288), st));
-        MPF_TRY(mpf_gemm3_tn_h2(E->gv, C, PF(MPF_ENCB_GV_AM), P(MPF_ENCB_TV), PF(MPF_ENCB_TV_AM), nullptr, E->ds1, C, i == 0 ? dq : nullptr,
-                                i == 0 ? C : 0, nullptr, 0, g_out, C, nullptr, R, C, C, 0, st));
+        if (g_dx_cat)
+            MPF_TRY(mpf_gemm3_tn_h2_cat2(E->draw, NO, PF(MPF_ENCB_DRAW_AM), P(MPF_ENCB_T288), PF(MPF_ENCB_T288_AM), NO, E->gv, C,
+                                         PF(MPF_ENCB_GV_AM), P(MPF_ENCB_TV), PF(MPF_ENCB_TV_AM), C, E->ds1, C, g_out, C, R, C, st));
+        else
+            MPF_TRY(mpf_gemm3_tn_h2(E->gv, C, PF(MPF_ENCB_GV_AM), P(MPF_ENCB_TV), PF(MPF_ENCB_TV_AM), nullptr, E->ds1, C, i == 0 ? dq : nullptr,
+                                    i == 0 ? C : 0, nullptr, 0, g_out, C, nullptr, R, C, C, 0, st));
         {
             float* part = E->part_group;
             const int64_t o2 = 0, o1 = o2 + (int64_t)C * F + C, oo = o1 + (int64_t)F * C + F, ov = oo + (int64_t)C * C + C;
diff --git a/mp_former_amd/csrc/gemm3.hip b/mp_former_amd/csrc/gemm3.hip
--- a/mp_former_amd/csrc/gemm3.hip
+++ b/mp_former_amd/csrc/gemm3.hip
@@ -44,6 +44,12 @@
     int64_t ldgbits, ldgbits_out;
     int gbits_cm;
     int t3_bm;
+    const float* sa;
+    const unsigned short* sbp;
+    int64_t slda, splane;
+    int sK;
+    const float* sa_amax;
+    const float* sb_amax;
 };
 
 int g_ablate = 0;
@@ -110,6 +116,8 @@
     *scale = __uint_as_float((unsigned)(268 - e) << 23);
     *inv = __uint_as_float((unsigned)(e - 14) << 23);
 }
+
+__device__ __forceinline__ int h2_exp(const unsigned amax_bits) { return max((int)((amax_bits >> 23) & 0xffu), 30); }
 
 __device__ __forceinline__ f16x8 as_fragh(const uint4 v)
 {
@@ -1558,6 +1566,8 @@
 inline Work g3_tn_work(const G3& p, const Route& r, double a_el = 4.0)
 {
     const double M = p.M, N = p.N, K = p.K;
+    if (p.sa)
+        return {4.0 * (M * (K + p.sK) + M * N) + r.w_el * N * (K + p.sK) + (p.cin_cm ? 4.0 * M * N : 0.0), 2.0 * M * N * (K + p.sK)};
     return {a_el * M * (p.cv_cin ? p.cv_cin : p.K) + (p.c16 ? 2.0 : 4.0) * M * N + r.w_el * N * K, 2.0 * M * N * K};
 }
 
@@ -1599,6 +1609,23 @@
     Route r;
     r.what = what;
     r.w_el = h2 ? 4.0 : 6.0;
+    auto tn3 = [&](const void* fn, mpf::LdsAttr& attr, const char* name192, const char* name176, const char* what3) {
+        const int cus = mpf::cu_count();
+        if (g_tn3_176 && cdiv(cdiv(M, 176) * (N / 256), cus) <= cdiv(cdiv(M, kT3BM) * (N / 256), cus)) p.t3_bm = 176;
+        p.tiles_n = N / 256;
+        p.ntiles = cdiv(M, p.t3_bm) * p.tiles_n;
+        r.fn = fn;
+        r.name = p.t3_bm == kT3BM ? name192 : name176;
+        r.what = what3;
+        r.threads = kT3T; r.lds = kT3Lds; r.attr = &attr;
+        r.blocks = round8(p.ntiles);
+    };
+    if (p.sa) {
+        static mpf::LdsAttr attr;
+        tn3((const void*)gemm3_tn3_kernel<true>, attr, "gemm3_tn_kernel<h2 192x256 cat2>", "gemm3_tn_kernel<h2 192x256:176 cat2>",
+            "mpf_gemm3_tn_h2_cat2(192x256)");
+        return r;
+    }
     if (h2 && !a2 && !p.gate_cm && !p.cin2_cm && g_ws > 0 && N >= g_ws && p.K == kWsK && N % 256 == 0 && a_al16) {
         const Route ws = g3_ws_route(p);
         if (ws.fn) return ws;
@@ -1606,16 +1633,9 @@
     if (h2 && !a2 && g_tn3 && N % 256 == 0 && M >= 2048 && a_al16 && p.lda % 4 == 0) {
         const int cus = mpf::cu_count(), nt3 = cdiv(M, kT3BM) * (N / 256), rem = nt3 % cus;
         if (g_tn3 == 2 || (nt3 >= cus * 3 / 4 && (rem == 0 || 4 * rem >= 3 * cus || nt3 >= 4 * cus))) {
-            const int nt176 = cdiv(M, 176) * (N / 256);
             static mpf::LdsAttr attr;
-            if (g_tn3_176 && cdiv(nt176, cus) <= cdiv(nt3, cus)) p.t3_bm = 176;
-            p.tiles_n = N / 256;
-            p.ntiles = cdiv(M, p.t3_bm) * p.tiles_n;
-            r.fn = (const void*)gemm3_tn3_kernel;
-            r.name = p.t3_bm == kT3BM ? "gemm3_tn_kernel<h2 192x256>" : "gemm3_tn_kernel<h2 192x256:176>";
-            r.what = "mpf_gemm3_tn_h2(192x256)";
-            r.threads = kT3T; r.lds = kT3Lds; r.attr = &attr;
-            r.blocks = round8(p.ntiles);
+            tn3((const void*)gemm3_tn3_kernel<false>, attr, "gemm3_tn_kernel<h2 192x256>", "gemm3_tn_kernel<h2 192x256:176>",
+                "mpf_gemm3_tn_h2(192x256)");
             return r;
         }
     }
@@ -1683,12 +1703,21 @@
     return r;
 }
 
+struct Seg2 {
+    const float* a;
+    int64_t lda;
+    const float* a_amax;
+    const void* planes;
+    const float* b_amax;
+    int K;
+};
+
 int g3_tn_impl(const float* a, int64_t lda, const float* a2, int a2_rows, const void* b_planes,
                const float* bias, const float* c_in, int64_t ldcin, const float* c_in2, int64_t ldcin2,
                const float* gate, int64_t ldgate, float* c, int64_t ldc, int M, int N, int K,
                int relu, void* stream, const float* a_amax, const float* b_amax, float* out_amax,
                const unsigned char* gbits = nullptr, int64_t ldgbits = 0, unsigned char* gbits_out = nullptr,
-               int64_t ldgbits_out = 0)
+               int64_t ldgbits_out = 0, const Seg2* seg2 = nullptr)
 {
     if (!a || !b_planes || !c) return mpf::fail(MPF_E_NULL, "gemm3_tn: NULL buffer");
     if (M <= 0 || N <= 0 || K <= 0) return mpf::fail(MPF_E_SHAPE, "gemm3_tn: bad sizes");
@@ -1705,6 +1734,14 @@
     if (gbits) { p.gbits = gbits; p.ldgbits = ldgbits; p.gbits_cm = 1; }
     p.gbits_out = gbits_out; p.ldgbits_out = ldgbits_out;
     p.a_amax = a_amax; p.b_amax = b_amax; p.out_amax = out_amax;
+    if (seg2) {
+        if (!seg2->a || !seg2->planes || !seg2->a_amax || !seg2->b_amax || !a_amax || !b_amax) return mpf::fail(MPF_E_NULL, "gemm3_tn_h2_cat2: NULL buffer");
+        if (seg2->K <= 0 || seg2->K % kBK != 0 || N % 256 != 0 || seg2->lda % 4 != 0 || ((uintptr_t)a & 15) || ((uintptr_t)seg2->a & 15))
+            return mpf::fail(MPF_E_SHAPE, "gemm3_tn_h2_cat2: K1, K2 must be multiples of 32, N of 256; 16-byte aligned A rows");
+        if ((int64_t)N * std::max(K, seg2->K) * 4 >= (1ll << 32)) return mpf::fail(MPF_E_TOO_LARGE, "gemm3_tn_h2_cat2: weight planes too large");
+        p.sa = seg2->a; p.slda = seg2->lda; p.sbp = (const unsigned short*)seg2->planes; p.splane = (int64_t)N * seg2->K; p.sK = seg2->K;
+        p.sa_amax = seg2->a_amax; p.sb_amax = seg2->b_amax;
+    }
     const Route r = g3_tn_route(p, false, "mpf_gemm3_tn");
     return g3_launch(r, p, (hipStream_t)stream, g3_tn_work(p, r));
 }
@@ -1745,6 +1782,15 @@
     if (!a_amax || !b_amax) return mpf::fail(MPF_E_NULL, "gemm3_tn_h2: NULL amax");
     return g3_tn_impl(a, lda, nullptr, 0, b_planes_h2, bias, c_in, ldcin, c_in2, ldcin2, gate, ldgate, c, ldc, M, N, K, relu, stream,
                       a_amax, b_amax, out_amax);
+}
+
+extern "C" int mpf_gemm3_tn_h2_cat2(const float* a1, int64_t lda1, const float* a1_amax, const void* w1_planes_h2, const float* w1_amax, int K1,
+                                    const float* a2, int64_t lda2, const float* a2_amax, const void* w2_planes_h2, const float* w2_amax, int K2,
+                                    const float* c_in, int64_t ldcin, float* c, int64_t ldc, int M, int N, void* stream)
+{
+    const Seg2 seg2{a2, lda2, a2_amax, w2_planes_h2, w2_amax, K2};
+    return g3_tn_impl(a1, lda1, nullptr, 0, w1_planes_h2, nullptr, c_in, ldcin, nullptr, 0, nullptr, 0, c, ldc, M, N, K1, 0, stream,
+                      a1_amax, w1_amax, nullptr, nullptr, 0, nullptr, 0, &seg2);
 }
 
 extern "C" int mpf_gemm3_tn_h2_bits(const float* a, int64_t lda, const float* a_amax, const void* b_planes_h2, const float* b_amax,
diff --git a/mp_former_amd/csrc/gemm3_tn3.h b/mp_former_amd/csrc/gemm3_tn3.h
--- a/mp_former_amd/csrc/gemm3_tn3.h
+++ b/mp_former_amd/csrc/gemm3_tn3.h
@@ -25,6 +25,7 @@
     *l = make_uint2(lb[0], lb[1]);
 }
 
+template <bool CAT>
 __global__ __launch_bounds__(kT3T, 2) void gemm3_tn3_kernel(G3 p)
 {
     extern __shared__ __attribute__((aligned(16))) unsigned char t3_lds[];
@@ -43,18 +44,31 @@
     h2_scale(amax_read(p.a_amax), &sc_a, &inv_a);
     h2_scale(amax_read(p.b_amax), &sc_b, &inv_b);
     (void)sc_b;
+    float sc_a2 = 0.f;
+    int cat_d = 0, cat_unit = 0;
+    if constexpr (CAT) {
+        const int eb2 = h2_exp(amax_read(p.sb_amax));
+        const int s1 = 282 - h2_exp(amax_read(p.a_amax)) - h2_exp(amax_read(p.b_amax));
+        const int s2 = 282 - h2_exp(amax_read(p.sa_amax)) - eb2;
+        cat_d = min(s2 - s1, 64);
+        cat_unit = s1 + cat_d;
+        sc_a2 = ldexpf(1.f, cat_unit - (141 - eb2));
+    }
+    const int nk1 = p.K / kBK;
 
     const int srow = tid >> 3, shc = tid & 7;
     const float* ap[3];
+    int arow[3];
     int aoff[3];
 #pragma unroll
     for (int u = 0; u < 3; ++u) {
         const int row = srow + 64 * u;
-        ap[u] = p.a + (int64_t)min(m0 + row, m_end - 1) * p.lda + shc * 4;
+        arow[u] = min(m0 + row, m_end - 1);
+        ap[u] = p.a + (int64_t)arow[u] * p.lda + shc * 4;
         const int kc = shc >> 1;
         aoff[u] = kc * kT3AKc + (row ^ (2 * kc)) * 16 + (shc & 1) * 8;
     }
-    unsigned boff[4];
+    unsigned boff[4], boff2[4];
     int bdst[4];
     {
         const int nl = lane >> 2, kc = (lane & 3) ^ ((0 - (nl >> 2)) & 3);
@@ -63,15 +77,32 @@
             const int q = wave + 8 * i;
             const int pl = q >> 4, nb = (q & 15) * 16;
             boff[i] = (unsigned)(((int64_t)pl * p.plane + (int64_t)(n0 + nb + nl) * p.K + kc * 8) * 2);
+            boff2[i] = CAT ? (unsigned)(((int64_t)pl * p.splane + (int64_t)(n0 + nb + nl) * p.sK + kc * 8) * 2) : 0u;
             bdst[i] = __builtin_amdgcn_readfirstlane(kT3A + pl * (256 * 64) + nb * 64);
         }
     }
     const unsigned lds0 = (unsigned)(uintptr_t)t3_lds;
 
     float4 ra[2][3];
-#define T3_LOAD_A(set, k0)                                                            \
+#define T3_LOAD_A(set, s)                                                             \
     {                                                                                 \
-        _Pragma("unroll") for (int u = 0; u < 3; ++u) ra[set][u] = *reinterpret_cast<const float4*>(ap[u] + (k0)); \
+        if constexpr (CAT) {                                                          \
+            const bool s2_ = (s) >= nk1;                                              \
+            const float* ab_ = (s2_ ? p.sa : p.a) + ((s2_ ? (s) - nk1 : (s)) * kBK + shc * 4); \
+            const int64_t ld_ = s2_ ? p.slda : p.lda;                                 \
+            _Pragma("unroll") for (int u = 0; u < 3; ++u) ra[set][u] = *reinterpret_cast<const float4*>(ab_ + arow[u] * ld_); \
+        } else {                                                                      \
+            _Pragma("unroll") for (int u = 0; u < 3; ++u) ra[set][u] = *reinterpret_cast<const float4*>(ap[u] + (s) * kBK); \
+        }                                                                             \
+    }
+#define T3_LOAD_B(i, s, nst_)                                                         \
+    {                                                                                 \
+        if constexpr (CAT) {                                                          \
+            const bool s2_ = (s) >= nk1;                                              \
+            glds16((s2_ ? p.sbp : p.bp) + (s2_ ? (s) - nk1 : (s)) * kBK, s2_ ? boff2[i] : boff[i], (nst_) + (unsigned)bdst[i]); \
+        } else {                                                                      \
+            glds16(p.bp + (s) * kBK, boff[i], (nst_) + (unsigned)bdst[i]);            \
+        }                                                                             \
     }
     f32x4 acc[6][4];
 #pragma unroll
@@ -79,8 +110,8 @@
 #pragma unroll
         for (int j = 0; j < 4; ++j) acc[i][j] = f32x4{0.f, 0.f, 0.f, 0.f};
 
-    const int nk = p.K / kBK;
-    const int klast = (nk - 1) * kBK;
+    const int nk = CAT ? nk1 + p.sK / kBK : nk1;
+    const int slast = nk - 1;
     const int nrt = wr ? (bm - 96) >> 4 : 6;
     const int a_frag = g * kT3AKc + ((wr * 96 + r16) ^ (2 * g)) * 16;
     const int b_frag = kT3A + (wc * 64 + r16) * 64 + ((g ^ ((0 - (r16 >> 2)) & 3)) * 16);
@@ -88,29 +119,36 @@
     T3_LOAD_A(0, 0);
     __builtin_amdgcn_sched_barrier(0);
 #pragma unroll
-    for (int i = 0; i < 4; ++i) glds16(p.bp, boff[i], lds0 + (unsigned)bdst[i]);
+    for (int i = 0; i < 4; ++i) T3_LOAD_B(i, 0, lds0);
     __builtin_amdgcn_sched_barrier(0);
-    T3_LOAD_A(1, min(kBK, klast));
+    T3_LOAD_A(1, min(1, slast));
     __builtin_amdgcn_sched_barrier(0);
 
 #define T3_STEP(set, kt)                                                                                                        \
     {                                                                                                                           \
         unsigned char* st = t3_lds + ((kt) & 1) * kT3Stage;                                                                     \
+        const float sc_ = CAT && (kt) >= nk1 ? sc_a2 : sc_a;                                                                    \
         _Pragma("unroll") for (int u = 0; u < 3; ++u) {                                                                         \
             uint2 h, l;                                                                                                         \
-            split4h(ra[set][u], sc_a, &h, &l);                                                                                  \
+            split4h(ra[set][u], sc_, &h, &l);                                                                                   \
             *reinterpret_cast<uint2*>(st + aoff[u]) = h;                                                                        \
             *reinterpret_cast<uint2*>(st + 4 * kT3AKc + aoff[u]) = l;                                                           \
         }                                                                                                                       \
         __builtin_amdgcn_sched_barrier(0);                                                                                      \
-        T3_LOAD_A(set, min(((kt) + 2) * kBK, klast));                                                                           \
+        T3_LOAD_A(set, min((kt) + 2, slast));                                                                                   \
         __builtin_amdgcn_sched_barrier(0);                                                                                      \
          \
         asm volatile("s_waitcnt vmcnt(3)" ::: "memory");                                                                        \
         ws_barrier();                                                                                                           \
                       \
-        const int kn = min(((kt) + 1) * kBK, klast);                                                                            \
+        const int kn = min((kt) + 1, slast);                                                                                    \
         const unsigned nst = lds0 + (unsigned)((((kt) + 1) & 1) * kT3Stage);                                                    \
+        if constexpr (CAT) {          \
+            if ((kt) == nk1) {                                                                                                  \
+                _Pragma("unroll") for (int i = 0; i < 6; ++i) _Pragma("unroll") for (int j = 0; j < 4; ++j)                     \
+                    _Pragma("unroll") for (int e = 0; e < 4; ++e) acc[i][j][e] = ldexpf(acc[i][j][e], cat_d);                   \
+            }                                                                                                                   \
+        }                                                                                                                       \
         f16x8 fb[2][4];                                                                                                         \
         _Pragma("unroll") for (int pl = 0; pl < 2; ++pl) _Pragma("unroll") for (int j = 0; j < 4; ++j)                          \
             fb[pl][j] = as_fragh(*reinterpret_cast<const uint4*>(st + b_frag + pl * (256 * 64) + j * 1024));                    \
@@ -121,7 +159,7 @@
             _Pragma("unroll") for (int j = 0; j < 4; ++j) acc[i][j] = __builtin_amdgcn_mfma_f32_16x16x32_f16(fb[1][j], fh0, acc[i][j], 0, 0, 0); \
             _Pragma("unroll") for (int j = 0; j < 4; ++j) acc[i][j] = __builtin_amdgcn_mfma_f32_16x16x32_f16(fb[0][j], fh1, acc[i][j], 0, 0, 0); \
             _Pragma("unroll") for (int j = 0; j < 4; ++j) acc[i][j] = __builtin_amdgcn_mfma_f32_16x16x32_f16(fb[0][j], fh0, acc[i][j], 0, 0, 0); \
-            if (i < 4) glds16(p.bp + kn, boff[i], nst + (unsigned)bdst[i]);                                                     \
+            if (i < 4) T3_LOAD_B(i, kn, nst)                                                                                    \
         }                                                                                                                       \
     }
     int kt = 0;
@@ -131,7 +169,17 @@
     }
     if (kt < nk) T3_STEP(0, kt)
 #undef T3_STEP
+#undef T3_LOAD_B
 #undef T3_LOAD_A
+    if constexpr (CAT) {
+#pragma unroll
+        for (int i = 0; i < 6; ++i)
+#pragma unroll
+            for (int j = 0; j < 4; ++j)
+#pragma unroll
+                for (int e = 0; e < 4; ++e) acc[i][j][e] = ldexpf(acc[i][j][e], -cat_unit);
+        inv_a = inv_b = 1.f;
+    }
     asm volatile("s_waitcnt vmcnt(0)" ::: "memory");
     float omax = 0.f;
 #pragma unroll
diff --git a/mp_former_amd/csrc/mpf_common.h b/mp_former_amd/csrc/mpf_common.h
--- a/mp_former_amd/csrc/mpf_common.h
+++ b/mp_former_amd/csrc/mpf_common.h
@@ -53,4 +53,5 @@
 int set_decoder_option(const char* key, int v);
 int set_attn_option(const char* key, int v);
 int set_small_gemm_option(const char* key, int v);
+int set_encoder_option(const char* key, int v);
 }
diff --git a/mp_former_amd/encoder_fused.py b/mp_former_amd/encoder_fused.py
--- a/mp_former_amd/encoder_fused.py
+++ b/mp_former_amd/encoder_fused.py
@@ -9,7 +9,7 @@
 from torch.autograd import Function
 
 from . import _lib
-from .gemm3 import (amax, amax_slots, gemm3_h2, gemm3_h2_bits, gemm3_nt, gemm3_nt_grouped, nt_reduce_levels, split_weights_grouped_h2,
+from .gemm3 import (amax, amax_slots, gemm3_h2, gemm3_h2_bits, gemm3_h2_cat2, gemm3_nt, gemm3_nt_grouped, nt_reduce_levels, split_weights_grouped_h2,
                     workgroup_slots)
 from .msda import host_workspace, ms_deform_attn_backward_raw, ms_deform_attn_forward_raw
 from .resln import LnGradGroup, ln256_forward, ln_partial_stride
@@ -336,13 +336,16 @@
     ns288, nsg = (R + rps - 1) // rps, (R + rpg - 1) // rpg
     gstride = sum(m_ * n_ + m_ for _, _, m_, n_ in wgrads)
     outs = (("wgrad", gstride), ("dw288", no3 * C), ("lvl", L * no3), ("db288", no3))
-    tmps = (("ds2", R * C), ("dx1", R * C), ("ds1", R * C), ("dao", R * C), ("gv", R * C), ("dh", R * F), ("draw", R * no3), ("dq0", R * C),
-            ("dq1", R * C), ("g0", R * C), ("g1", R * C), ("cpart", ns288 * no3 * C), ("cs", ns288 * no3), ("pgroup", nsg * gstride))
+    dq_floats = 0 if lib.mpf_encoder_dx_cat() else R * C
+    tmps = (("ds2", R * C), ("dx1", R * C), ("ds1", R * C), ("dao", R * C), ("gv", R * C), ("dh", R * F), ("draw", R * no3), ("dq0", dq_floats),
+            ("dq1", dq_floats), ("g0", R * C), ("g1", R * C), ("cpart", ns288 * no3 * C), ("cs", ns288 * no3), ("pgroup", nsg * gstride))
     oo = dict(zip((k for k, _ in outs), accumulate((n for _, n in outs), initial=0)))
     ot = dict(zip((k for k, _ in tmps), accumulate((n for _, n in tmps), initial=0)))
     out = torch.empty((nl, sum(n for _, n in outs)), dtype=torch.float32, device=dev)
     tmp = torch.empty(sum(n for _, n in tmps), dtype=torch.float32, device=dev)
     t = {k: tmp.data_ptr() + 4 * o for k, o in ot.items()}
+    if not dq_floats:
+        t["dq0"] = t["dq1"] = None
     ln_stride = ln_partial_stride(R)
     ln_parts = torch.empty(2 * nl * ln_stride, dtype=torch.uint8, device=dev)
     host_shapes = meta["shapes"]._mpf_host
@@ -382,6 +385,7 @@
     no = M * L * meta["n_points"] * 2
     ams, _ = _records(BwdAmax, amax_slots(len(BwdAmax._fields) * nl, g.device).unbind(0), nl)
     dprm, lvls, gq = [None] * nl, [None] * nl, None
+    dx_cat = bool(_lib.lib().mpf_encoder_dx_cat())
     lng = LnGradGroup(2 * nl, R, g.device)
     for i in reversed(range(nl)):
         p, s, t, am = prm[i], saved[i], planes_t[i], ams[i]
@@ -400,7 +404,7 @@
                                                am.draw_am, am.gv_am)
         _audit("bwd draw (d offsets | weights)", draw, am.draw_am)
         _audit("bwd grad_value (d value_proj output)", gv.view(R, C), am.gv_am)
-        dq = gemm3_h2(draw, am.draw_am, t.t288, t.t288_am)
+        dq = None if dx_cat else gemm3_h2(draw, am.draw_am, t.t288, t.t288_am)
         cpart, _, cs = gemm3_nt(s.q, draw, rps, want_csum_b=True, transpose_out=True, amax_ab=(s.q_am, am.draw_am))
         if aligned and L <= 4 and cpart[0].numel() % 4 == 0:
             dw288, lvl, db288 = nt_reduce_levels(cpart, cs, split_level, L)
@@ -413,7 +417,10 @@
             db288 = lvl.sum(0)
         lvls[i] = lvl
         gv2 = gv.view(R, C)
-        g = gemm3_h2(gv2, am.gv_am, t.tv, t.tv_am, cin=ds1, cin2=dq if i == 0 else None)
+        if dx_cat:
+            g = gemm3_h2_cat2(draw, am.draw_am, t.t288, t.t288_am, gv2, am.gv_am, t.tv, t.tv_am, cin=ds1)
+        else:
+            g = gemm3_h2(gv2, am.gv_am, t.tv, t.tv_am, cin=ds1, cin2=dq if i == 0 else None)
         gq = dq
         (w2, bb2), (w1, bb1), (wo, bo), (wv, bv) = _wgrad_group(
             [(ds2, s.h), (dh, s.x1), (ds1, s.ao), (gv2, s.x)], [(am.ds2_am, s.h_am), (am.dh_am, s.x1_am), (am.ds1_am, s.ao_am), (am.gv_am, s.x_am)])
diff --git a/mp_former_amd/gemm3.py b/mp_former_amd/gemm3.py
--- a/mp_former_amd/gemm3.py
+++ b/mp_former_amd/gemm3.py
@@ -117,6 +117,20 @@
     return c
 
 
+def gemm3_h2_cat2(a1, a1_amax, planes1, w1_amax, a2, a2_amax, planes2, w2_amax, cin=None):
+    for a, planes in ((a1, planes1), (a2, planes2)):
+        assert a.is_cuda and a.dtype == torch.float32 and a.dim() == 2 and a.stride(1) == 1
+        assert planes.dtype == torch.float16 and planes.is_contiguous() and planes.shape[0] == 2 and planes.shape[2] == a.shape[1]
+    M, N = a1.shape[0], planes1.shape[1]
+    assert a2.shape[0] == M and planes2.shape[1] == N and N % 256 == 0
+    c = torch.empty((M, N), dtype=torch.float32, device=a1.device)
+    _lib.call("mpf_gemm3_tn_h2_cat2", a1.device,
+              a1.data_ptr(), a1.stride(0), a1_amax.data_ptr(), planes1.data_ptr(), w1_amax.data_ptr(), a1.shape[1],
+              a2.data_ptr(), a2.stride(0), a2_amax.data_ptr(), planes2.data_ptr(), w2_amax.data_ptr(), a2.shape[1],
+              _lib.ptr(cin), _rows(cin, N) if cin is not None else 0, c.data_ptr(), c.stride(0), M, N, _lib.stream_ptr(a1.device))
+    return c
+
+
 def gemm3_h2_bits(a, a_amax, planes, w_amax, bias=None, cin=None, cin2=None, gate_bits=None, relu=False, out_amax=None,
                   want_bits=False):
     assert a.is_cuda and a.dtype == torch.float32 and a.dim() == 2 and a.stride(1) == 1
```

After: 87.06 images/sec, median of 6. About the same (+0.6%).
